# bigpon/QPNet

Hardware: AMD Instinct MI355X
Metric: train steps/sec (batch-1 chunk-steps of RF+20000 samples, aggregate over GPUs) (higher is better)
Workload: dtype f32; 1 GPU; config[1]: paper-size SI-QPNet (C=64,S=256,4F+4A) training step, forward+CE+backward+Adam on one chunk of 20900 samples (RF 946 + batch_length 19954), batch 1 per GPU; global_batch=1, parallelism=dp1 (utterance-sharded chunks, one flat-gradient all-reduce per step), backend=none, world_size=1, aux_1x1=frame rate (hoisted: K = 128 + one 4-deep step)

## Files before the change

### qpnet_amd/csrc/train_bwd.hip

```cpp
#include "train_common.h"
#include "train_post.h"
#include "qpn_handle.h"
#include <string.h>
#include <stdlib.h>
#include <math.h>

template <int MT>
__global__ __launch_bounds__(512) void k_post_bwd(TrainParams p, TrainBwd bw) {
    constexpr int TM = 16 * MT;
    extern __shared__ float sm[];
    const int S = p.S, Q = p.Q, LC = p.LC;
    const int ldp = tr_lda(Q > S ? Q : S), ldr = tr_lda(S);
    float* P = sm; float* R = sm + TM * ldp;
    const int b = blockIdx.y, t0 = blockIdx.x * TM;
    const int tid = threadIdx.x, lane = tid & 63, wave = tid >> 6;
    const int NTS = S / 16;
    const int npairs = (NTS + 1) / 2;
    const int np0 = wave < npairs ? wave : 0;
    const int pnt[2] = {2 * np0, (2 * np0 + 1 < NTS) ? 2 * np0 + 1 : 2 * np0};
    float my[2][MT][4], ms[2][MT][4];
    auto mask_load = [&](const float* src, float (&m)[2][MT][4]) {
#pragma unroll
        for (int j = 0; j < 2; ++j)
#pragma unroll
// ... 1031 lines not shown
            float ev[TR_EB_SLOTS];
#pragma unroll
            for (int k = 0; k < TR_EB_SLOTS; ++k) ev[k] = p.EB[(size_t)(l * TR_EB_SLOTS + k) * 2 * C + n];
#pragma unroll
            for (int k = 0; k < TR_EB_SLOTS; ++k) e += ev[k];
        }
        float acc = 0.f;
        for (int b = 0; b < p.B; ++b) {
            const float* hb = p.h + ((size_t)b * A + a) * p.F + p.ffirst;
            const float* D = p.DPA + (size_t)(l * p.B + b) * (p.nfr + 1) * 2 * C + n;
            for (int f0 = 0; f0 < p.nfr; f0 += 1024) {
                const int nf = p.nfr - f0 < 1024 ? p.nfr - f0 : 1024;
                __syncthreads();
                for (int i = tid; i < nf; i += 128) hrow[i] = hb[f0 + i];
                __syncthreads();
                int f = 0;
                for (; f + 64 <= nf; f += 64) {
                    float d[64];
#pragma unroll
                    for (int k = 0; k < 64; ++k) d[k] = D[(size_t)(f0 + f + k) * 2 * C];
#pragma unroll
                    for (int k = 0; k < 64; ++k) acc += d[k] * hrow[f + k];
                }
                for (; f + 16 <= nf; f += 16) {
                    float d[16];
#pragma unroll
                    for (int k = 0; k < 16; ++k) d[k] = D[(size_t)(f0 + f + k) * 2 * C];
#pragma unroll
                    for (int k = 0; k < 16; ++k) acc += d[k] * hrow[f + k];
                }
                for (; f < nf; ++f) acc += D[(size_t)(f0 + f) * 2 * C] * hrow[f];
            }
        }
        p.gflat[wi] = (acc + p.flat[p.up_b] * e) * p.gscale;
        v = va * e;
    } else {
        const int j = bx - L * A;
        const int q0 = p.F * p.U - p.N1;
        const int items = L * p.B * p.nfr;
        for (int it = tid; it < items; it += 128) {
            const int fx = it % p.nfr, lb = it / p.nfr, l = lb / p.B;
            const int n = (p.ffirst + fx) * p.U + j - q0;
            if (n >= ag.s_out[l] && n < p.N1) v += p.GW[(size_t)lb * p.N1 + n];
        }
    }
    for (int sft = 32; sft >= 1; sft >>= 1) v += __shfl_xor(v, sft);
    if ((tid & 63) == 0) red[tid >> 6] = v;
    __syncthreads();
    if (tid == 0) {
        if (role_a) atomicAdd(p.gflat + p.up_b, (red[0] + red[1]) * p.gscale);
        else p.gflat[p.up_w + (bx - L * A)] = (red[0] + red[1]) * p.gscale;
    }
}

struct AdamReports { int* h_status; double* h_loss; const double* d_loss; };
__device__ __forceinline__ void adam_update(float* __restrict__ w, float* __restrict__ m, float* __restrict__ v, int64_t i, float gi,
                                            float lr, float b1, float b2, float eps, float wd, float bc1, float bc2_sqrt) {
    if (wd != 0.f) gi += wd * w[i];
    const float mi = m[i] + (gi - m[i]) * (1.0f - b1);
    const float vi = v[i] * b2 + (1.0f - b2) * gi * gi;
    m[i] = mi; v[i] = vi;
    const float denom = sqrtf(vi) / bc2_sqrt + eps;
    w[i] = w[i] - (lr / bc1) * (mi / denom);
}
__global__ void k_adam(float* __restrict__ w, const float* __restrict__ g, float* __restrict__ m, float* __restrict__ v, int64_t n,
                       float lr, float b1, float b2, float eps, float wd, float bc1, float bc2_sqrt, const float* __restrict__ den, int* __restrict__ status, AdamReports rep) {
    int64_t i = (int64_t)blockIdx.x * blockDim.x + threadIdx.x;
    const bool peer = den && den[1] > 0.f;
    const bool skip = peer || (status && *status);
    if (blockIdx.x == 0) {
        if (rep.h_loss && threadIdx.x < 64) rep.h_loss[threadIdx.x] = rep.d_loss[threadIdx.x];
        if (threadIdx.x == 0 && status) {
            int st = *status;
            if (peer && !st) { st = 8; atomicOr(status, 8); }
            if (rep.h_status) *rep.h_status = st;
            if (!skip) atomicAdd((unsigned long long*)(status + 2), 1ull);
        }
    }
    if (i >= n || skip) return;
    float gi = g[i];
    if (den) gi = gi / den[0];
    adam_update(w, m, v, i, gi, lr, b1, b2, eps, wd, bc1, bc2_sqrt);
}

__device__ __forceinline__ double block_sum_f64(double x, double* red) {
    for (int sft = 32; sft >= 1; sft >>= 1) x += __shfl_xor(x, sft);
    if ((threadIdx.x & 63) == 0) red[threadIdx.x >> 6] = x;
    __syncthreads();
    return (red[0] + red[1]) + (red[2] + red[3]);
}
__global__ __launch_bounds__(256) void k_grad_sumsq(const float* __restrict__ g, int64_t n, double* __restrict__ part) {
    __shared__ double red[4];
    const int64_t nq = n >> 2, nthr = (int64_t)gridDim.x * 256, t = (int64_t)blockIdx.x * 256 + threadIdx.x;
    double acc = 0.0;
    if ((reinterpret_cast<uintptr_t>(g) & 15) == 0) {
        const float4* g4 = reinterpret_cast<const float4*>(g);
#pragma unroll 4
        for (int64_t q = t; q < nq; q += nthr) {
            const float4 x = g4[q];
            acc += (double)x.x * (double)x.x; acc += (double)x.y * (double)x.y; acc += (double)x.z * (double)x.z; acc += (double)x.w * (double)x.w;
        }
    } else {
#pragma unroll 4
        for (int64_t q = t; q < nq; q += nthr) {
            const float x0 = g[4 * q], x1 = g[4 * q + 1], x2 = g[4 * q + 2], x3 = g[4 * q + 3];
            acc += (double)x0 * (double)x0; acc += (double)x1 * (double)x1; acc += (double)x2 * (double)x2; acc += (double)x3 * (double)x3;
        }
    }
    if (t == nq % nthr) for (int64_t i = nq * 4; i < n; ++i) acc += (double)g[i] * (double)g[i];
    const double s = block_sum_f64(acc, red);
    if (threadIdx.x == 0) part[blockIdx.x] = s;
}

__global__ __launch_bounds__(256) void k_adam_clip(float* __restrict__ w, const float* __restrict__ g, float* __restrict__ m, float* __restrict__ v, int64_t n,
                                                   float lr, float b1, float b2, float eps, float wd, float bc1, float bc2_sqrt, const float* __restrict__ den, int* __restrict__ status, AdamReports rep,
                                                   const double* __restrict__ part, int npart, float max_norm, double* __restrict__ d_norm, double* h_norm) {
    __shared__ double red[4];
    int64_t i = (int64_t)blockIdx.x * blockDim.x + threadIdx.x;
    double total = sqrt(block_sum_f64((int)threadIdx.x < npart ? part[threadIdx.x] : 0.0, red));
    if (den) total = total / (double)den[0];
    const bool bad = !isfinite(total);
    const bool peer = den && den[1] > 0.f;
    const bool skip = bad || peer || (status && *status);
    if (blockIdx.x == 0) {
        if (rep.h_loss && threadIdx.x < 64) rep.h_loss[threadIdx.x] = rep.d_loss[threadIdx.x];
        if (threadIdx.x == 0) {
            *d_norm = total;
            if (h_norm) *h_norm = total;
            if (status) {
                int st = *status;
                if (peer && !st) { st = 8; atomicOr(status, 8); }
                if (bad) { st |= 1 << 16; atomicOr(status, 1 << 16); }
                if (rep.h_status) *rep.h_status = st;
                if (!skip) atomicAdd((unsigned long long*)(status + 2), 1ull);
            }
        }
    }
    if (i >= n || skip) return;
    const double c = (double)max_norm / (total + 1e-6);
    const float coef = c < 1.0 ? (float)c : 1.0f;
    float gi = g[i];
    if (den) gi = gi / den[0];
    gi = __fmul_rn(gi, coef);
    adam_update(w, m, v, i, gi, lr, b1, b2, eps, wd, bc1, bc2_sqrt);
}

__device__ __forceinline__ void zero_dx_slice(const TrainParams& p, const TrainBwd& bw, int j, int b, size_t part, size_t nparts, int t, int nthr) {
    const int C = p.C;
    const TrLayer ly = p.layers[j];
    const size_t nDX = (size_t)p.B * p.N1 * C;
    float* A = bw.DXA[0] + (size_t)j * nDX + (size_t)b * p.N1 * C;
    float* Bq = bw.DXB[0] + (size_t)j * nDX + (size_t)b * p.N1 * C;
    const int a0 = j == 0 ? 0 : ly.s_in, a1 = ly.s_out;
    const int b0 = ly.adaptive ? 0 : p.N1 - ly.dilation, b1 = p.N1;
    const size_t na = (size_t)(a1 - a0) * C / 4, nb = (size_t)(b1 > b0 ? b1 - b0 : 0) * C / 4;
    const float4 z = make_float4(0.f, 0.f, 0.f, 0.f);
    const size_t nh = p.hoist ? (size_t)(p.nfr + 1) * 2 * C / 4 : (j == 0 ? (size_t)p.N1 * p.Ap / 4 : 0);
    const size_t ne = (p.hoist && b == 0) ? (size_t)TR_EB_SLOTS * 2 * C / 4 : 0;
    float* H = p.hoist ? bw.DPA + (size_t)(j * p.B + b) * (p.nfr + 1) * 2 * C : bw.DHUP + (size_t)b * p.N1 * p.Ap;
    for (size_t i = part * nthr + t; i < na + nb + nh + ne; i += nparts * nthr) {
        if (i < na) ((float4*)(A + (size_t)a0 * C))[i] = z;
        else if (i < na + nb) ((float4*)(Bq + (size_t)(b0 > 0 ? b0 : 0) * C))[i - na] = z;
        else if (i < na + nb + nh) ((float4*)H)[i - na - nb] = z;
        else ((float4*)(bw.EB + (size_t)j * TR_EB_SLOTS * 2 * C))[i - na - nb - nh] = z;
    }
}
__global__ void k_zero_dx(TrainParams p, TrainBwd bw) {
    zero_dx_slice(p, bw, blockIdx.y, blockIdx.z, blockIdx.x, gridDim.x, threadIdx.x, blockDim.x);
}

void qpn_launch_zero_dx(const TrainParams& p, const TrainBwd& bw, hipStream_t stream) {
    hipLaunchKernelGGL(k_zero_dx, dim3(64, p.L, p.B), dim3(256), 0, stream, p, bw);
}

static void launch_reduce_early(const TrainBwd& bw, hipStream_t st, int tail, int nch_side) {
    const TrainSlabs& sl = *bw.sl;
    const int64_t n = (int64_t)(sl.g_early1 - sl.g_early0) + (tail ? bw.n_gzero + 4 : 0);
    hipLaunchKernelGGL(k_reduce_grad_s, dim3((unsigned)((n + 255) / 256)), dim3(256), 0, st, bw.slab, bw.gdst, bw.gdst_list, bw.gzero, bw.n_gzero,
                       nch_side, bw.gstage, bw.n_params, bw.gflat, bw.gscale, bw.append_scale, sl.g_early0, sl.g_early1, 0, 0, tail, bw.status, 0);
}
static void launch_up_bwd(const TrainParams& p, const TrainBwd& bw, hipStream_t st) {
    const UpArgs u = up_args(p, bw);
    hipLaunchKernelGGL(k_up_bwd, dim3(u.nfr, p.B), dim3(128), 0, st, u);
}

static void launch_aux_tail(const TrainParams& p, const TrainBwd& bw, const AuxGeom& ag, hipStream_t st) {
    hipLaunchKernelGGL(k_aux_tail, dim3(p.L * p.A + p.U), dim3(128), 0, st, tr_aux_args(p, &bw, ag));
}

int qpn_launch_grad_tail(const TrainParams& p, const TrainBwd& bw, const AuxGeom* ag, hipStream_t stream, bool early_done, bool up_done) {
    const int C = p.C, Q = p.Q, B = p.B, N1 = p.N1;
    const TrainSlabs& sl = *bw.sl;
    hipLaunchKernelGGL(k_reduce_grad_s, dim3((unsigned)(((int64_t)bw.gstage + (up_done ? 0 : bw.n_gzero + 4) + 255) / 256)), dim3(256), 0, stream, bw.slab, bw.gdst, bw.gdst_list, bw.gzero, bw.n_gzero,
                       bw.nch, bw.gstage, bw.n_params, bw.gflat, bw.gscale, bw.append_scale, 0, bw.gstage, early_done ? sl.g_early0 : 0, early_done ? sl.g_early1 : 0, up_done ? 0 : 1, bw.status, bw.append_scale == 1 ? 1 : 0);
    {
        const int64_t total = (int64_t)B * N1;
        const int nwg = 128, rpw = (int)((total + nwg - 1) / nwg);
        if (sl.g_cw < 0) {
            int CB = C < 64 ? C : 64;
            while (CB > 1 && (size_t)2 * Q * CB * sizeof(float) > 128 * 1024) CB /= 2;
            const size_t lds_c = (size_t)2 * Q * CB * sizeof(float);
            if (lds_c > 160 * 1024) { qpn_set_error("causal-table gradient: n_quantize too large for the LDS histogram"); return QPN_EINVAL; }
            if (lds_c > 48 * 1024) QPN_HIP(hipFuncSetAttribute((const void*)k_causal_bwd, hipFuncAttributeMaxDynamicSharedMemorySize, (int)lds_c));
            hipLaunchKernelGGL(k_causal_bwd, dim3(nwg), dim3(256), lds_c, stream, p, bw, rpw, CB);
        }
        if (p.U > 0 && !up_done && !p.hoist) launch_up_bwd(p, bw, stream);
        if (p.hoist && ag && !up_done) launch_aux_tail(p, bw, *ag, stream);
    }
    qpn_prof_mark(PG_GRAD_TAIL, stream);
    QPN_HIP(hipGetLastError());
    return QPN_OK;
}

bool qpn_stack_bwd_fits(const TrainParams& p);
int qpn_launch_stack_bwd(const TrainParams& p, const TrainBwd& bw, const StackQ& q, const TrainKnobs& k, hipStream_t stream);

void qpn_launch_post_fb(const TrainParams& p, const TrainBwd& bw, hipStream_t stream) {
    constexpr int MTW = 5;
    const size_t ldsw = (size_t)16 * MTW * (tr_lda(256) + 2 * tr_lda(64)) * sizeof(float);
    (void)hipFuncSetAttribute((const void*)k_post_fb_w<MTW>, hipFuncAttributeMaxDynamicSharedMemorySize, (int)ldsw);
    hipLaunchKernelGGL((k_post_fb_w<MTW>), dim3((p.BL + 16 * MTW - 1) / (16 * MTW), p.B), dim3(512), ldsw, stream, p, bw, 1);
}

int qpn_launch_bwd(const TrainParams& p, const TrainBwd& bw, const TrainKnobs& k, const AuxGeom& ag, const StackQ* sq, hipStream_t stream, bool post_done) {
    const int C = p.C, S = p.S, Q = p.Q, L = p.L, B = p.B, N1 = p.N1, BL = p.BL;
    const TrainSlabs& sl = *bw.sl;
    const bool off32 = N1 < (1 << 24) && (int64_t)N1 * (p.LC > 2 * C ? p.LC : 2 * C) < (1ll << 32);
    const bool persist = C == 64 && (p.Ktp == 176 || p.hoist) && p.Ap <= 64 && off32 && k.persist_bwd;
    const bool stack_q = persist && k.stack_q_bwd && sq && sq->flags && p.qctl && qpn_stack_bwd_fits(p);
    const bool wr_summed = stack_q;
    const size_t nDX = (size_t)B * N1 * C;
    const size_t lds_post = (size_t)16 * (tr_lda(Q > S ? Q : S) + tr_lda(S)) * sizeof(float);
    const size_t lds_layer = (size_t)16 * (4 * tr_lda(C) + tr_lda(2 * C)) * sizeof(float);
    if (lds_post > 160 * 1024 || lds_layer > 160 * 1024) { qpn_set_error("backward tiles do not fit LDS"); return QPN_EINVAL; }
    hipStream_t side = bw.side; hipEvent_t ev_fork = bw.ev_fork, ev_join = bw.ev_join;
    const bool overlap = side && !qpn_prof_serial() && !k.serial;
    const bool post_wide = S == 256 && Q == 256 && C == 64 && (p.LC == 256 || p.LC == 512) && k.post_wide;
    const bool zero_in_post = post_wide && k.zero_in_post;
    if (post_done) { }
    else if (!zero_in_post) qpn_launch_zero_dx(p, bw, stream);
    if (post_done) { }
    else if (post_wide) {
        constexpr int MTW = 5;
        const size_t ldsw = (size_t)16 * MTW * tr_lda(256) * sizeof(float);
        QPN_HIP(hipFuncSetAttribute((const void*)k_post_bwd_w<MTW>, hipFuncAttributeMaxDynamicSharedMemorySize, (int)ldsw));
        hipLaunchKernelGGL((k_post_bwd_w<MTW>), dim3((BL + 16 * MTW - 1) / (16 * MTW), B), dim3(512), ldsw, stream, p, bw, zero_in_post ? 1 : 0);
    } else {
        if (lds_post > 48 * 1024) (void)hipFuncSetAttribute((const void*)k_post_bwd<1>, hipFuncAttributeMaxDynamicSharedMemorySize, (int)lds_post);
        hipLaunchKernelGGL((k_post_bwd<1>), dim3((BL + 15) / 16, B), dim3(512), lds_post, stream, p, bw);
    }
    qpn_prof_mark(PG_POST_BWD, stream);
    const int nch = bw.nch;
    int nch_side_ = nch;
    const bool gen = k.wgrad_generic;
    Wg2 wbase; memset(&wbase, 0, sizeof(wbase));
    wbase.slab = bw.slab; wbase.gstage = bw.gstage; wbase.nb = B; wbase.C = C; wbase.Ap = p.Ap; wbase.hup = p.HUP; wbase.tap = p.TAP; wbase.ncol_groups = 1;
    bool ok = true;
    auto launch_skip_post = [&](hipStream_t st) {
        Wg2 w = wbase;
        {
            w.nlayers = L;
            w.A = bw.DS0; w.A2 = nullptr; w.A_lstride = 0; w.lda = S; w.M = S; w.rowsA = BL;
            w.bmode = 0; w.B1 = p.TH; w.B2 = nullptr; w.B_lstride = nDX; w.ldb = C; w.N = C; w.Nvalid = C; w.rowsB = N1; w.ldc = C;
            w.ncol_groups = wgrad_col_groups(w.M, w.N);
            for (int l = 0; l < L; ++l) { w.row0A[l] = 0; w.row0B[l] = N1 - BL; w.R[l] = BL; w.goff[l] = sl.g_ws[l]; w.gbias[l] = l == 0 ? sl.g_bs : -1; w.tap_off[l] = -1; }
            ok = ok && wgrad2_any(w, nch_side_, gen, st);
            qpn_prof_mark(PG_WGRAD_SKIP, st);
        }
        {
            w.nlayers = 1; w.A_lstride = w.B_lstride = 0; w.B2 = nullptr; w.bmode = 1; w.rowsA = w.rowsB = BL;
            w.row0A[0] = w.row0B[0] = 0; w.R[0] = BL; w.tap_off[0] = -1;
            w.ncol_groups = S % 64 == 0 ? S / 64 : 1;
            w.A = bw.dlogits; w.lda = Q; w.M = Q; w.B1 = p.Y0; w.ldb = S; w.N = S; w.Nvalid = S; w.ldc = S; w.goff[0] = sl.g_p2; w.gbias[0] = sl.g_bp2;
            if (Q == S && k.post_pair) {
                w.nlayers = 2;
                w.A_lstride = (size_t)(bw.DY0 - bw.dlogits); w.B_lstride = (size_t)(p.S0 - p.Y0);
                w.row0A[1] = w.row0B[1] = 0; w.R[1] = BL; w.tap_off[1] = -1; w.goff[1] = sl.g_p1; w.gbias[1] = sl.g_bp1;
                ok = ok && wgrad2_any(w, nch_side_, gen, st);
            } else {
                ok = ok && wgrad2_any(w, nch_side_, gen, st);
                w.A = bw.DY0; w.lda = S; w.M = S; w.B1 = p.S0; w.goff[0] = sl.g_p1; w.gbias[0] = sl.g_bp1;
                ok = ok && wgrad2_any(w, nch_side_, gen, st);
            }
            qpn_prof_mark(PG_WGRAD_POST, st);
        }
    };
    auto build_w1 = [&]() {
        Wg2 w = wbase;
        w.A = bw.DZ; w.A2 = nullptr; w.A_lstride = (size_t)B * N1 * 2 * C; w.lda = 2 * C; w.M = 2 * C; w.rowsA = N1;
        w.bmode = 3; w.B1 = p.X; w.B2 = nullptr; w.B_lstride = nDX; w.ldb = C; w.N = p.Ktp; w.Nvalid = p.hoist ? 2 * C : 2 * C + p.Ap; w.rowsB = N1;
        w.nlayers = L; w.ldc = p.Ktp; w.ncol_groups = wgrad_col_groups(w.M, w.N);
        for (int l = 0; l < L; ++l) {
            const TrLayer& ly = p.layers[l];
            w.row0A[l] = w.row0B[l] = ly.s_out; w.R[l] = N1 - ly.s_out; w.goff[l] = sl.g_w1[l]; w.gbias[l] = sl.g_b1[l];
            w.tap_off[l] = ly.tap_off; w.dil[l] = ly.dilation;
        }
        return w;
    };
    auto build_wr = [&]() {
        Wg2 w = wbase;
        w.A = bw.DXA[0] + nDX; w.A2 = wr_summed ? nullptr : bw.DXB[0] + nDX; w.A_lstride = nDX; w.lda = C; w.M = C; w.rowsA = N1;
        w.bmode = 0; w.B1 = p.TH; w.B2 = nullptr; w.B_lstride = nDX; w.ldb = C; w.N = C; w.Nvalid = C; w.rowsB = N1; w.ldc = C;
        w.nlayers = L; w.ncol_groups = wgrad_col_groups(w.M, w.N);
        for (int l = 0; l < L; ++l) {
            w.row0A[l] = w.row0B[l] = p.layers[l].s_out;
            w.R[l] = l == L - 1 ? 0 : N1 - p.layers[l].s_out; w.goff[l] = sl.g_wr[l]; w.gbias[l] = sl.g_br[l]; w.tap_off[l] = -1; w.dil[l] = 0;
        }
        return w;
    };
    const bool early_reduce = overlap && bw.gdst && sl.g_early1 > sl.g_early0 && k.reduce_early;
    const bool up_side = early_reduce && p.U > 0 && k.up_side;
    if (early_reduce) {
        nch_side_ = k.wgrad_chunks_side > 0 && k.wgrad_chunks_side <= nch ? k.wgrad_chunks_side : (nch <= 48 ? nch : 48);
    }
    if (overlap) {
        QPN_HIP(hipEventRecord(ev_fork, stream));
        QPN_HIP(hipStreamWaitEvent(side, ev_fork, 0));
        qpn_prof_mark(-1, side);
        launch_skip_post(side);
        if (early_reduce) { launch_reduce_early(bw, side, up_side ? 1 : 0, nch_side_); qpn_prof_mark(PG_GRAD_TAIL, side); }
        if (early_reduce && up_side && bw.ev_early && bw.early_recorded) { QPN_HIP(hipEventRecord(bw.ev_early, side)); *bw.early_recorded = 1; }
    }
    const int swz = k.xcd_swizzle ? 1 : 0;
    if (p.hoist && !persist) { qpn_set_error("internal: the frame-rate aux term needs the register-resident layer kernels"); return QPN_EINVAL; }
    if (stack_q) {
        const int rcq = qpn_launch_stack_bwd(p, bw, *sq, k, stream);
        if (rcq) return rcq;
    }
    for (int l = L - 1; l >= 0 && !stack_q; --l) {
        const TrLayer& ly = p.layers[l];
        const int rows = N1 - ly.s_out;
        const int tiles = (rows + 15) / 16;
        if (persist) {
            int G = qpn_num_cus() * 2; if (G > tiles) G = tiles;
            if (G > 1024) G = 1024;
            const size_t ldsp = (size_t)(8 * 16 * tr_lda(C) + 16 * tr_lda(2 * C) + 16 * tr_lda(p.Ktp) + 64) * sizeof(float);
            const bool last = l == L - 1;
            const void* kf = p.hoist ? (last ? (const void*)k_layer_bwd_p<8, true> : (const void*)k_layer_bwd_p<8, false>)
                                     : (last ? (const void*)k_layer_bwd_p<11, true> : (const void*)k_layer_bwd_p<11, false>);
            (void)hipFuncSetAttribute(kf, hipFuncAttributeMaxDynamicSharedMemorySize, (int)ldsp);
            if (p.hoist) {
                if (last) hipLaunchKernelGGL((k_layer_bwd_p<8, true>), dim3(G, B), dim3(256), ldsp, stream, p, bw, l, swz ? 2 : 0, tiles, p.scratch_rows);
                else hipLaunchKernelGGL((k_layer_bwd_p<8, false>), dim3(G, B), dim3(256), ldsp, stream, p, bw, l, swz ? 2 : 0, tiles, p.scratch_rows);
            } else {
                if (last) hipLaunchKernelGGL((k_layer_bwd_p<11, true>), dim3(G, B), dim3(256), ldsp, stream, p, bw, l, swz ? 2 : 0, tiles, p.scratch_rows);
                else hipLaunchKernelGGL((k_layer_bwd_p<11, false>), dim3(G, B), dim3(256), ldsp, stream, p, bw, l, swz ? 2 : 0, tiles, p.scratch_rows);
            }
        } else {
            if (lds_layer > 48 * 1024) (void)hipFuncSetAttribute((const void*)k_layer_bwd<1>, hipFuncAttributeMaxDynamicSharedMemorySize, (int)lds_layer);
            hipLaunchKernelGGL((k_layer_bwd<1>), dim3(tiles, B), dim3(256), lds_layer, stream, p, bw, l, l == L - 1 ? 1 : 0, swz);
        }
    }
    auto build_causal = [&]() {
        Wg2 w = wbase;
        w.nlayers = 2; w.ncol_groups = Q / (Q % 64 == 0 ? 64 : 128);      w.bmode = 4; w.xc = p.XC; w.B1 = w.B2 = nullptr; w.B_lstride = 0;
        w.A = bw.DXA[0]; w.A2 = bw.DXB[0]; w.A_lstride = 0; w.lda = C; w.M = C; w.rowsA = N1;
        w.N = Q; w.Nvalid = Q; w.rowsB = N1 + 1; w.ldb = 0; w.ldc = Q;
        for (int tp = 0; tp < 2; ++tp) { w.row0A[tp] = 0; w.row0B[tp] = tp; w.R[tp] = N1; w.goff[tp] = sl.g_cw + tp * C * Q; w.gbias[tp] = tp == 0 ? sl.g_cb : -1; w.tap_off[tp] = -1; w.dil[tp] = 0; }
        return w;
    };
    const bool wr_side = overlap && k.wr_side;
    if (wr_side || up_side) {
        QPN_HIP(hipEventRecord(bw.ev_mid, stream));
        QPN_HIP(hipStreamWaitEvent(side, bw.ev_mid, 0));
        qpn_prof_mark(-1, side);
        if (up_side) { if (p.hoist) launch_aux_tail(p, bw, ag, side); else launch_up_bwd(p, bw, side); qpn_prof_mark(PG_GRAD_TAIL, side); }
        if (wr_side) { ok = ok && wgrad2_any(build_wr(), nch, gen, side); qpn_prof_mark(PG_WGRAD_WR, side); }
    }
    if (overlap) QPN_HIP(hipEventRecord(ev_join, side));
    qpn_prof_mark(PG_LAYER_BWD, stream);
    ok = ok && wgrad2_any(build_w1(), nch, gen, stream);
    qpn_prof_mark(PG_WGRAD, stream);
    if (!wr_side) { ok = ok && wgrad2_any(build_wr(), nch, gen, stream); qpn_prof_mark(PG_WGRAD_WR, stream); }
    if (!overlap) launch_skip_post(stream);
    if (sl.g_cw >= 0) ok = ok && wgrad2_any(build_causal(), nch, gen, stream);
    qpn_prof_mark(PG_WGRAD_CAUSAL, stream);
    if (overlap) { QPN_HIP(hipStreamWaitEvent(stream, ev_join, 0)); qpn_prof_mark(-1, stream); }
    if (!ok) { qpn_set_error("weight-gradient tiles: unsupported geometry (n_resch <= 128 on this path; wider stacks take the GEMM path)"); return QPN_EINVAL; }
    return qpn_launch_grad_tail(p, bw, &ag, stream, early_reduce, up_side);
}

int qpn_launch_adam(float* w, const float* g, float* m, float* v, int64_t n, int step, float lr, float b1, float b2, float eps, float wd, const float* den, int* status,
                    int* h_status, double* h_loss, const double* d_loss, hipStream_t stream) {
// ... 22 lines not shown
```

### qpnet_amd/csrc/train_common.h

```cpp
#pragma once
#include "qpn_common.h"

typedef float f32x4 __attribute__((ext_vector_type(4)));

#define TR_MAXL QPN_MAX_LAYERS

__host__ __device__ static inline int tr_lda(int K) { return ((K + 29) / 32) * 32 + 2; }
__host__ __device__ static inline int tr_ldt(int N) { return ((N + 15) / 32) * 32 + 16; }

struct TrLayer {
    int adaptive, dilation;
    int s_in, s_out;
    int tap_off;
    int w1_f4, wr_f4;
    int w1t_f4, wrt_f4;
    int bias1, biasr;
};

struct TrainParams {
    int C, S, Q, A, Ap, L, U;
    int B, T, F, Td, BL, N1, N0, maxd;
    int Kt, Ktp;
    int LC;
    const float* flat;
    const float4* wp;
    const float* ct;
    float* bp;
    const int64_t* x; const float* h; const float* d;
    float* X;
    float* SG; float* TH;
    float* HUP;
    int hoist;
    int nfr, ffirst;
    float* PA;
    float2* WJ;
    int* TAP;
    int* XC;
    float* S0; float* Y0;
    float* logits;
    const int64_t* ce_tgt; int64_t ce_stride; float* ce_dlogits; double* ce_loss;
    int* status;
    float* scratch_rows;
    unsigned* qctl;
    int4* qtab;
    int4* qtab_b;
    int qtotal;
    int qP[TR_MAXL + 1];
    int qT[TR_MAXL];
    int ws_f4, p1_f4, p2_f4;
    int wst_f4, p1t_f4, p2t_f4;
    int bias_s, bias_p1, bias_p2;
    int64_t causal_w, causal_b, up_w, up_b;
    TrLayer layers[TR_MAXL];
};

struct TrainSlabs {
    int g_w1[TR_MAXL], g_b1[TR_MAXL], g_wr[TR_MAXL], g_br[TR_MAXL], g_ws[TR_MAXL], g_bs;
    int g_p1, g_bp1, g_p2, g_bp2;
    int g_early0, g_early1;
    int g_cw, g_cb;
};

struct TrainBwd {
    const float* dlogits; float* gflat;
    float* DXA[2]; float* DXB[2];
    float* DZ;
    float* DS0; float* DY0;
    float* DGS;
    float* DHUP;
    float* DPA;
    float* GW;
    float* EB;
    float* slab;
    const int* gdst; const int* gdst_list;
    const int* gzero; int n_gzero;
    int nch, gstage;
    int64_t n_params;
    const struct TrainSlabs* sl;
    float gscale;
    int append_scale;
    const int* status;
    hipStream_t side; hipEvent_t ev_fork, ev_join, ev_mid;
    hipEvent_t ev_early; int* early_recorded;
};


struct AuxGeom { int auxS[TR_MAXL], auxT[TR_MAXL], bias1[TR_MAXL], s_out[TR_MAXL]; };
struct AuxArgs {
    const float* flat; const float* h; float* PA; float* bp; const float* DPA; const float* EB; const float* GW; float* gflat;
    float gscale; int C, A, L, B, F, U, N1, nfr, ffirst; int64_t up_w, up_b;
    AuxGeom g;
};
static inline AuxArgs tr_aux_args(const TrainParams& p, const TrainBwd* bw, const AuxGeom& ag) {
    AuxArgs a; a.flat = p.flat; a.h = p.h; a.PA = p.PA; a.bp = p.bp; a.DPA = bw ? bw->DPA : nullptr; a.EB = bw ? bw->EB : nullptr; a.GW = bw ? bw->GW : nullptr;
    a.gflat = bw ? bw->gflat : nullptr; a.gscale = bw ? bw->gscale : 1.f;
    a.C = p.C; a.A = p.A; a.L = p.L; a.B = p.B; a.F = p.F; a.U = p.U; a.N1 = p.N1; a.nfr = p.nfr; a.ffirst = p.ffirst; a.up_w = p.up_w; a.up_b = p.up_b; a.g = ag;
    return a;
}
struct TrainKnobs {
    bool serial;
    bool stack_q_fwd, stack_q_bwd;
    int stack_wgs, stack_wgs_bwd;
    bool persist_fwd, persist_bwd;
    bool wgrad_generic;
    int wgrad_chunks, wgrad_chunks_side;
    bool post_fuse;
    bool up_side, reduce_early, wr_side;
    bool post_pair, zero_in_post, post_wide;
    bool xcd_swizzle;
    bool ce_separate;
    bool event_fence;
    bool aux_hoist;
    bool test_stack_gives_up;
};
void qpn_train_knobs_parse(TrainKnobs& k);

#define TR_QHEAD_STRIDE 1056
#define TR_QHDR_WORDS 17920
struct StackQ {
    unsigned* flags;
    unsigned* head;
    unsigned* stats;
    unsigned* abort;
    const int4* tab;
    unsigned epoch;
    unsigned epoch_pub;
    unsigned spin_limit;
    int total, nq;
};

__host__ __device__ __forceinline__ int tr_pa_off(const TrainParams& p, int l, int b, int n0) {
    const int q = p.F * p.U - p.N1 + n0;
    return ((l * p.B + b) * (p.nfr + 1) + (q / p.U - p.ffirst)) * 2 * p.C;
}

__device__ __forceinline__ void tr_queue_entry_fwd(const TrainParams& p, int pos, int4& a, int4& b) {
    const bool valid = pos < p.qtotal;
    const int ps = valid ? pos : 0;
    int l = 0;
    for (int k = 1; k < p.L; ++k) l += ps >= p.qP[k] ? 1 : 0;
    const int r = ps - p.qP[l], T = p.qT[l];
    const int bi = r / T, t = r - bi * T;
    const TrLayer ly = p.layers[l];
    const int n0 = ly.s_out + 16 * t;
    int first = 0, n = 0;
    if (valid && l > 0) {
        const int reach = ly.s_out - ly.s_in, s_prev = p.layers[l - 1].s_out;
        int lo = n0 - reach; if (lo < s_prev) lo = s_prev;
        int hi = n0 + 15; if (hi > p.N1 - 1) hi = p.N1 - 1;
        const int t_lo = (lo - s_prev) >> 4, t_hi = (hi - s_prev) >> 4;
        first = p.qP[l - 1] + bi * p.qT[l - 1] + t_lo; n = t_hi - t_lo + 1;
    }
    a = make_int4(n0, l | (bi << 8) | (l == p.L - 1 ? 1 << 24 : 0) | (valid ? 1 << 25 : 0), first, n);
    b = make_int4((l * p.B + bi) * p.N1, ly.tap_off + bi * p.N1, p.hoist ? tr_pa_off(p, l, bi, n0) : bi * p.N1, 0);
}

__device__ __forceinline__ void tr_queue_entry_bwd(const TrainParams& p, int pos, int4& a, int4& b) {
    const bool valid = pos < p.qtotal;
    const int ps = valid ? pos : 0;
    int k = 0, base = 0;
    for (int j = 0; j + 1 < p.L; ++j) { const int n = p.B * p.qT[p.L - 1 - j]; if (ps >= base + n) { base += n; k = j + 1; } else break; }
    const int l = p.L - 1 - k;
    const int r = ps - base, T = p.qT[l];
    const int bi = r / T, t = r - bi * T;
    const TrLayer ly = p.layers[l];
    const int n0 = ly.s_out + 16 * t;
    int first = 0, n = 0;
    if (valid && l < p.L - 1) {
        const TrLayer up = p.layers[l + 1];
        const int reach = up.s_out - up.s_in;
        int lo = n0 - up.s_out; if (lo < 0) lo = 0;
        int hi = n0 + 15 + reach; if (hi > p.N1 - 1) hi = p.N1 - 1;
        hi -= up.s_out;
        const int t_lo = lo >> 4, t_hi = hi >> 4;
        const int pbase = base - p.B * p.qT[l + 1];
        first = pbase + bi * p.qT[l + 1] + t_lo; n = t_hi - t_lo + 1;
    }
    a = make_int4(n0, l | (bi << 8) | (l == p.L - 1 ? 1 << 24 : 0) | (valid ? 1 << 25 : 0) | (ly.adaptive ? 1 << 26 : 0), first, n);
    b = make_int4((l * p.B + bi) * p.N1, ly.tap_off + bi * p.N1, p.hoist ? tr_pa_off(p, l, bi, n0) : bi * p.N1, bi * p.BL * p.LC + l * p.C);
}

struct TrainGemm {
    const float* wp;
    float* G;
    int K1;
    int N1g, Cg, Sg, Qg, LCg, Ktg;
    long w1[TR_MAXL], w1t[TR_MAXL], wr[TR_MAXL], wrt[TR_MAXL];
    long ws, wst, p1, p1t, p2, p2t;
};

#define TR_LDS_BARRIER() asm volatile("s_waitcnt lgkmcnt(0)\n\ts_barrier" ::: "memory")

int qpn_num_cus();

#define TR_GN_BLOCKS 256

enum { PG_PREP = 0, PG_LAYER_FWD, PG_POST_FWD, PG_CE, PG_POST_BWD, PG_WGRAD, PG_LAYER_BWD, PG_GRAD_TAIL, PG_ADAM, PG_ALLREDUCE,
       PG_WGRAD_WR, PG_WGRAD_SKIP, PG_WGRAD_POST, PG_WGRAD_CAUSAL, PG_COUNT };
void qpn_prof_mark(int group, hipStream_t stream);
bool qpn_prof_serial();
bool qpn_prof_active();

__device__ __forceinline__ int tr_xcd_tile(int orig, int nwg, int swz) {
    if (!swz || nwg <= 8) return orig;
    const int q = nwg / 8, r = nwg % 8, xcd = orig % 8;
    return (xcd < r ? xcd * (q + 1) : r * (q + 1) + (xcd - r) * q) + orig / 8;
}

__device__ __forceinline__ void tr_tile_range(int orig, int G, int tiles, int swz, int& t_first, int& t_count) {
    const int base = tiles / G, rem = tiles - base * G;
    if (!swz || G <= 8) { t_first = orig * base + (orig < rem ? orig : rem); t_count = base + (orig < rem ? 1 : 0); return; }
    const int q = G / 8, r = G % 8, xcd = orig % 8, j = orig / 8;
    const int g = (xcd < r ? xcd * (q + 1) : r * (q + 1) + (xcd - r) * q) + j;
    int before = 0;
    for (int x = 0; x < xcd; ++x) before += rem > x ? (rem - x + 7) / 8 : 0;
    const int mine = rem > xcd ? (rem - xcd + 7) / 8 : 0;
    before += j < mine ? j : mine;
    t_first = g * base + before; t_count = base + (orig < rem ? 1 : 0);
}

__device__ __forceinline__ int tr_aux_slot(float2 wj, int row) { return __float_as_int(wj.y) < row ? 1 : 0; }
__device__ __forceinline__ float tr_aux_a(float2 wj, int lane) { return tr_aux_slot(wj, lane & 15) == (lane >> 4) ? wj.x : 0.f; }
__device__ __forceinline__ float tr_dpp_row_sum(float a) {
    a += __int_as_float(__builtin_amdgcn_update_dpp(0, __float_as_int(a), 0x128, 0xf, 0xf, true));
    a += __int_as_float(__builtin_amdgcn_update_dpp(0, __float_as_int(a), 0x124, 0xf, 0xf, true));
    a += __int_as_float(__builtin_amdgcn_update_dpp(0, __float_as_int(a), 0x4E, 0xf, 0xf, true));
    a += __int_as_float(__builtin_amdgcn_update_dpp(0, __float_as_int(a), 0xB1, 0xf, 0xf, true));
    return a;
}
__device__ __forceinline__ float tr_wave_max(float a) {
    a = fmaxf(a, __int_as_float(__builtin_amdgcn_update_dpp(0, __float_as_int(a), 0x128, 0xf, 0xf, true)));
    a = fmaxf(a, __int_as_float(__builtin_amdgcn_update_dpp(0, __float_as_int(a), 0x124, 0xf, 0xf, true)));
    a = fmaxf(a, __int_as_float(__builtin_amdgcn_update_dpp(0, __float_as_int(a), 0x4E, 0xf, 0xf, true)));
    a = fmaxf(a, __int_as_float(__builtin_amdgcn_update_dpp(0, __float_as_int(a), 0xB1, 0xf, 0xf, true)));
    const int i = __float_as_int(a);
    return fmaxf(fmaxf(__int_as_float(__builtin_amdgcn_readlane(i, 0)), __int_as_float(__builtin_amdgcn_readlane(i, 16))),
                 fmaxf(__int_as_float(__builtin_amdgcn_readlane(i, 32)), __int_as_float(__builtin_amdgcn_readlane(i, 48))));
}
__device__ __forceinline__ float tr_wave_sum(float a) {
    const int i = __float_as_int(tr_dpp_row_sum(a));
    return (__int_as_float(__builtin_amdgcn_readlane(i, 0)) + __int_as_float(__builtin_amdgcn_readlane(i, 16))) +
           (__int_as_float(__builtin_amdgcn_readlane(i, 32)) + __int_as_float(__builtin_amdgcn_readlane(i, 48)));
}
struct TrAuxBwd { float d[4]; float gp[4]; float e[2]; };
#define TR_EB_SLOTS 32
__device__ __forceinline__ TrAuxBwd tr_aux_bwd(const float2 (&wj)[4], const float (&pa)[4], const float (&dzs)[4], const float (&dzt)[4], int lane) {
    TrAuxBwd o;
    f32x4 as = (f32x4){0, 0, 0, 0}, at = (f32x4){0, 0, 0, 0};
    const int m = lane & 15, g4 = 4 * (lane >> 4);
#pragma unroll
    for (int i = 0; i < 4; ++i) {
        const int k = tr_aux_slot(wj[i], g4 + i);
        const float a = m == 2 ? 1.f : (k == m ? wj[i].x : 0.f);
        as = __builtin_amdgcn_mfma_f32_16x16x4f32(a, dzs[i], as, 0, 0, 0);
        at = __builtin_amdgcn_mfma_f32_16x16x4f32(a, dzt[i], at, 0, 0, 0);
        o.gp[i] = tr_dpp_row_sum(dzs[i] * (k ? pa[2] : pa[0]) + dzt[i] * (k ? pa[3] : pa[1]));
    }
    o.d[0] = as[0]; o.d[1] = at[0]; o.d[2] = as[1]; o.d[3] = at[1];
    o.e[0] = as[2]; o.e[1] = at[2];
    return o;
}

template <int MT, int NJ>
__device__ __forceinline__ void wave_gemm_step(f32x4 (&acc)[MT][NJ], const float* __restrict__ A_lds, int lda, int ks4, int arow, int ak, const float4 (&b)[NJ]) {
#pragma unroll
    for (int mt = 0; mt < MT; ++mt) {
        const float* ap = A_lds + (size_t)(16 * mt + arow) * lda + 16 * ks4 + ak;
        const float a0 = ap[0], a1 = ap[4], a2 = ap[8], a3 = ap[12];
#pragma unroll
        for (int j = 0; j < NJ; ++j) {
            acc[mt][j] = __builtin_amdgcn_mfma_f32_16x16x4f32(a0, b[j].x, acc[mt][j], 0, 0, 0);
            acc[mt][j] = __builtin_amdgcn_mfma_f32_16x16x4f32(a1, b[j].y, acc[mt][j], 0, 0, 0);
            acc[mt][j] = __builtin_amdgcn_mfma_f32_16x16x4f32(a2, b[j].z, acc[mt][j], 0, 0, 0);
            acc[mt][j] = __builtin_amdgcn_mfma_f32_16x16x4f32(a3, b[j].w, acc[mt][j], 0, 0, 0);
        }
    }
}
template <int MT, int NJ>
__device__ __forceinline__ void wave_gemm(f32x4 (&acc)[MT][NJ], const float* __restrict__ A_lds, int lda,
                                          const float4* __restrict__ Bp, int NT, const int (&nts)[NJ], int K, int lane) {
    const int arow = lane & 15, ak = lane >> 4;
    const int nk = K / 16;
    float4 b0[NJ], b1[NJ];
#pragma unroll
    for (int j = 0; j < NJ; ++j) b0[j] = Bp[(size_t)nts[j] * 64 + lane];
    int ks4 = 0;
    for (; ks4 + 1 < nk; ks4 += 2) {
#pragma unroll
        for (int j = 0; j < NJ; ++j) b1[j] = Bp[((size_t)(ks4 + 1) * NT + nts[j]) * 64 + lane];
        __builtin_amdgcn_sched_barrier(0);
        wave_gemm_step<MT, NJ>(acc, A_lds, lda, ks4, arow, ak, b0);
        __builtin_amdgcn_sched_barrier(0);
        const int kn = ks4 + 2 < nk ? ks4 + 2 : nk - 1;
#pragma unroll
        for (int j = 0; j < NJ; ++j) b0[j] = Bp[((size_t)kn * NT + nts[j]) * 64 + lane];
        __builtin_amdgcn_sched_barrier(0);
        wave_gemm_step<MT, NJ>(acc, A_lds, lda, ks4 + 1, arow, ak, b1);
        __builtin_amdgcn_sched_barrier(0);
    }
    if (ks4 < nk) wave_gemm_step<MT, NJ>(acc, A_lds, lda, ks4, arow, ak, b0);
}

template <int NJ, int PD>
__device__ __forceinline__ void wave_b_preload(float4 (&bq)[PD][NJ], const float4* __restrict__ Bp, int NT, const int (&nts)[NJ], int K, int lane) {
    const int nk = K / 16;
#pragma unroll
    for (int d = 0; d < PD; ++d) {
        const int kd = d < nk ? d : nk - 1;
#pragma unroll
        for (int j = 0; j < NJ; ++j) bq[d][j] = Bp[((size_t)kd * NT + nts[j]) * 64 + lane];
    }
}
template <int MT, int NJ, int PD>
__device__ __forceinline__ void wave_gemm_run(f32x4 (&acc)[MT][NJ], const float* __restrict__ A_lds, int lda, float4 (&bq)[PD][NJ],
                                              const float4* __restrict__ Bp, int NT, const int (&nts)[NJ], int K, int lane) {
    const int arow = lane & 15, ak = lane >> 4;
    const int nk = K / 16;
    for (int ks0 = 0; ks0 < nk; ks0 += PD) {
        const bool more = ks0 + PD < nk;
#pragma unroll
        for (int d = 0; d < PD; ++d) {
            const int ks4 = ks0 + d;
            if (ks4 < nk) {
#pragma unroll
                for (int mt = 0; mt < MT; ++mt) {
                    const float* ap = A_lds + (size_t)(16 * mt + arow) * lda + 16 * ks4 + ak;
                    const float a0 = ap[0], a1 = ap[4], a2 = ap[8], a3 = ap[12];
#pragma unroll
                    for (int j = 0; j < NJ; ++j) {
                        acc[mt][j] = __builtin_amdgcn_mfma_f32_16x16x4f32(a0, bq[d][j].x, acc[mt][j], 0, 0, 0);
                        acc[mt][j] = __builtin_amdgcn_mfma_f32_16x16x4f32(a1, bq[d][j].y, acc[mt][j], 0, 0, 0);
// ... 66 lines not shown
```

### qpnet_amd/csrc/train_fwd.hip

```cpp
#include "train_common.h"
#include "train_post.h"

__device__ __forceinline__ float sigmoidf_(float z) { return __builtin_amdgcn_rcpf(1.0f + __expf(-z)); }
__device__ __forceinline__ float tanhf_(float z) { return 2.0f * __builtin_amdgcn_rcpf(1.0f + __expf(-2.0f * z)) - 1.0f; }

#define AUXP_FPB 8
__device__ __forceinline__ void aux_proj_block(const TrainParams& p, const AuxGeom& ag, int fxb, int l, int b, float* sm) {
    const int fx0 = fxb * AUXP_FPB, tid = threadIdx.x, n = tid & 127, fh = tid >> 7, C = p.C, A = p.A, CA = C * A;
    float* Va = sm; float* hs = sm + 2 * CA;
    {
        const float* s0 = p.flat + ag.auxS[l]; const float* s1 = p.flat + ag.auxT[l];
        for (int base = 0; base < 2 * CA; base += 256 * 16) {
            float v[16];
#pragma unroll
            for (int k = 0; k < 16; ++k) { const int i = base + 256 * k + tid, ic = i < 2 * CA ? i : 0; v[k] = ic < CA ? s0[ic] : s1[ic - CA]; }
#pragma unroll
            for (int k = 0; k < 16; ++k) { const int i = base + 256 * k + tid; if (i < 2 * CA) Va[i] = v[k]; }
        }
    }
    for (int i = tid; i < A * AUXP_FPB; i += 256) {
        const int a = i / AUXP_FPB, f = i - a * AUXP_FPB, fx = fx0 + f;
        hs[i] = fx < p.nfr ? p.h[((size_t)b * A + a) * p.F + p.ffirst + fx] : 0.f;
    }
    __syncthreads();
    float acc[4] = {0.f, 0.f, 0.f, 0.f}, vs = 0.f;
    for (int a = 0; a < A; ++a) {
        const float v = Va[n * A + a];
        const float4 h4 = *(const float4*)(hs + a * AUXP_FPB + 4 * fh);
        acc[0] += v * h4.x; acc[1] += v * h4.y; acc[2] += v * h4.z; acc[3] += v * h4.w;
        vs += v;
    }
    float* out = p.PA + ((size_t)(l * p.B + b) * (p.nfr + 1) + fx0 + 4 * fh) * 2 * C + n;
#pragma unroll
    for (int f = 0; f < 4; ++f) if (fx0 + 4 * fh + f <= p.nfr) out[(size_t)f * 2 * C] = acc[f];
    if (fxb == 0 && b == 0 && fh == 0) p.bp[ag.bias1[l] + n] += p.flat[p.up_b] * vs;
}

__global__ __launch_bounds__(256) void k_train_prep(TrainParams p, AuxGeom ag, int nprep) {
    const int b = blockIdx.y;
    if ((int)blockIdx.x >= nprep) {
        extern __shared__ float sm[];
        const int idx = blockIdx.x - nprep, nfxb = (p.nfr + 1 + AUXP_FPB - 1) / AUXP_FPB;
        aux_proj_block(p, ag, idx % nfxb, idx / nfxb, b, sm);
        return;
    }
    const int C = p.C, Q = p.Q, N1 = p.N1, Ap = p.Ap;
    const int C4 = C / 4, A4 = Ap / 4;
    const int nX = N1 * C4, nH = p.hoist ? 0 : N1 * A4;
    const int total = nX + nH + N1 * p.L;
    if (p.hoist && b == 0)
        for (int n = blockIdx.x * 256 + threadIdx.x; n < N1 + 16; n += nprep * 256) {
            const int q = p.F * p.U - N1 + n, j = q - (q / p.U) * p.U;
            p.WJ[n] = make_float2(p.flat[p.up_w + j], __int_as_float(j));
        }
    if (p.qctl && blockIdx.x == 0 && b == 0 && threadIdx.x < 32) p.qctl[threadIdx.x < 16 ? threadIdx.x : 1024 + (threadIdx.x - 16) * TR_QHEAD_STRIDE] = 0u;
    if (p.qtab && b == 0)
        for (int pos = blockIdx.x * 256 + threadIdx.x; pos <= p.qtotal; pos += nprep * 256) {
            int4 ea, eb; tr_queue_entry_fwd(p, pos, ea, eb);
            p.qtab[2 * pos] = ea; p.qtab[2 * pos + 1] = eb;
            if (p.qtab_b) { tr_queue_entry_bwd(p, pos, ea, eb); p.qtab_b[2 * pos] = ea; p.qtab_b[2 * pos + 1] = eb; }
        }
    for (int it = blockIdx.x * 256 + threadIdx.x; it < total; it += nprep * 256) {
        if (it < nX) {
            const int n = it / C4, c = (it - n * C4) * 4;
            const int64_t xo = (int64_t)p.T - p.N0 + n;
            int64_t s0 = p.x[(size_t)b * p.T + xo] % Q, s1 = p.x[(size_t)b * p.T + xo + 1] % Q;
            if (s0 < 0) s0 += Q;
            if (s1 < 0) s1 += Q;
            const float4 r0 = *(const float4*)(p.ct + (size_t)s0 * C + c);
            const float4 r1 = *(const float4*)(p.ct + ((size_t)Q + s1) * C + c);
            const float4 bb = *(const float4*)(p.flat + p.causal_b + c);
            float4 v;
            v.x = (r0.x + r1.x) + bb.x; v.y = (r0.y + r1.y) + bb.y; v.z = (r0.z + r1.z) + bb.z; v.w = (r0.w + r1.w) + bb.w;
            *(float4*)(p.X + ((size_t)b * N1 + n) * C + c) = v;
            if (c == 0) { p.XC[(size_t)b * (N1 + 1) + n] = (int)s0; if (n == N1 - 1) p.XC[(size_t)b * (N1 + 1) + N1] = (int)s1; }
        } else if (it < nX + nH) {
            const int i2 = it - nX, n = i2 / A4, a0 = (i2 - n * A4) * 4;
            float v[4];
            int64_t f = 0; int j = 0;
            if (p.U > 0) { const int64_t q = (int64_t)p.F * p.U - N1 + n; f = q / p.U; j = (int)(q - f * p.U); }
            else f = (int64_t)p.F - N1 + n;
            const float wj = p.U > 0 ? p.flat[p.up_w + j] : 1.0f, ub = p.U > 0 ? p.flat[p.up_b] : 0.0f;
#pragma unroll
            for (int e = 0; e < 4; ++e) {
                const int a = a0 + e;
                float t = 0.0f;
                if (a < p.A) { t = p.h[((size_t)b * p.A + a) * p.F + f]; if (p.U > 0) t = t * wj + ub; }
                v[e] = t;
            }
            *(float4*)(p.HUP + ((size_t)b * N1 + n) * Ap + a0) = make_float4(v[0], v[1], v[2], v[3]);
        } else {
            const int i3 = it - nX - nH, l = i3 / N1, n = i3 - l * N1;
            const TrLayer ly = p.layers[l];
            int tap;
            if (ly.adaptive) {
                const float dv = p.d[(size_t)b * p.Td + (p.Td - N1 + n)];
                const float dil = -dv * (float)ly.dilation;
                const float s = __fadd_rn(dil, (float)(n - N1));
                tap = N1 + (int)rintf(s);
                if (n >= ly.s_out && (tap < ly.s_in || tap > n)) { atomicOr(p.status, 1); }
            } else tap = n - ly.dilation;
            tap = tap < 0 ? 0 : (tap >= N1 ? N1 - 1 : tap);
            p.TAP[ly.tap_off + (size_t)b * N1 + n] = tap;
        }
    }
}

template <int MT>
__device__ __forceinline__ void layer_fwd_tile(const TrainParams& p, const int l, const int last, const int b, const int n0, float* sm) {
    constexpr int TM = 16 * MT;
    const TrLayer ly = p.layers[l];
    const int C = p.C, Ktp = p.Ktp, Ap = p.Ap;
    const int lda = tr_lda(Ktp), ldg = tr_lda(C);
    float* As = sm; float* Gs = sm + TM * lda;
    const int tid = threadIdx.x, lane = tid & 63, wave = tid >> 6;
    const float* Xin = p.X + ((size_t)(l * p.B + b) * p.N1) * C;
    const float* hup = p.HUP + (size_t)b * p.N1 * Ap;
    const int* taps = p.TAP + ly.tap_off + (size_t)b * p.N1;
    const float* bias1 = p.bp + ly.bias1;
    const float* br = p.bp + ly.biasr;
    const int cpre = 16 * (wave < C / 16 ? wave : 0) + (lane & 15);
    const float bs_pre = bias1[cpre], bt_pre = bias1[C + cpre], bb_pre = br[cpre];
    float4 wrq[4][1];
    if (!last) { const int ntp[1] = {wave < C / 16 ? wave : 0}; wave_b_preload<1, 4>(wrq, p.wp + ly.wr_f4, C / 16, ntp, C, lane); }
    {
        const int K4 = Ktp / 4;
        const int tpr = K4 < 64 ? K4 : 64;
        const int rpp = 256 / tpr;
        const int tr = tid / tpr, tc = tid - tr * tpr;
        constexpr int NR = TM / 4;
        if (tr < rpp) {
            int tp[NR];
#pragma unroll
            for (int k = 0; k < NR; ++k) {
                const int n = n0 + tr + k * rpp;
                tp[k] = taps[n < p.N1 ? n : p.N1 - 1];
            }
            for (int c4 = tc; c4 < K4; c4 += tpr) {
                const int k0 = c4 * 4;
                const int kind = k0 < C ? 0 : k0 < 2 * C ? 1 : k0 < 2 * C + Ap ? 2 : 3;
                const bool from_x = kind <= 1;
                const int col = kind == 0 ? k0 : kind == 1 ? k0 - C : kind == 2 ? k0 - 2 * C : 0;
                const unsigned long long ax = (unsigned long long)Xin, ah = (unsigned long long)hup;
                const float* base = (const float*)(from_x ? ax : ah) + col;
                const int stride = from_x ? C : Ap;
                float4 v[NR];
#pragma unroll
                for (int k = 0; k < NR; ++k) {
                    const int r = tr + k * rpp, n = n0 + r;
                    const bool ok = r < TM && n < p.N1 && kind != 3;
                    const int row = ok ? (kind == 1 ? tp[k] : n) : 0;
                    v[k] = *(const float4*)(base + (size_t)row * stride);
                }
                __builtin_amdgcn_sched_barrier(0);
#pragma unroll
                for (int k = 0; k < NR; ++k) {
                    const int r = tr + k * rpp;
                    if (r < TM) {
                        const bool ok = n0 + r < p.N1 && kind != 3;
                        const float4 w = ok ? v[k] : make_float4(0.f, 0.f, 0.f, 0.f);
                        float* dst = As + (size_t)r * lda + k0;
                        *(float2*)dst = make_float2(w.x, w.y); *(float2*)(dst + 2) = make_float2(w.z, w.w);
                    }
                }
            }
        }
    }
    __syncthreads();
    const float4* W1 = p.wp + ly.w1_f4;
    asm volatile("" :: "v"(bs_pre), "v"(bt_pre), "v"(bb_pre));
    float* SG = p.SG + ((size_t)(l * p.B + b) * p.N1) * C;
    float* TH = p.TH + ((size_t)(l * p.B + b) * p.N1) * C;
    const int NCG = C / 16;
    for (int cg = wave; cg < NCG; cg += 4) {
        f32x4 acc[MT][2];
#pragma unroll
        for (int mt = 0; mt < MT; ++mt) { acc[mt][0] = (f32x4){0, 0, 0, 0}; acc[mt][1] = (f32x4){0, 0, 0, 0}; }
        const int nts[2] = {cg, NCG + cg};
        wave_gemm<MT, 2>(acc, As, lda, W1, 2 * NCG, nts, Ktp, lane);
        const int c = 16 * cg + (lane & 15);
        const float bs = cg == wave ? bs_pre : bias1[c], bt = cg == wave ? bt_pre : bias1[C + c];
#pragma unroll
        for (int mt = 0; mt < MT; ++mt)
#pragma unroll
            for (int i = 0; i < 4; ++i) {
                const int r = 16 * mt + 4 * (lane >> 4) + i;
                const float sg = sigmoidf_(acc[mt][0][i] + bs);
                const float th = tanhf_(acc[mt][1][i] + bt);
                const float gg = sg * th;
                Gs[(size_t)r * ldg + c] = gg;
                if (n0 + r < p.N1) { SG[(size_t)(n0 + r) * C + c] = sg; TH[(size_t)(n0 + r) * C + c] = gg; }
            }
    }
    if (last) return;
    __syncthreads();
    const float4* Wr = p.wp + ly.wr_f4;
    float* Xout = p.X + ((size_t)((l + 1) * p.B + b) * p.N1) * C;
    for (int nt = wave; nt < NCG; nt += 4) {
        f32x4 acc[MT][1];
#pragma unroll
        for (int mt = 0; mt < MT; ++mt) acc[mt][0] = (f32x4){0, 0, 0, 0};
        const int nts[1] = {nt};
        if (nt == wave) wave_gemm_run<MT, 1, 4>(acc, Gs, ldg, wrq, Wr, NCG, nts, C, lane);
        else wave_gemm_deep<MT, 1, 4>(acc, Gs, ldg, Wr, NCG, nts, C, lane);
        const int c = 16 * nt + (lane & 15);
        const float bb = nt == wave ? bb_pre : br[c];
#pragma unroll
        for (int mt = 0; mt < MT; ++mt)
#pragma unroll
            for (int i = 0; i < 4; ++i) {
                const int r = 16 * mt + 4 * (lane >> 4) + i;
                if (n0 + r < p.N1) Xout[(size_t)(n0 + r) * C + c] = (acc[mt][0][i] + bb) + As[(size_t)r * lda + c];
            }
    }
}

template <int MT>
__global__ __launch_bounds__(256) void k_layer_fwd(TrainParams p, int l, int last) {
    extern __shared__ float sm[];
    layer_fwd_tile<MT>(p, l, last & 1, blockIdx.y, p.layers[l].s_out + tr_xcd_tile(blockIdx.x, gridDim.x, last & 2) * 16 * MT, sm);
}

template <int KS, bool LAST>
__global__ __launch_bounds__(256, 2) void k_layer_fwd_p(TrainParams p, int l, int flags, int tiles, float* dummy) {
    constexpr int C = 64, Ktp = 16 * KS;
    constexpr bool HOIST = KS == 8;
    constexpr int lda = ((Ktp + 29) / 32) * 32 + 2, ldg = ((C + 29) / 32) * 32 + 2;
    extern __shared__ float sm[];
    float* Gs = sm + 32 * lda;
    float* SGs = Gs + 16 * ldg; float* THs = SGs + 16 * ldg; float* Xs = THs + 16 * ldg;
    const TrLayer ly = p.layers[l];
    const int Ap = p.Ap, N1 = p.N1;
    const int tid = threadIdx.x, lane = tid & 63, wave = __builtin_amdgcn_readfirstlane(tid >> 6);
    const int b = blockIdx.y;
    int t_first, t_count;
    tr_tile_range(blockIdx.x, gridDim.x, tiles, flags & 2, t_first, t_count);
    if (t_count <= 0) return;
    const int t_last = t_first + t_count - 1;
    const float* Xin = p.X + ((size_t)(l * p.B + b) * N1) * C;
    const float* hup = p.HUP + (size_t)b * N1 * Ap;
    const int* taps = p.TAP + ly.tap_off + (size_t)b * N1;
    float* SG = p.SG + ((size_t)(l * p.B + b) * N1) * C;
    float* TH = p.TH + ((size_t)(l * p.B + b) * N1) * C;
    float* Xout = p.X + ((size_t)((l + 1) * p.B + b) * N1) * C;
    const float4* W1 = p.wp + ly.w1_f4; const float4* Wr = p.wp + ly.wr_f4;
    float4 w1[KS][2], wr[4];
#pragma unroll
    for (int ks = 0; ks < KS; ++ks) { w1[ks][0] = W1[((size_t)ks * 8 + wave) * 64 + lane]; w1[ks][1] = W1[((size_t)ks * 8 + 4 + wave) * 64 + lane]; }
#pragma unroll
    for (int ks = 0; ks < 4; ++ks) wr[ks] = LAST ? make_float4(0.f, 0.f, 0.f, 0.f) : Wr[((size_t)ks * 4 + wave) * 64 + lane];
    const int c = 16 * wave + (lane & 15);
    const float bs = p.bp[ly.bias1 + c], bt = p.bp[ly.bias1 + C + c], bb = p.bp[ly.biasr + c];
    const int srow = tid >> 4, sc4 = tid & 15;
    const bool aux_thread = sc4 < (Ktp - 2 * C) / 4, aux_real = 4 * sc4 < Ap;
    const int orow = tid >> 5, oc2 = (tid & 31) * 2;
    float* const dmy = dummy + (size_t)(blockIdx.y * gridDim.x + blockIdx.x) * 2 * C + oc2;
// ... 464 lines not shown
```

### qpnet_amd/csrc/train_host.hip

```cpp
#include "train_common.h"
#include "qpn_handle.h"
#include <algorithm>
#include <string.h>

int qpn_launch_fwd(const TrainParams& p, const TrainKnobs& k, const AuxGeom& ag, const StackQ* sq, hipStream_t stream, const TrainBwd* fuse_post_bwd);
void qpn_stack_fill(TrainParams& p);
int qpn_launch_ce(const float* logits, const int64_t* tgt, int64_t tgt_stride, int B, int BL, int Q, float* dlogits, double* loss, int* status, bool loss_cleared, hipStream_t stream);
int qpn_launch_bwd(const TrainParams& p, const TrainBwd& bw, const TrainKnobs& k, const AuxGeom& ag, const StackQ* sq, hipStream_t stream, bool post_done);
int qpn_launch_fwd_gemm(const TrainParams& p, const TrainGemm& w, hipStream_t stream);
int qpn_launch_bwd_gemm(const TrainParams& p, const TrainBwd& bw, const TrainGemm& w, hipStream_t stream);
int qpn_launch_adam(float* w, const float* g, float* m, float* v, int64_t n, int step, float lr, float b1, float b2, float eps, float wd, const float* den, int* status,
                    int* h_status, double* h_loss, const double* d_loss, hipStream_t stream);
int qpn_launch_adam_clip(float* w, const float* g, float* m, float* v, int64_t n, int step, float lr, float b1, float b2, float eps, float wd, const float* den, int* status,
                         int* h_status, double* h_loss, const double* d_loss, float max_norm, double* part, double* d_norm, double* h_norm, hipStream_t stream);

#define LOSS_SLOT 72

struct TrainState {
    std::vector<int> h_wmap;
    std::vector<int> h_bstart, h_blist;
    std::vector<int> h_gsrc;
    int* d_wmap; float* d_wp; int* d_bstart; int* d_blist; float* d_bp; int n_bias;
    int* d_gdst; int* d_gdst_list; int* d_gzero; int n_gzero;
    bool hoist;
    TrainParams tp;
    TrainBwd bw;
    TrainSlabs slabs;
    TrainKnobs knobs;
    AuxGeom ag;
    float* d_ws; size_t ws_cap;
    int* d_tap; size_t tap_cap;
    int* d_status; double* d_loss;
    hipStream_t last_stream;
    int* h_status_pinned; hipEvent_t ev_status[2]; bool status_pending[2]; int status_newest;
    double* h_loss_pinned; hipEvent_t ev_loss[2]; bool loss_pending[2]; int loss_newest;
    double* d_gnorm; bool gnorm_last;
    bool gnorm_slot[2];
    double gnorm_collected; bool gnorm_collected_valid;
    bool fwd_valid;
    bool loss_clear;
    bool use_gemm;
    int* d_ctmap; float* d_ct;
    std::vector<int> h_gmap; int* d_gmap; float* d_gwp;
    TrainGemm gm;
    int64_t generation;
    hipStream_t side; hipEvent_t ev_fork, ev_join, ev_mid;
    hipEvent_t ev_early; int early_recorded; int64_t early_first;
    int64_t bwd_generation;
    const float* post_bwd_dlogits;
    bool post_bwd_done;
    bool stack_disabled;
    unsigned* d_sq; size_t sq_pos_cap, sq_per_dir;
    StackQ sqf, sqb;
};

static int env_int(const char* name, int dflt) { const char* e = getenv(name); return (e && *e) ? atoi(e) : dflt; }
void qpn_train_knobs_parse(TrainKnobs& k) {
    k.serial = env_int("QPN_TRAIN_SERIAL", 0) != 0;
    k.stack_q_fwd = env_int("QPN_STACK_QUEUE", 1) != 0;
    k.stack_q_bwd = k.stack_q_fwd && env_int("QPN_STACK_QUEUE_BWD", 1) != 0;
    k.stack_wgs = env_int("QPN_STACK_WGS", 0); if (k.stack_wgs < 0 || k.stack_wgs > 4096) k.stack_wgs = 0;
    k.stack_wgs_bwd = env_int("QPN_STACK_WGS_BWD", 0); if (k.stack_wgs_bwd < 0 || k.stack_wgs_bwd > 4096) k.stack_wgs_bwd = 0;
    k.persist_fwd = env_int("QPN_LAYER_PERSIST", 1) != 0;
    k.persist_bwd = env_int("QPN_LAYER_BWD_PERSIST", 1) != 0;
    k.wgrad_generic = getenv("QPN_WGRAD_GENERIC") != nullptr;
    k.wgrad_chunks = env_int("QPN_WGRAD_CHUNKS", 0); if (k.wgrad_chunks < 1 || k.wgrad_chunks > 512) k.wgrad_chunks = 0;
    k.wgrad_chunks_side = env_int("QPN_WGRAD_CHUNKS_SIDE", 0); if (k.wgrad_chunks_side < 1 || k.wgrad_chunks_side > 512) k.wgrad_chunks_side = 0;
    k.up_side = env_int("QPN_UP_SIDE", 1) != 0;
    k.reduce_early = env_int("QPN_REDUCE_EARLY", 1) != 0;
    k.wr_side = env_int("QPN_WR_SIDE", 1) != 0;
    k.post_fuse = env_int("QPN_POST_FUSE", 1) != 0;
    k.post_pair = env_int("QPN_POST_WGRAD_PAIR", 1) != 0;
    k.zero_in_post = env_int("QPN_ZERO_IN_POST", 1) != 0;
    k.post_wide = env_int("QPN_POST_WIDE", 1) != 0;
    k.xcd_swizzle = getenv("QPN_NO_XCD_SWIZZLE") == nullptr;
    k.ce_separate = getenv("QPN_CE_SEPARATE") != nullptr;
    k.event_fence = env_int("QPN_EVENT_FENCE", 0) == 1;
    k.aux_hoist = env_int("QPN_AUX_HOIST", 1) != 0;
    k.test_stack_gives_up = false;
#ifdef QPN_TESTING
    k.test_stack_gives_up = env_int("QPN_TEST_STACK_GIVES_UP", 0) == 1;
#endif
}

int qpn_num_cus() {
    static int cached[64] = {0};
    int dev = 0;
    if (hipGetDevice(&dev) != hipSuccess || dev < 0 || dev >= 64) return 256;
    if (!cached[dev]) { int n = 0; if (hipDeviceGetAttribute(&n, hipDeviceAttributeMultiprocessorCount, dev) != hipSuccess || n < 1) n = 256; cached[dev] = n; }
    return cached[dev];
}

struct Prof { bool on = false; bool overlapped = false; std::vector<hipEvent_t> ev; std::vector<int> grp; std::vector<hipStream_t> st; size_t used = 0; };
static thread_local Prof g_prof;
bool qpn_prof_active() { return g_prof.on; }
bool qpn_prof_serial() { return g_prof.on && !g_prof.overlapped; }
void qpn_prof_mark(int group, hipStream_t stream) {
    Prof& P = g_prof;
    if (!P.on) return;
    if (P.used == P.ev.size()) { hipEvent_t e; if (hipEventCreate(&e) != hipSuccess) return; P.ev.push_back(e); P.grp.push_back(0); P.st.push_back(nullptr); }
    P.grp[P.used] = group; P.st[P.used] = stream;
    (void)hipEventRecord(P.ev[P.used++], stream);
}
extern "C" int qpn_train_profile_begin(qpn_handle* h, void* stream) {
    (void)h; g_prof.on = true; g_prof.overlapped = false; g_prof.used = 0;
    qpn_prof_mark(-1, (hipStream_t)stream);
    return QPN_OK;
}
extern "C" int qpn_train_profile_begin_overlapped(qpn_handle* h, void* stream) {
    (void)h; g_prof.on = true; g_prof.overlapped = true; g_prof.used = 0;
    qpn_prof_mark(-1, (hipStream_t)stream);
    return QPN_OK;
}
extern "C" int qpn_train_profile_mark(qpn_handle* h, int group, void* stream) {
    (void)h; qpn_prof_mark(group, (hipStream_t)stream); return QPN_OK;
}
extern "C" int qpn_train_profile_end(qpn_handle* h, float* h_ms, int n, void* stream) {
    Prof& P = g_prof;
    QPN_HIP(hipStreamSynchronize((hipStream_t)stream));
    if (h && h->train && h->train->side) QPN_HIP(hipStreamSynchronize(h->train->side));
    for (int i = 0; i < n; ++i) h_ms[i] = 0.f;
    for (size_t i = 1; i < P.used; ++i) {
        if (P.grp[i] < 0 || P.grp[i] >= n) continue;
        size_t j = i;
        while (j > 0 && P.st[j - 1] != P.st[i]) --j;
        if (j == 0) continue;
        float ms = 0.f;
        QPN_HIP(hipEventElapsedTime(&ms, P.ev[j - 1], P.ev[i]));
        h_ms[P.grp[i]] += ms;
    }
    P.on = false;
    return QPN_OK;
}

__global__ void k_gather_f(const float* __restrict__ flat, const int* __restrict__ map, float* __restrict__ out, int64_t n) {
    int64_t i = (int64_t)blockIdx.x * blockDim.x + threadIdx.x;
    if (i < n) { int m = map[i]; out[i] = m >= 0 ? flat[m] : 0.0f; }
}
__global__ void k_refresh(const float* __restrict__ flat, const int* __restrict__ wmap, float* __restrict__ wout, int64_t nw,
                          const int* __restrict__ ctmap, float* __restrict__ ct, int64_t nct,
                          const int* __restrict__ bstart, const int* __restrict__ blist, float* __restrict__ bp, int nb,
                          int* __restrict__ status, double* __restrict__ loss) {
    int64_t i = (int64_t)blockIdx.x * blockDim.x + threadIdx.x;
    if (i < nw) { const int m = wmap[i]; wout[i] = m >= 0 ? flat[m] : 0.0f; return; }
    i -= nw;
    if (i < nct) { ct[i] = flat[ctmap[i]]; return; }
    i -= nct;
    if (i < nb) { float a = 0.f; for (int j = bstart[i]; j < bstart[i + 1]; ++j) a += flat[blist[j]]; bp[i] = a; return; }
    i -= nb;
    (void)status;
    if (i >= 16 && i < 16 + 64) loss[i - 16] = 0.0;
}
template <class F>
static long kmajor_pack(std::vector<int>& map, int K, int Kp, int N, int Np, F src) {
    const long off = (long)map.size();
    map.resize(map.size() + (size_t)Kp * Np, -1);
    int* m = map.data() + off;
    for (int k = 0; k < K; ++k)
        for (int n = 0; n < N; ++n) m[(size_t)k * Np + n] = (int)src(k, n);
    return off;
}
static inline int pad_to(int v, int q) { return (v + q - 1) / q * q; }

template <class F>
static int frag_pack(std::vector<int>& map, int K, int N, F src) {
    const int NT = N / 16, off4 = (int)(map.size() / 4);
    map.resize(map.size() + (size_t)K * N);
    int* m = map.data() + (size_t)off4 * 4;
    for (int ks4 = 0; ks4 < K / 16; ++ks4)
        for (int nt = 0; nt < NT; ++nt)
            for (int lane = 0; lane < 64; ++lane)
                for (int e = 0; e < 4; ++e) {
                    int k = 16 * ks4 + 4 * e + (lane >> 4), n = 16 * nt + (lane & 15);
                    m[(((size_t)ks4 * NT + nt) * 64 + lane) * 4 + e] = (int)src(k, n);
                }
    return off4;
}

static int train_init(qpn_handle* h) {
    if (h->train) return QPN_OK;
    const Geom& g = h->g;
    const int C = g.C, S = g.S, Q = g.Q, A = g.A, L = g.L;
    if (L > TR_MAXL) { qpn_set_error("training kernels support up to %d residual layers", TR_MAXL); return QPN_EINVAL; }
    if (C % 16 || S % 16 || Q % 16) { qpn_set_error("training kernels need n_resch, n_skipch, n_quantize multiples of 16"); return QPN_EINVAL; }
    TrainState* t = new TrainState();
    memset(&t->tp, 0, sizeof(t->tp)); memset(&t->bw, 0, sizeof(t->bw));
    t->d_wmap = nullptr; t->d_wp = nullptr; t->d_bstart = t->d_blist = nullptr; t->d_bp = nullptr;
    t->d_gdst = t->d_gdst_list = t->d_gzero = nullptr; t->n_gzero = 0;
    t->d_ws = nullptr; t->ws_cap = 0; t->d_tap = nullptr; t->tap_cap = 0; t->d_status = nullptr; t->d_loss = nullptr; t->fwd_valid = false; t->loss_clear = false;
    t->generation = 0; t->side = nullptr; t->ev_fork = t->ev_join = t->ev_mid = nullptr; t->ev_early = nullptr; t->early_recorded = 0; t->early_first = -1;
    t->d_sq = nullptr; t->sq_pos_cap = 0; t->sq_per_dir = 0; t->bwd_generation = -1; t->stack_disabled = false; memset(&t->sqf, 0, sizeof(t->sqf)); memset(&t->sqb, 0, sizeof(t->sqb));
    qpn_train_knobs_parse(t->knobs);
    memset(&t->slabs, 0, sizeof(t->slabs));
    t->use_gemm = (C > 128 || getenv("QPN_TRAIN_GEMM")) && !getenv("QPN_TRAIN_TILES");
    t->d_gmap = nullptr; t->d_gwp = nullptr; t->d_ctmap = nullptr; t->d_ct = nullptr; memset(&t->gm, 0, sizeof(t->gm));
    if (t->use_gemm && (C % 32 || S % 32 || Q % 32)) { qpn_set_error("the GEMM training path needs n_resch, n_skipch, n_quantize multiples of 32"); delete t; return QPN_EINVAL; }
    TrainParams& p = t->tp;
    const int Ap = (A + 3) / 4 * 4;
    t->hoist = !t->use_gemm && C == 64 && g.U >= 16 && A <= 64 && t->knobs.aux_hoist && t->knobs.persist_fwd && t->knobs.persist_bwd;
    p.hoist = t->hoist ? 1 : 0;
    p.C = C; p.S = S; p.Q = Q; p.A = A; p.Ap = Ap; p.L = L; p.U = g.U;
    p.Kt = t->hoist ? 2 * C : 2 * C + Ap; p.Ktp = (p.Kt + 15) / 16 * 16; p.LC = L * C;
    p.causal_w = g.causal_w; p.causal_b = g.causal_b; p.up_w = g.up_w; p.up_b = g.up_b;
    std::vector<int>& map = t->h_wmap;
    std::vector<std::vector<int>> biases;
    auto add_bias = [&](int n, auto f) { int off = (int)biases.size(); for (int i = 0; i < n; ++i) biases.push_back(f(i)); return off; };
    const int Ktp = p.Ktp;
    int n_adapt = 0;
    for (int l = 0; l < L; ++l) {
        const LayerGeom y = g.layers[l];
        TrLayer& ly = p.layers[l];
        ly.adaptive = y.adaptive; ly.dilation = y.dilation;
        ly.tap_off = y.adaptive ? n_adapt++ : -1;
        auto w1src = [&](int k, int n) -> int64_t {
            const int half = n / C, r = n % C;
            if (k < C) return y.adaptive ? (half ? y.wT : y.wS) + (int64_t)r * C + k : (half ? y.wT : y.wS) + ((int64_t)r * C + k) * 2 + 1;
            if (k < 2 * C) { const int kk = k - C; return y.adaptive ? (half ? y.wTP : y.wSP) + (int64_t)r * C + kk : (half ? y.wT : y.wS) + ((int64_t)r * C + kk) * 2; }
            if (k < 2 * C + A) return (half ? y.auxT : y.auxS) + (int64_t)r * A + (k - 2 * C);
            return -1;
        };
        ly.w1_f4 = frag_pack(map, Ktp, 2 * C, w1src);
        ly.w1t_f4 = frag_pack(map, 2 * C, Ktp, [&](int k, int n) { return w1src(n, k); });
        ly.wr_f4 = frag_pack(map, C, C, [&](int k, int n) { return y.res + (int64_t)n * C + k; });
        ly.wrt_f4 = frag_pack(map, C, C, [&](int k, int n) { return y.res + (int64_t)k * C + n; });
        ly.bias1 = add_bias(2 * C, [&](int n) {
            const int half = n / C, r = n % C;
            std::vector<int> v{(int)((half ? y.bT : y.bS) + r), (int)((half ? y.auxTb : y.auxSb) + r)};
            if (y.adaptive) v.push_back((int)((half ? y.bTP : y.bSP) + r));
            return v; });
        ly.biasr = add_bias(C, [&](int n) { return std::vector<int>{(int)(y.resb + n)}; });
    }
    p.ws_f4 = frag_pack(map, L * C, S, [&](int k, int n) { return g.layers[k / C].skip + (int64_t)n * C + (k % C); });
    p.wst_f4 = frag_pack(map, S, L * C, [&](int k, int n) { return g.layers[n / C].skip + (int64_t)k * C + (n % C); });
    p.p1_f4 = frag_pack(map, S, S, [&](int k, int n) { return g.post1_w + (int64_t)n * S + k; });
    p.p1t_f4 = frag_pack(map, S, S, [&](int k, int n) { return g.post1_w + (int64_t)k * S + n; });
    p.p2_f4 = frag_pack(map, S, Q, [&](int k, int n) { return g.post2_w + (int64_t)n * S + k; });
    p.p2t_f4 = frag_pack(map, Q, S, [&](int k, int n) { return g.post2_w + (int64_t)k * S + n; });
    p.bias_s = add_bias(S, [&](int n) { std::vector<int> v; for (int l = 0; l < L; ++l) v.push_back((int)(g.layers[l].skipb + n)); return v; });
    p.bias_p1 = add_bias(S, [&](int n) { return std::vector<int>{(int)(g.post1_b + n)}; });
    p.bias_p2 = add_bias(Q, [&](int n) { return std::vector<int>{(int)(g.post2_b + n)}; });
    if (t->use_gemm) {
        TrainGemm& gm = t->gm;
        std::vector<int>& gmap = t->h_gmap;
        const int Apad = pad_to(Ap, 32);
        gm.K1 = 2 * C + Apad; gm.N1g = pad_to(C, 64) * 2; gm.Cg = pad_to(C, 128); gm.Sg = pad_to(S, 128); gm.Qg = pad_to(Q, 128);
        gm.LCg = pad_to(L * C, 128); gm.Ktg = pad_to(2 * C + Ap, 128);
        for (int l = 0; l < L; ++l) {
            const LayerGeom y = g.layers[l];
            auto w1src = [&](int k, int n) -> int64_t {
                const int half = n / C, r = n % C;
                if (k < C) return y.adaptive ? (half ? y.wT : y.wS) + (int64_t)r * C + k : (half ? y.wT : y.wS) + ((int64_t)r * C + k) * 2 + 1;
                if (k < 2 * C) { const int kk = k - C; return y.adaptive ? (half ? y.wTP : y.wSP) + (int64_t)r * C + kk : (half ? y.wT : y.wS) + ((int64_t)r * C + kk) * 2; }
                if (k < 2 * C + A) return (half ? y.auxT : y.auxS) + (int64_t)r * A + (k - 2 * C);
                return -1;
            };
            gm.w1[l] = kmajor_pack(gmap, 2 * C + A, gm.K1, gm.N1g, gm.N1g, [&](int k, int q) -> int64_t {
                const int tile = q / 128, w = q % 128, half = w / 64, c = 64 * tile + w % 64;
                return c < C ? w1src(k, half * C + c) : -1; });
            gm.w1t[l] = kmajor_pack(gmap, 2 * C, 2 * C, 2 * C + A, gm.Ktg, [&](int k, int n) { return w1src(n, k); });
            gm.wr[l] = kmajor_pack(gmap, C, C, C, gm.Cg, [&](int k, int n) { return y.res + (int64_t)n * C + k; });
            gm.wrt[l] = kmajor_pack(gmap, C, C, C, gm.Cg, [&](int k, int n) { return y.res + (int64_t)k * C + n; });
        }
        gm.ws = kmajor_pack(gmap, L * C, L * C, S, gm.Sg, [&](int k, int n) { return g.layers[k / C].skip + (int64_t)n * C + (k % C); });
        gm.wst = kmajor_pack(gmap, S, S, L * C, gm.LCg, [&](int k, int n) { return g.layers[n / C].skip + (int64_t)k * C + (n % C); });
        gm.p1 = kmajor_pack(gmap, S, S, S, gm.Sg, [&](int k, int n) { return g.post1_w + (int64_t)n * S + k; });
        gm.p1t = kmajor_pack(gmap, S, S, S, gm.Sg, [&](int k, int n) { return g.post1_w + (int64_t)k * S + n; });
        gm.p2 = kmajor_pack(gmap, S, S, Q, gm.Qg, [&](int k, int n) { return g.post2_w + (int64_t)n * S + k; });
        gm.p2t = kmajor_pack(gmap, Q, Q, S, gm.Sg, [&](int k, int n) { return g.post2_w + (int64_t)k * S + n; });
    }
    memset(&t->ag, 0, sizeof(t->ag));
    for (int l = 0; l < L; ++l) { t->ag.auxS[l] = (int)g.layers[l].auxS; t->ag.auxT[l] = (int)g.layers[l].auxT; t->ag.bias1[l] = p.layers[l].bias1; }
    t->n_bias = (int)biases.size();
    t->h_bstart.assign(1, 0);
    for (auto& v : biases) { for (int x : v) t->h_blist.push_back(x); t->h_bstart.push_back((int)t->h_blist.size()); }

    TrainBwd& bw = t->bw;
    TrainSlabs& sl = t->slabs;
    bw.sl = &t->slabs;
    int go = 0;
    auto gtake = [&](int n) { int r = go; go += (n + 63) & ~63; return r; };
    std::vector<int>& gs = t->h_gsrc;
    gs.assign(g.n_params, -1);
    for (int l = 0; l < L; ++l) {
        sl.g_w1[l] = gtake(2 * C * Ktp);
        sl.g_b1[l] = gtake(2 * C);
        sl.g_wr[l] = gtake(C * C);
        sl.g_br[l] = gtake(C);
    }
    sl.g_early0 = go;
    for (int l = 0; l < L; ++l) sl.g_ws[l] = gtake(S * C);
    for (int l = 0; l < L; ++l) {
        const LayerGeom y = g.layers[l];
        for (int n = 0; n < 2 * C; ++n) {
            const int half = n / C, r = n % C;
            if (t->hoist) for (int a = 0; a < A; ++a) gs[(half ? y.auxT : y.auxS) + (int64_t)r * A + a] = -2;
            for (int k = 0; k < (t->hoist ? 2 * C : 2 * C + A); ++k) {
                int64_t dst;
                if (k < C) dst = y.adaptive ? (half ? y.wT : y.wS) + (int64_t)r * C + k : (half ? y.wT : y.wS) + ((int64_t)r * C + k) * 2 + 1;
                else if (k < 2 * C) { const int kk = k - C; dst = y.adaptive ? (half ? y.wTP : y.wSP) + (int64_t)r * C + kk : (half ? y.wT : y.wS) + ((int64_t)r * C + kk) * 2; }
                else dst = (half ? y.auxT : y.auxS) + (int64_t)r * A + (k - 2 * C);
                gs[dst] = sl.g_w1[l] + n * Ktp + k;
            }
            gs[(half ? y.bT : y.bS) + r] = sl.g_b1[l] + n;
            gs[(half ? y.auxTb : y.auxSb) + r] = sl.g_b1[l] + n;
            if (y.adaptive) gs[(half ? y.bTP : y.bSP) + r] = sl.g_b1[l] + n;
        }
        for (int o = 0; o < C; ++o) { for (int c = 0; c < C; ++c) gs[y.res + (int64_t)o * C + c] = sl.g_wr[l] + o * C + c; gs[y.resb + o] = sl.g_br[l] + o; }
        for (int s = 0; s < S; ++s) for (int c = 0; c < C; ++c) gs[y.skip + (int64_t)s * C + c] = sl.g_ws[l] + s * C + c;
    }
    sl.g_bs = gtake(S);
    for (int l = 0; l < L; ++l) for (int s = 0; s < S; ++s) gs[g.layers[l].skipb + s] = sl.g_bs + s;
    sl.g_p1 = gtake(S * S); sl.g_bp1 = gtake(S); sl.g_p2 = gtake(Q * S); sl.g_bp2 = gtake(Q);
    sl.g_early1 = go;
    t->early_first = (g.post1_b == g.post1_w + (int64_t)S * S && g.post2_w == g.post1_b + S && g.post2_b == g.post2_w + (int64_t)Q * S && g.post2_b + Q == g.n_params) ? g.post1_w : -1;
    for (int o = 0; o < S; ++o) { for (int s = 0; s < S; ++s) gs[g.post1_w + (int64_t)o * S + s] = sl.g_p1 + o * S + s; gs[g.post1_b + o] = sl.g_bp1 + o; }
    for (int q = 0; q < Q; ++q) { for (int s = 0; s < S; ++s) gs[g.post2_w + (int64_t)q * S + s] = sl.g_p2 + q * S + s; gs[g.post2_b + q] = sl.g_bp2 + q; }
    sl.g_cw = sl.g_cb = -1;
    if (C == 64 && Q % 128 == 0 && !t->use_gemm) {
        sl.g_cw = gtake(2 * C * Q); sl.g_cb = gtake(C);
        for (int c = 0; c < C; ++c) {
            for (int q = 0; q < Q; ++q) for (int tp = 0; tp < 2; ++tp) gs[g.causal_w + ((int64_t)c * Q + q) * 2 + tp] = sl.g_cw + tp * C * Q + c * Q + q;
            gs[g.causal_b + c] = sl.g_cb + c;
        }
    }
    bw.gstage = go; bw.nch = t->use_gemm ? 4 : 64; bw.n_params = g.n_params;
    if (t->knobs.wgrad_chunks > 0) bw.nch = t->knobs.wgrad_chunks;
    if (t->hoist) for (int j = 0; j < g.U; ++j) gs[g.up_w + j] = -2;

    const size_t nmap = t->use_gemm ? 4 : map.size();
    QPN_HIP(hipMalloc(&t->d_wmap, nmap * sizeof(int)));
    QPN_HIP(hipMalloc(&t->d_wp, nmap * sizeof(float)));
    QPN_HIP(hipMalloc(&t->d_bstart, t->h_bstart.size() * sizeof(int)));
    QPN_HIP(hipMalloc(&t->d_blist, t->h_blist.size() * sizeof(int)));
    QPN_HIP(hipMalloc(&t->d_bp, (size_t)t->n_bias * sizeof(float)));
    QPN_HIP(hipMalloc(&t->d_status, 64));
    QPN_HIP(hipMemset(t->d_status, 0, 64));
    t->last_stream = nullptr;
    t->h_status_pinned = nullptr; t->ev_status[0] = t->ev_status[1] = nullptr; t->status_pending[0] = t->status_pending[1] = false; t->status_newest = 0;
    QPN_HIP(hipHostMalloc((void**)&t->h_status_pinned, 64, hipHostMallocDefault));
    t->h_loss_pinned = nullptr; t->ev_loss[0] = t->ev_loss[1] = nullptr; t->loss_pending[0] = t->loss_pending[1] = false; t->loss_newest = 0;
    QPN_HIP(hipHostMalloc((void**)&t->h_loss_pinned, 2 * LOSS_SLOT * sizeof(double), hipHostMallocDefault));
    t->d_gnorm = nullptr; t->gnorm_last = false; t->gnorm_slot[0] = t->gnorm_slot[1] = false; t->gnorm_collected = 0.0; t->gnorm_collected_valid = false;
    QPN_HIP(hipMalloc(&t->d_gnorm, TR_GN_BLOCKS * sizeof(double)));
    QPN_HIP(hipMemset(t->d_gnorm, 0, TR_GN_BLOCKS * sizeof(double)));
    QPN_HIP(hipEventCreateWithFlags(&t->ev_loss[0], hipEventDisableTiming));
    QPN_HIP(hipEventCreateWithFlags(&t->ev_loss[1], hipEventDisableTiming));
    QPN_HIP(hipEventCreateWithFlags(&t->ev_status[0], hipEventDisableTiming));
    QPN_HIP(hipEventCreateWithFlags(&t->ev_status[1], hipEventDisableTiming));
    QPN_HIP(hipMalloc(&t->d_loss, LOSS_SLOT * sizeof(double)));
    QPN_HIP(hipMemset(t->d_loss, 0, LOSS_SLOT * sizeof(double)));
    if (!t->use_gemm) QPN_HIP(hipMemcpy(t->d_wmap, map.data(), nmap * sizeof(int), hipMemcpyHostToDevice));
    QPN_HIP(hipMemcpy(t->d_bstart, t->h_bstart.data(), t->h_bstart.size() * sizeof(int), hipMemcpyHostToDevice));
    QPN_HIP(hipMemcpy(t->d_blist, t->h_blist.data(), t->h_blist.size() * sizeof(int), hipMemcpyHostToDevice));
    {
        std::vector<int> start((size_t)go + 1, 0), list, gz;
        for (int64_t i = 0; i < g.n_params; ++i) { if (gs[i] >= 0) ++start[(size_t)gs[i] + 1]; else if (gs[i] == -1) gz.push_back((int)i); }
        for (int k = 0; k < go; ++k) start[(size_t)k + 1] += start[k];
        list.resize((size_t)start[go] + 1);
        std::vector<int> fill(start.begin(), start.end() - 1);
        for (int64_t i = 0; i < g.n_params; ++i) if (gs[i] >= 0) list[(size_t)fill[gs[i]]++] = (int)i;
        QPN_HIP(hipMalloc(&t->d_gdst, start.size() * sizeof(int)));
        QPN_HIP(hipMemcpy(t->d_gdst, start.data(), start.size() * sizeof(int), hipMemcpyHostToDevice));
        QPN_HIP(hipMalloc(&t->d_gdst_list, list.size() * sizeof(int)));
        QPN_HIP(hipMemcpy(t->d_gdst_list, list.data(), list.size() * sizeof(int), hipMemcpyHostToDevice));
        t->n_gzero = (int)gz.size();
        QPN_HIP(hipMalloc(&t->d_gzero, (gz.size() + 1) * sizeof(int)));
        if (!gz.empty()) QPN_HIP(hipMemcpy(t->d_gzero, gz.data(), gz.size() * sizeof(int), hipMemcpyHostToDevice));
    }
    if (t->use_gemm) {
        QPN_HIP(hipMalloc(&t->d_gmap, t->h_gmap.size() * sizeof(int)));
        QPN_HIP(hipMalloc(&t->d_gwp, t->h_gmap.size() * sizeof(float)));
        QPN_HIP(hipMemcpy(t->d_gmap, t->h_gmap.data(), t->h_gmap.size() * sizeof(int), hipMemcpyHostToDevice));
        t->gm.wp = t->d_gwp;
        std::vector<int>().swap(t->h_wmap);
    }
    {
        std::vector<int> ctm((size_t)2 * Q * C);
        for (int tp = 0; tp < 2; ++tp) for (int q = 0; q < Q; ++q) for (int c = 0; c < C; ++c)
            ctm[((size_t)tp * Q + q) * C + c] = (int)(g.causal_w + ((int64_t)c * Q + q) * 2 + tp);
        QPN_HIP(hipMalloc(&t->d_ctmap, ctm.size() * sizeof(int)));
        QPN_HIP(hipMalloc(&t->d_ct, ctm.size() * sizeof(float)));
        QPN_HIP(hipMemcpy(t->d_ctmap, ctm.data(), ctm.size() * sizeof(int), hipMemcpyHostToDevice));
    }
    QPN_HIP(hipStreamCreateWithFlags(&t->side, hipStreamNonBlocking));
    const unsigned evf = hipEventDisableTiming | (t->knobs.event_fence ? 0u : (unsigned)hipEventDisableSystemFence);
    QPN_HIP(hipEventCreateWithFlags(&t->ev_fork, evf));
    QPN_HIP(hipEventCreateWithFlags(&t->ev_join, evf));
    QPN_HIP(hipEventCreateWithFlags(&t->ev_mid, evf));
    QPN_HIP(hipEventCreateWithFlags(&t->ev_early, evf));
    h->train = t;
    return QPN_OK;
}

void qpn_train_destroy(TrainState* t) {
    if (!t) return;
    void* bufs[] = {t->d_wmap, t->d_wp, t->d_bstart, t->d_blist, t->d_bp, t->d_gdst, t->d_gdst_list, t->d_gzero, t->d_ws, t->d_tap, t->d_status, t->d_loss, t->d_gmap, t->d_gwp, t->d_ctmap, t->d_ct, t->d_sq, t->d_gnorm};
    for (void* b : bufs) if (b) (void)hipFree(b);
    if (t->h_status_pinned) (void)hipHostFree(t->h_status_pinned);
    if (t->h_loss_pinned) (void)hipHostFree(t->h_loss_pinned);
    for (int i = 0; i < 2; ++i) if (t->ev_loss[i]) (void)hipEventDestroy(t->ev_loss[i]);
    for (int i = 0; i < 2; ++i) if (t->ev_status[i]) (void)hipEventDestroy(t->ev_status[i]);
    if (t->side) (void)hipStreamDestroy(t->side);
    if (t->ev_fork) (void)hipEventDestroy(t->ev_fork);
    if (t->ev_join) (void)hipEventDestroy(t->ev_join);
    if (t->ev_mid) (void)hipEventDestroy(t->ev_mid);
    if (t->ev_early) (void)hipEventDestroy(t->ev_early);
    delete t;
}

static int need_dev(qpn_handle* h) {
    if (!h) { qpn_set_error("null handle"); return QPN_EINVAL; }
    if (h->device < 0) { qpn_set_error("no HIP device: libqpnet_hip has no CPU fallback"); return QPN_ENODEV; }
    return QPN_OK;
}

static int train_forward_impl(qpn_handle* h, const float* d_flat, int B, int64_t T, int64_t F, int64_t Td, int BL, int maxd,
                              const int64_t* d_x, const float* d_h, const float* d_dfac, float* d_logits,
                              const int64_t* d_targets, int64_t tgt_stride, float* d_dlogits, int want_logits, void* stream_, bool fuse_bwd = false) {
    int rc = need_dev(h); if (rc) return rc;
    rc = train_init(h); if (rc) return rc;
    TrainState* t = h->train;
    hipStream_t stream = (hipStream_t)stream_;
    const Geom& g = h->g;
    if (!d_flat || !d_x || !d_h || !d_dfac || !d_logits || B < 1 || BL < 1 || maxd < 1) { qpn_set_error("bad train_forward arguments"); return QPN_EINVAL; }
    if (d_targets && tgt_stride < BL) { qpn_set_error("bad train_forward_loss arguments: target rows shorter than batch_length"); return QPN_EINVAL; }
    const int64_t N0 = (int64_t)g.recA * maxd + g.recF + 1 + BL;
    if (N0 > T || N0 - 1 > Td || N0 - 1 > (g.U > 0 ? F * g.U : F)) {
        qpn_set_error("chunk too short: need receptive field (%lld) + batch_length (%d) = %lld samples, have x:%lld d:%lld h_up:%lld",
                      (long long)(N0 - BL), BL, (long long)N0, (long long)T, (long long)Td, (long long)(g.U > 0 ? F * g.U : F));
        return QPN_EINVAL;
    }
    if (T >= ((int64_t)1 << 31) || Td >= ((int64_t)1 << 31) || F * (g.U > 0 ? g.U : 1) >= ((int64_t)1 << 31) || (int64_t)B * N0 >= ((int64_t)1 << 31)) {
        qpn_set_error("chunk too long: the training kernels index rows with 32 bits"); return QPN_EINVAL;
    }
    TrainParams& p = t->tp;
    p.B = B; p.T = (int)T; p.F = (int)F; p.Td = (int)Td; p.BL = BL; p.N0 = (int)N0; p.N1 = (int)N0 - 1; p.maxd = maxd;
    const int C = g.C, S = g.S, L = g.L, N1 = p.N1;
    int s = 0, nA = 0;
    for (int l = 0; l < L; ++l) {
        TrLayer& ly = p.layers[l];
        ly.s_in = s; s += ly.adaptive ? ly.dilation * maxd : ly.dilation; ly.s_out = s;
        ly.tap_off = (nA++) * B * N1;
        t->ag.s_out[l] = ly.s_out;
    }
    if (t->hoist) {
        if (N1 >= (1 << 24)) { qpn_set_error("chunk too long for the register-resident layer kernels (%d rows; QPN_AUX_HOIST=0 QPN_LAYER_PERSIST=0 QPN_LAYER_BWD_PERSIST=0 selects the tile-per-workgroup kernels)", N1); return QPN_EINVAL; }
        p.ffirst = (int)(((int64_t)F * g.U - N1) / g.U); p.nfr = (int)F - p.ffirst;
    } else { p.ffirst = 0; p.nfr = 0; }
    const size_t nPA = t->hoist ? (size_t)L * B * (p.nfr + 1) * 2 * C : 0, nWJ = t->hoist ? (size_t)2 * (N1 + 16) : 0, nGW = t->hoist ? (size_t)L * B * N1 : 0;
    const size_t nX = (size_t)(L + 1) * B * N1 * C, nG = (size_t)L * B * N1 * C, nH = t->hoist ? 64 : (size_t)B * N1 * p.Ap, nS = (size_t)B * BL * S;
    TrainBwd& bw = t->bw;
    const size_t nDX = (size_t)B * N1 * C, nDZ = (size_t)B * N1 * 2 * C, nDGS = (size_t)B * BL * L * C, nSlab = (size_t)bw.nch * bw.gstage;
    const size_t nXC = (size_t)B * (N1 + 1);
    const size_t nScr = (size_t)B * 1024 * 2 * 128;
    size_t need = nScr + nX + 2 * nG + nH + 2 * (nS + 96 * (size_t)S + 64) + 2 * (size_t)(L + 1) * nDX + (size_t)L * nDZ + 2 * nS + nDGS + nH + nSlab + nXC + (t->use_gemm ? nG : 0) + 2 * nPA + nWJ + nGW + (size_t)L * TR_EB_SLOTS * 2 * C + 8192;
    if (need > t->ws_cap) {
        if (t->d_ws) (void)hipFree(t->d_ws);
        t->d_ws = nullptr; t->ws_cap = 0;
        hipError_t e = hipMalloc(&t->d_ws, need * sizeof(float));
        if (e != hipSuccess) { qpn_set_error("hipMalloc(%zu MiB) for the training workspace failed", need * 4 >> 20); return QPN_ENOMEM; }
        t->ws_cap = need;
    }
    const size_t ntap = (size_t)std::max(nA, 1) * B * N1;
    if (ntap > t->tap_cap) {
        if (t->d_tap) (void)hipFree(t->d_tap);
        t->d_tap = nullptr; t->tap_cap = 0;
        QPN_HIP(hipMalloc(&t->d_tap, ntap * sizeof(int)));
        t->tap_cap = ntap;
    }
    float* w = t->d_ws;
    auto carve = [&](size_t n) { float* r = w; w += (n + 63) & ~(size_t)63; return r; };
    p.X = carve(nX); p.SG = carve(nG); p.TH = carve(nG); p.HUP = carve(nH); p.S0 = carve(nS + 96 * (size_t)S); p.Y0 = carve(nS + 96 * (size_t)S);
    bw.DXA[0] = carve((size_t)(L + 1) * nDX); bw.DXB[0] = carve((size_t)(L + 1) * nDX); bw.DXA[1] = bw.DXB[1] = nullptr;
    bw.DZ = carve((size_t)L * nDZ); bw.DS0 = carve(nS); bw.DY0 = carve(nS); bw.DGS = carve(nDGS); bw.DHUP = carve(nH); bw.slab = carve(nSlab);
    p.XC = (int*)carve(nXC);
    p.scratch_rows = carve(nScr);
    if (t->use_gemm) t->gm.G = carve(nG);
    p.PA = nullptr; p.WJ = nullptr; bw.DPA = nullptr; bw.GW = nullptr;
    bw.EB = nullptr;
    if (t->hoist) { p.PA = carve(nPA); bw.DPA = carve(nPA + (size_t)L * TR_EB_SLOTS * 2 * C); bw.EB = bw.DPA + nPA; p.WJ = (float2*)carve(nWJ); bw.GW = carve(nGW); }
    p.TAP = t->d_tap; p.status = t->d_status;
    t->last_stream = stream;
    {
        qpn_stack_fill(p);
        if ((size_t)p.qtotal > t->sq_pos_cap) {
            if (t->d_sq) (void)hipFree(t->d_sq);
            t->d_sq = nullptr; t->sq_pos_cap = 0;
            const size_t cap = (size_t)p.qtotal + (size_t)p.qtotal / 2 + 64;
            const size_t per_dir = (cap / 32 + 2) * 1056;
            const size_t nsq = TR_QHDR_WORDS + 2 * per_dir + 2 * (cap + 1) * 8;
            QPN_HIP(hipMalloc(&t->d_sq, nsq * sizeof(unsigned)));
            QPN_HIP(hipMemsetAsync(t->d_sq, 0, nsq * sizeof(unsigned), stream));
            t->sq_pos_cap = cap; t->sq_per_dir = per_dir;
        }
        hipStreamCaptureStatus cap_st = hipStreamCaptureStatusNone;
        (void)hipStreamIsCapturing(stream, &cap_st);
        const bool no_queue = t->stack_disabled || cap_st != hipStreamCaptureStatusNone;
        p.qctl = no_queue ? nullptr : t->d_sq;
        p.qtab = no_queue ? nullptr : (int4*)(t->d_sq + TR_QHDR_WORDS + 2 * t->sq_per_dir);
        p.qtab_b = no_queue ? nullptr : p.qtab + 2 * (t->sq_pos_cap + 1);
        const unsigned epoch = (unsigned)((t->generation + 1) % 0xFFFFFFFFll) + 1u;
        StackQ& f = t->sqf; StackQ& bq = t->sqb;
        f.flags = t->d_sq + TR_QHDR_WORDS; f.head = t->d_sq + 1024; f.abort = t->d_sq + 1; f.stats = t->d_sq + 4; f.epoch = epoch; f.total = p.qtotal; f.tab = p.qtab;
        bq.flags = f.flags + t->sq_per_dir; bq.head = f.head + 8 * TR_QHEAD_STRIDE; bq.abort = f.abort; bq.stats = t->d_sq + 8; bq.epoch = epoch; bq.total = p.qtotal; bq.tab = p.qtab_b;
    }
    p.flat = d_flat; p.wp = (const float4*)t->d_wp; p.bp = t->d_bp; p.x = d_x; p.h = d_h; p.d = d_dfac; p.logits = d_logits;
    {
        const int* wmap = t->use_gemm ? t->d_gmap : t->d_wmap;
        float* wout = t->use_gemm ? t->d_gwp : t->d_wp;
        const int64_t nw = (int64_t)(t->use_gemm ? t->h_gmap.size() : t->h_wmap.size()), nct = (int64_t)2 * g.Q * g.C;
        const int64_t tot = nw + nct + t->n_bias + 16 + 64;
        hipLaunchKernelGGL(k_refresh, dim3((unsigned)((tot + 255) / 256)), dim3(256), 0, stream, d_flat, wmap, wout, nw, t->d_ctmap, t->d_ct, nct,
                           t->d_bstart, t->d_blist, t->d_bp, t->n_bias, t->d_status, t->d_loss);
        p.ct = t->d_ct;
    }
    qpn_prof_mark(PG_PREP, stream);
    t->fwd_valid = false; t->loss_clear = true;
    ++t->generation;
    const bool fuse_ce = d_targets && !t->use_gemm && g.Q <= g.S && g.Q % 256 == 0 && !t->knobs.ce_separate;
    p.ce_tgt = fuse_ce ? d_targets : nullptr; p.ce_stride = tgt_stride; p.ce_dlogits = d_dlogits; p.ce_loss = t->d_loss;
    if (fuse_ce && !want_logits) p.logits = nullptr;
    const bool fuse_post = fuse_bwd && fuse_ce && d_dlogits && t->knobs.post_fuse && t->knobs.post_wide && t->knobs.zero_in_post && g.S == 256 && g.Q == 256 && g.C == 64 && (p.LC == 256 || p.LC == 512);
    t->post_bwd_done = false;
    rc = t->use_gemm ? qpn_launch_fwd_gemm(p, t->gm, stream) : qpn_launch_fwd(p, t->knobs, t->ag, &t->sqf, stream, fuse_post ? &t->bw : nullptr);
    if (!rc) { t->post_bwd_done = fuse_post; t->post_bwd_dlogits = d_dlogits; }
    p.ce_tgt = nullptr; p.logits = d_logits;
    if (rc) return rc;
    t->fwd_valid = true;
    if (fuse_ce) { t->loss_clear = false; qpn_prof_mark(PG_CE, stream); }
    else if (d_targets) {
        rc = qpn_launch_ce(d_logits, d_targets, tgt_stride, B, BL, g.Q, d_dlogits, t->d_loss, t->d_status, t->loss_clear, stream); if (rc) return rc;
        t->loss_clear = false;
    }
    return QPN_OK;
}

extern "C" int qpn_train_forward(qpn_handle* h, const float* d_flat, int B, int64_t T, int64_t F, int64_t Td, int BL, int maxd,
                                 const int64_t* d_x, const float* d_h, const float* d_dfac, float* d_logits, void* stream_) {
    return train_forward_impl(h, d_flat, B, T, F, Td, BL, maxd, d_x, d_h, d_dfac, d_logits, nullptr, 0, nullptr, 1, stream_);
}

extern "C" int qpn_train_forward_loss(qpn_handle* h, const float* d_flat, int B, int64_t T, int64_t F, int64_t Td, int BL, int maxd,
                                      const int64_t* d_x, const float* d_h, const float* d_dfac, const int64_t* d_targets, int64_t tgt_stride,
                                      float* d_logits, int want_logits, float* d_dlogits, void* stream_) {
    if (!d_targets) { qpn_set_error("bad train_forward_loss arguments: no targets"); return QPN_EINVAL; }
    return train_forward_impl(h, d_flat, B, T, F, Td, BL, maxd, d_x, d_h, d_dfac, d_logits, d_targets, tgt_stride, d_dlogits, want_logits & 1, stream_, (want_logits & QPN_FWD_BACKWARD_FOLLOWS) != 0);
}

extern "C" int qpn_train_loss(qpn_handle* h, double* h_loss, void* stream_) {
    int rc = need_dev(h); if (rc) return rc;
    if (!h->train || !h_loss) { qpn_set_error("qpn_train_loss needs a preceding qpn_train_forward_loss / qpn_ce_loss"); return QPN_ESTATE; }
    hipStream_t stream = (hipStream_t)stream_;
    double parts[64];
    QPN_HIP(hipMemcpyAsync(parts, h->train->d_loss, sizeof(parts), hipMemcpyDeviceToHost, stream));
    QPN_HIP(hipStreamSynchronize(stream));
    double sum = 0.0;
    for (int i = 0; i < 64; ++i) sum += parts[i];
    *h_loss = sum;
    return QPN_OK;
}

extern "C" int qpn_train_loss_enqueue(qpn_handle* h, void* stream_) {
    int rc = need_dev(h); if (rc) return rc;
    if (!h->train) { qpn_set_error("qpn_train_loss_enqueue needs a preceding qpn_train_forward_loss / qpn_ce_loss"); return QPN_ESTATE; }
    TrainState* t = h->train;
    const int slot = t->loss_newest ^ 1;
    if (t->loss_pending[slot]) QPN_HIP(hipEventSynchronize(t->ev_loss[slot]));
    QPN_HIP(hipMemcpyAsync(t->h_loss_pinned + LOSS_SLOT * slot, t->d_loss, (t->gnorm_last ? 65 : 64) * sizeof(double), hipMemcpyDeviceToHost, (hipStream_t)stream_));
    t->gnorm_slot[slot] = t->gnorm_last;
    QPN_HIP(hipEventRecord(t->ev_loss[slot], (hipStream_t)stream_));
    t->loss_pending[slot] = true; t->loss_newest = slot;
    return QPN_OK;
}
extern "C" int qpn_train_loss_collect(qpn_handle* h, int newest, double* h_loss, int* h_valid) {
    int rc = need_dev(h); if (rc) return rc;
    if (!h_loss || !h_valid) { qpn_set_error("bad loss_collect arguments"); return QPN_EINVAL; }
    *h_valid = 0; *h_loss = 0.0;
    if (!h->train) return QPN_OK;
    TrainState* t = h->train;
    const int slot = newest ? t->loss_newest : t->loss_newest ^ 1;
    t->gnorm_collected_valid = false;
    if (!t->loss_pending[slot]) return QPN_OK;
    QPN_HIP(hipEventSynchronize(t->ev_loss[slot]));
    t->loss_pending[slot] = false;
    double sum = 0.0;
    for (int i = 0; i < 64; ++i) sum += t->h_loss_pinned[LOSS_SLOT * slot + i];
    *h_loss = sum; *h_valid = 1;
    if (t->gnorm_slot[slot]) { t->gnorm_collected = t->h_loss_pinned[LOSS_SLOT * slot + 64]; t->gnorm_collected_valid = true; }
    return QPN_OK;
}

static int status_to_rc(int st);
extern "C" int qpn_train_status(qpn_handle* h, void* stream_) {
    int rc = need_dev(h); if (rc) return rc;
    if (!h->train) { qpn_set_error("no training call yet"); return QPN_ESTATE; }
    QPN_HIP(hipStreamSynchronize((hipStream_t)stream_));
    int st = 0;
    QPN_HIP(hipMemcpy(&st, h->train->d_status, sizeof(int), hipMemcpyDeviceToHost));
    if (st) QPN_HIP(hipMemsetAsync(h->train->d_status, 0, sizeof(int), (hipStream_t)stream_));
    h->train->last_stream = (hipStream_t)stream_;
    if (st & 4) h->train->stack_disabled = true;
    h->train->status_pending[0] = h->train->status_pending[1] = false;
    return status_to_rc(st);
}

static int status_to_rc(int st) {
    if (st & 1) { qpn_set_error("pitch-dependent tap outside the layer input (dilated factor > maxd or < 0; reference assert qpnet.py:294)"); return QPN_ERANGE; }
    if (st & 4) { qpn_set_error("the one-launch residual stack gave up waiting for a peer workgroup: the flagged step's results are invalid (its Adam update, and that of the steps enqueued behind it until this report, were skipped on the device: parameters and moments are those of the last clean step); the handle runs a launch per layer from here on (QPN_STACK_QUEUE=0 selects that from the start)"); return QPN_ENODEV; }
    if (st & 2) { qpn_set_error("target class outside [0, n_quantize) (reference assert qpnet_train.py:525)"); return QPN_ERANGE; }
    if (st & (1 << 16)) { qpn_set_error("non-finite gradient norm (an inf or NaN in the gradient): the step's Adam update, and that of the steps enqueued behind it until this report, were skipped on the device: parameters and moments are those of the last clean step"); return QPN_ERANGE; }
    if (st & 8) { qpn_set_error("a peer rank flagged its chunk of this data-parallel step (a tap or target out of range, or an abandoned stack launch there): every rank skipped the update, the replicas are unchanged"); return QPN_ERANGE; }
    return QPN_OK;
}

static int status_collect_slot(TrainState* t, int slot) {
    if (!t->status_pending[slot]) return QPN_OK;
    QPN_HIP(hipEventSynchronize(t->ev_status[slot]));
    t->status_pending[slot] = false;
    const int st = t->h_status_pinned[slot];
    if (st & 4) t->stack_disabled = true;
    if (st) {
        QPN_HIP(hipMemsetAsync(t->d_status, 0, sizeof(int), t->last_stream));
        const int other = slot ^ 1;
        if (t->status_pending[other]) {
            QPN_HIP(hipEventSynchronize(t->ev_status[other]));
            t->h_status_pinned[other] &= ~st;
            if (!t->h_status_pinned[other]) t->status_pending[other] = false;
        }
    }
    return status_to_rc(st);
}
extern "C" int qpn_train_status_enqueue(qpn_handle* h, void* stream_) {
    int rc = need_dev(h); if (rc) return rc;
    if (!h->train) { qpn_set_error("no training call yet"); return QPN_ESTATE; }
    TrainState* t = h->train;
    const int slot = t->status_newest ^ 1;
    t->last_stream = (hipStream_t)stream_;
    rc = status_collect_slot(t, slot); if (rc) return rc;
    QPN_HIP(hipMemcpyAsync(t->h_status_pinned + slot, t->d_status, sizeof(int), hipMemcpyDeviceToHost, (hipStream_t)stream_));
    QPN_HIP(hipEventRecord(t->ev_status[slot], (hipStream_t)stream_));
    t->status_pending[slot] = true; t->status_newest = slot;
    return QPN_OK;
}
extern "C" int qpn_train_status_collect(qpn_handle* h) {
    int rc = need_dev(h); if (rc) return rc;
    if (!h->train) return QPN_OK;
    TrainState* t = h->train;
    rc = status_collect_slot(t, t->status_newest ^ 1); if (rc) return rc;
    return status_collect_slot(t, t->status_newest);
}
extern "C" int qpn_train_status_poll(qpn_handle* h, int* pending) {
    int rc = need_dev(h); if (rc) return rc;
    if (pending) *pending = 0;
    if (!h->train) return QPN_OK;
    TrainState* t = h->train;
    for (int k = 0; k < 2; ++k) {
        const int slot = k == 0 ? t->status_newest ^ 1 : t->status_newest;
        if (!t->status_pending[slot]) continue;
// ... 197 lines not shown
```

### qpnet_amd/csrc/train_stack.hip

```cpp
#include "train_common.h"

typedef unsigned u32x4 __attribute__((ext_vector_type(4)));
#ifndef SQ_EXP
#define SQ_EXP 0
#endif
#if SQ_EXP & 2
#define SQ_SC1 0
#else
#define SQ_SC1 16
#endif
#define SQ_OOB 0x80000000u
#define SQ_SPIN_LIMIT (1u << 22)
#define SQ_FLINE 1056u
#define SQ_NQ 8

__device__ __forceinline__ unsigned sq_ld(const unsigned* p) { return __hip_atomic_load(p, __ATOMIC_RELAXED, __HIP_MEMORY_SCOPE_AGENT); }
__device__ __forceinline__ void sq_st(unsigned* p, unsigned v) { __hip_atomic_store(p, v, __ATOMIC_RELAXED, __HIP_MEMORY_SCOPE_AGENT); }
__device__ __forceinline__ int sq_rfl(int v) { return __builtin_amdgcn_readfirstlane(v); }
__device__ __forceinline__ float sq_sigmoid(float z) { return __builtin_amdgcn_rcpf(1.0f + __expf(-z)); }
__device__ __forceinline__ float sq_tanh(float z) { return 2.0f * __builtin_amdgcn_rcpf(1.0f + __expf(-2.0f * z)) - 1.0f; }

#ifdef QPN_STACK_STAMPS
#define SQ_STAMP(i) do { __builtin_amdgcn_sched_barrier(0); unsigned long long t_; asm volatile("s_memtime %0\n\ts_waitcnt lgkmcnt(0)" : "=s"(t_) :: "memory"); \
    __builtin_amdgcn_sched_barrier(0); if (blockIdx.x == 5 && tid == 0 && it < 25) q.stats[596 + 8 * it + (i)] = (unsigned)t_; __builtin_amdgcn_sched_barrier(0); } while (0)
#else
#define SQ_STAMP(i) do { } while (0)
#endif
#ifdef QPN_STACK_STAMPS_BWD
#define SQ_STAMPB(i) do { __builtin_amdgcn_sched_barrier(0); unsigned long long t_; asm volatile("s_memtime %0\n\ts_waitcnt lgkmcnt(0)" : "=s"(t_) :: "memory"); \
    __builtin_amdgcn_sched_barrier(0); if (blockIdx.x == 5 && tid == 0 && it < 25) q.stats[592 + 8 * it + (i)] = (unsigned)t_; __builtin_amdgcn_sched_barrier(0); } while (0)
#else
#define SQ_STAMPB(i) do { } while (0)
#endif

__host__ __device__ __forceinline__ static unsigned sq_fidx(unsigned pos) { return (pos >> 5) * SQ_FLINE + (pos & 31u); }

#ifdef SQ_NOPRIO
#define SQ_PRIO(x) do { } while (0)
#else
#define SQ_PRIO(x) __builtin_amdgcn_s_setprio(x)
#endif

struct SqTile { int n0, meta, dfirst, dn, xrow, tapb, hrow, dgs, pos; };
__device__ __forceinline__ bool sq_valid(const SqTile& d) { return (d.meta >> 25) & 1; }
__device__ __forceinline__ bool sq_last(const SqTile& d) { return (d.meta >> 24) & 1; }
__device__ __forceinline__ int sq_layer(const SqTile& d) { return d.meta & 255; }

struct SqRaw { int4 a, b; int pos; };
__device__ __forceinline__ SqRaw sq_fetch(const StackQ& q, int pos) {
    const int i = (pos >= 0 && pos < q.total) ? pos : q.total;
    SqRaw r; r.a = q.tab[2 * i]; r.b = q.tab[2 * i + 1]; r.pos = i;
    return r;
}
__device__ __forceinline__ SqTile sq_take(const SqRaw& r) {
    SqTile d;
    d.n0 = sq_rfl(r.a.x); d.meta = sq_rfl(r.a.y); d.dfirst = sq_rfl(r.a.z); d.dn = sq_rfl(r.a.w);
    d.xrow = sq_rfl(r.b.x); d.tapb = sq_rfl(r.b.y); d.hrow = sq_rfl(r.b.z); d.dgs = sq_rfl(r.b.w); d.pos = r.pos;
    return d;
}

__device__ __forceinline__ int sq_wait(const StackQ& q, int first, int n, int lane, int* status, unsigned bound) {
    unsigned total_spins = 0;
    int rc = 1;
    for (int base = 0; base < n && rc == 1; base += 64) {
        const int i = base + lane < n ? base + lane : n - 1;
        const unsigned* fp = q.flags + sq_fidx((unsigned)(first + i));
        unsigned spins = 0;
        for (;;) {
            const unsigned v = sq_ld(fp);
            if (__all(v == q.epoch)) break;
            ++total_spins;
            if ((spins & 63u) == 63u && sq_ld(q.abort)) { rc = 0; break; }
            ++spins;
            if (bound && spins >= bound) { rc = 2; break; }
            if (spins > q.spin_limit) {
#ifdef QPN_STACK_DEBUG
                if (sq_ld(q.abort) == 0u) { const unsigned long long miss = __ballot(v != q.epoch); if (lane == 0) { q.stats[24] = (unsigned)first; q.stats[25] = (unsigned)n; q.stats[26] = (unsigned)base; q.stats[27] = (unsigned)miss; q.stats[28] = (unsigned)(miss >> 32); q.stats[29] = blockIdx.x; q.stats[30] = q.epoch; } if (lane == (int)__ffsll(miss) - 1) q.stats[31] = v; }
#endif
                if (lane == 0) { sq_st(q.abort, 1u); atomicOr(status, 4); } rc = 0; break; }
            if (spins > 2) __builtin_amdgcn_s_sleep(8);
        }
    }
    if (total_spins && lane == 0) atomicAdd(q.stats + 1, total_spins);
    return rc;
}

template <int KS>
__global__ __launch_bounds__(256, 2) void k_stack_fwd(TrainParams p, StackQ q) {
    constexpr int C = 64, Ktp = 16 * KS;
    constexpr bool HOIST = KS == 8;
    constexpr int lda = ((Ktp + 29) / 32) * 32 + 2, ldg = ((C + 29) / 32) * 32 + 2;
    extern __shared__ float sm[];
    float* Gs = sm + 32 * lda;
    float* SGs = Gs + 16 * ldg; float* THs = SGs + 16 * ldg; float* Xs = THs + 16 * ldg;
    int* ctl = (int*)(Xs + 16 * ldg);
    const int Ap = p.Ap, N1 = p.N1;
    const int tid = threadIdx.x, lane = tid & 63, wave = sq_rfl(tid >> 6);
    const int srow = tid >> 4, sc4 = tid & 15;
    const bool aux_thread = sc4 < (Ktp - 2 * C) / 4, aux_real = 4 * sc4 < Ap;
    const int orow = tid >> 5, oc2 = (tid & 31) * 2;
    const int c = 16 * wave + (lane & 15);
    const int arow = lane & 15, ak = lane >> 4;
    float* const dmy = p.scratch_rows + (size_t)blockIdx.x * 2 * C + oc2;
    const unsigned xbytes = (unsigned)N1 * C * 4u;
    const size_t xlayer = (size_t)p.B * N1 * C;

    float4 w1[KS][2], wr[4];
    float bs = 0.f, bt = 0.f, bb = 0.f;
    auto load_weights = [&](int l) {
        const TrLayer ly = p.layers[l];
        const float4* W1 = p.wp + ly.w1_f4; const float4* Wr = p.wp + ly.wr_f4;
#pragma unroll
        for (int ks = 0; ks < KS; ++ks) { w1[ks][0] = W1[((size_t)ks * 8 + wave) * 64 + lane]; w1[ks][1] = W1[((size_t)ks * 8 + 4 + wave) * 64 + lane]; }
#pragma unroll
        for (int ks = 0; ks < 4; ++ks) wr[ks] = Wr[((size_t)ks * 4 + wave) * 64 + lane];
        bs = p.bp[ly.bias1 + c]; bt = p.bp[ly.bias1 + C + c]; bb = p.bp[ly.biasr + c];
        __builtin_amdgcn_s_waitcnt(0x0F70);
    };
    auto xrsrc = [&](const float* base) { return __builtin_amdgcn_make_buffer_rsrc((void*)base, 0, xbytes, 0x00020000); };
    int tp = 0; float4 rc, rp, rx = make_float4(0.f, 0.f, 0.f, 0.f);
    float2 rwj = make_float2(0.f, 0.f); float rpb0 = 0.f, rpb1 = 0.f, xaux_a = 0.f, xaux_b0 = 0.f, xaux_b1 = 0.f;
    auto load_tap = [&](const SqTile& d, int& out) {
        const int n = d.n0 + srow;
        out = (p.TAP + d.tapb)[n < N1 ? n : N1 - 1];
    };
    auto load_rows = [&](const SqTile& d, bool go) {
        const int n = d.n0 + srow, nn = n < N1 ? n : N1 - 1;
        const auto rs = xrsrc(p.X + (size_t)d.xrow * C);
        const unsigned oc = go ? (__umul24((unsigned)nn, (unsigned)C) + 4u * sc4) * 4u : SQ_OOB;
        const unsigned op = go ? (__umul24((unsigned)tp, (unsigned)C) + 4u * sc4) * 4u : SQ_OOB;
        const u32x4 a = __builtin_amdgcn_raw_buffer_load_b128(rs, (int)oc, 0, SQ_SC1);
        const u32x4 b4 = __builtin_amdgcn_raw_buffer_load_b128(rs, (int)op, 0, SQ_SC1);
        rc = make_float4(__uint_as_float(a.x), __uint_as_float(a.y), __uint_as_float(a.z), __uint_as_float(a.w));
        rp = make_float4(__uint_as_float(b4.x), __uint_as_float(b4.y), __uint_as_float(b4.z), __uint_as_float(b4.w));
        if constexpr (HOIST) {
            const float* pa = p.PA + d.hrow + ((lane >> 4) & 1) * 2 * C + 16 * wave + (lane & 15);
            rwj = p.WJ[d.n0 + (lane & 15)];
            rpb0 = pa[0]; rpb1 = pa[C];
        } else rx = *(const float4*)(p.HUP + (size_t)d.hrow * Ap + (__umul24((unsigned)nn, (unsigned)Ap) + (aux_real ? 4u * sc4 : 0u)));
        __builtin_amdgcn_sched_barrier(0);
    };
    auto store_rows = [&](const SqTile& d, float* As) {
        if constexpr (HOIST) asm volatile("" : "+v"(rpb1)); else asm volatile("" : "+v"(rx.w));
        const bool in = d.n0 + srow < N1;
        const float4 z = make_float4(0.f, 0.f, 0.f, 0.f);
        const float4 vc = in ? rc : z, vp = in ? rp : z, vx = (in && aux_real) ? rx : z;
        float* dd = As + (size_t)srow * lda + 4 * sc4;
        *(float2*)dd = make_float2(vc.x, vc.y); *(float2*)(dd + 2) = make_float2(vc.z, vc.w);
        *(float2*)(dd + C) = make_float2(vp.x, vp.y); *(float2*)(dd + C + 2) = make_float2(vp.z, vp.w);
        if constexpr (HOIST) { xaux_a = tr_aux_a(rwj, lane); xaux_b0 = lane < 32 ? rpb0 : 0.f; xaux_b1 = lane < 32 ? rpb1 : 0.f; }
        else if (aux_thread) { *(float2*)(dd + 2 * C) = make_float2(vx.x, vx.y); *(float2*)(dd + 2 * C + 2) = make_float2(vx.z, vx.w); }
    };
    auto store_out = [&](const float* T, float* dst, int n0) {
        const float2 v0 = *(const float2*)(T + (size_t)orow * ldg + oc2), v1 = *(const float2*)(T + (size_t)(orow + 8) * ldg + oc2);
        float* d0 = dst + (__umul24((unsigned)(n0 + orow), (unsigned)C) + oc2);
        float* d1 = d0 + 8 * C;
        d0 = n0 + orow < N1 ? d0 : dmy;
        d1 = n0 + orow + 8 < N1 ? d1 : dmy + C;
        *(float2*)d0 = v0; *(float2*)d1 = v1;
    };
    u32x4 xkeep = {0u, 0u, 0u, 0u};
    auto store_x = [&](const SqTile& d, bool go) {
        const float2 v0 = *(const float2*)(Xs + (size_t)srow * ldg + 4 * sc4), v1 = *(const float2*)(Xs + (size_t)srow * ldg + 4 * sc4 + 2);
        const int n = d.n0 + srow;
        const unsigned o = (go && n < N1) ? (__umul24((unsigned)n, (unsigned)C) + 4u * sc4) * 4u : SQ_OOB;
        const u32x4 v = {__float_as_uint(v0.x), __float_as_uint(v0.y), __float_as_uint(v1.x), __float_as_uint(v1.y)};
        __builtin_amdgcn_raw_buffer_store_b128(v, xrsrc(p.X + (size_t)d.xrow * C + xlayer), (int)o, 0, SQ_SC1);
        xkeep = v;
    };
    auto publishes = [&](const SqTile& d) { return sq_valid(d) && !sq_last(d); };

    int zero_v; asm volatile("v_mov_b32 %0, 0" : "=v"(zero_v));
    const int NQ = q.nq, sub = (blockIdx.x / 8) % NQ;
    unsigned* const head = q.head + sub * TR_QHEAD_STRIDE + zero_v;
    if (tid == 0) {
        ctl[8] = 0;
        const unsigned k0 = atomicAdd(head, 1u); ctl[0] = (int)(k0 * NQ + sub);
        asm volatile("" ::: "memory");
        const unsigned k1 = atomicAdd(head, 1u); ctl[1] = (int)(k1 * NQ + sub);
        asm volatile("" ::: "memory");
        const unsigned k2 = atomicAdd(head, 1u); ctl[2] = (int)(k2 * NQ + sub);
    }
    __syncthreads();
    SqTile cur = sq_take(sq_fetch(q, sq_rfl(ctl[0]))), next = sq_take(sq_fetch(q, sq_rfl(ctl[1]))), nn = sq_take(sq_fetch(q, sq_rfl(ctl[2])));
    if (!sq_valid(cur)) return;
    SqTile prev = cur; prev.meta = 0;
    int lw = sq_layer(cur);
    load_weights(lw);
    load_tap(cur, tp);
    sq_wait(q, cur.dfirst, cur.dn, lane, p.status, 0u);
    load_rows(cur, true);
    store_rows(cur, sm);
    load_tap(next, tp);
    bool cur_published = false;
    for (int it = 0;; ++it) {
        float* As = sm + (it & 1) * 16 * lda;
        const bool last = sq_last(cur);
        SQ_STAMP(0);
        unsigned rtk = 0;
// ... 18 lines not shown
#pragma unroll
        for (int ks = 0; ks < KS; ++ks) {
            a0 = __builtin_amdgcn_mfma_f32_16x16x4f32(xa[ks][0], w1[ks][0].x, a0, 0, 0, 0); a1 = __builtin_amdgcn_mfma_f32_16x16x4f32(xa[ks][0], w1[ks][1].x, a1, 0, 0, 0);
            a0 = __builtin_amdgcn_mfma_f32_16x16x4f32(xa[ks][1], w1[ks][0].y, a0, 0, 0, 0); a1 = __builtin_amdgcn_mfma_f32_16x16x4f32(xa[ks][1], w1[ks][1].y, a1, 0, 0, 0);
            a0 = __builtin_amdgcn_mfma_f32_16x16x4f32(xa[ks][2], w1[ks][0].z, a0, 0, 0, 0); a1 = __builtin_amdgcn_mfma_f32_16x16x4f32(xa[ks][2], w1[ks][1].z, a1, 0, 0, 0);
            a0 = __builtin_amdgcn_mfma_f32_16x16x4f32(xa[ks][3], w1[ks][0].w, a0, 0, 0, 0); a1 = __builtin_amdgcn_mfma_f32_16x16x4f32(xa[ks][3], w1[ks][1].w, a1, 0, 0, 0);
        }
        SQ_PRIO(2);
        __builtin_amdgcn_sched_barrier(0);
        SQ_STAMP(2);
        __builtin_amdgcn_s_waitcnt(0x0F71);
        asm volatile("" :: "v"(xkeep));
        if (lane == 0) {
            const int old = __hip_atomic_fetch_add(ctl + 8, 1, __ATOMIC_RELAXED, __HIP_MEMORY_SCOPE_WORKGROUP);
            if ((old & 3) == 3 && pub_prev) sq_st(q.flags + sq_fidx((unsigned)prev.pos), q.epoch_pub);
        }
        __builtin_amdgcn_sched_barrier(0);
        SQ_STAMP(3);
#pragma unroll
        for (int i = 0; i < 4; ++i) {
            const int o = (4 * (lane >> 4) + i) * ldg + c;
            const float sg = sq_sigmoid(a0[i] + bs), th = sq_tanh(a1[i] + bt);
            Gs[o] = sg * th; SGs[o] = sg;
        }
        SQ_STAMP(4);
        if (tid == 0) ctl[(it + 3) & 3] = (int)(rtk * NQ + sub);
        TR_LDS_BARRIER();
        SQ_STAMP(5);
        const SqRaw raw3 = sq_fetch(q, sq_rfl(ctl[(it + 3) & 3]));
        const int fn = next.dn, fnm1 = fn > 0 ? fn - 1 : 0, fbase = fn > 0 ? next.dfirst : cur.pos;
        unsigned fv0 = sq_ld(q.flags + sq_fidx((unsigned)(fbase + (lane < fnm1 ? lane : fnm1)))), fv1 = sq_ld(q.flags + sq_fidx((unsigned)(fbase + (lane + 64 < fnm1 ? lane + 64 : fnm1))));
        asm volatile("" ::: "memory");
        float* SG = p.SG + (size_t)cur.xrow * C;
        float* TH = p.TH + (size_t)cur.xrow * C;
        if (!last) {
            float ga[4][4];
#pragma unroll
            for (int ks = 0; ks < 4; ++ks) {
                const float* gp = Gs + (size_t)arow * ldg + 16 * ks + ak;
                ga[ks][0] = gp[0]; ga[ks][1] = gp[4]; ga[ks][2] = gp[8]; ga[ks][3] = gp[12];
            }
            __builtin_amdgcn_sched_barrier(0);
            SQ_PRIO(0);
            f32x4 ar0 = (f32x4){0, 0, 0, 0}, ar1 = (f32x4){0, 0, 0, 0};
#pragma unroll
            for (int ks = 0; ks < 4; ks += 2) {
                ar0 = __builtin_amdgcn_mfma_f32_16x16x4f32(ga[ks][0], wr[ks].x, ar0, 0, 0, 0); ar1 = __builtin_amdgcn_mfma_f32_16x16x4f32(ga[ks + 1][0], wr[ks + 1].x, ar1, 0, 0, 0);
                ar0 = __builtin_amdgcn_mfma_f32_16x16x4f32(ga[ks][1], wr[ks].y, ar0, 0, 0, 0); ar1 = __builtin_amdgcn_mfma_f32_16x16x4f32(ga[ks + 1][1], wr[ks + 1].y, ar1, 0, 0, 0);
                ar0 = __builtin_amdgcn_mfma_f32_16x16x4f32(ga[ks][2], wr[ks].z, ar0, 0, 0, 0); ar1 = __builtin_amdgcn_mfma_f32_16x16x4f32(ga[ks + 1][2], wr[ks + 1].z, ar1, 0, 0, 0);
                ar0 = __builtin_amdgcn_mfma_f32_16x16x4f32(ga[ks][3], wr[ks].w, ar0, 0, 0, 0); ar1 = __builtin_amdgcn_mfma_f32_16x16x4f32(ga[ks + 1][3], wr[ks + 1].w, ar1, 0, 0, 0);
            }
            SQ_PRIO(2);
#pragma unroll
            for (int i = 0; i < 4; ++i) {
                const int r = 4 * (lane >> 4) + i;
                Xs[r * ldg + c] = ((ar0[i] + ar1[i]) + bb) + As[(size_t)r * lda + c];
            }
        }
        SQ_STAMP(6);
        asm volatile("" : "+v"(fv0), "+v"(fv1));
        bool ready = fn == 0 || (fn <= 128 && __all(fv0 == q.epoch && fv1 == q.epoch));
#if SQ_EXP & 512
        ready = true;
#endif
        asm volatile("" ::: "memory");
#if !(SQ_EXP & 64)
        store_out(SGs, SG, cur.n0);
        store_out(Gs, TH, cur.n0);
#endif
        if (lane == 0) ctl[4 + wave] = ready ? 0 : 1;
        TR_LDS_BARRIER();
        int any_slow = sq_rfl(ctl[4] | ctl[5] | ctl[6] | ctl[7]);
        cur_published = false;
        if (any_slow) {
            if (tid == 0) atomicAdd(q.stats + 2, 1u);
            if (!ready) {
                const unsigned g0 = sq_ld(q.flags + sq_fidx((unsigned)(fbase + (lane < fnm1 ? lane : fnm1)))), g1 = sq_ld(q.flags + sq_fidx((unsigned)(fbase + (lane + 64 < fnm1 ? lane + 64 : fnm1))));
                ready = fn <= 128 && __all(g0 == q.epoch && g1 == q.epoch);
            }
            if (lane == 0) ctl[12 + wave] = ready ? 0 : 1;
            TR_LDS_BARRIER();
            any_slow = sq_rfl(ctl[12] | ctl[13] | ctl[14] | ctl[15]);
        }
        if (any_slow) {
            if (tid == 0) atomicAdd(q.stats, 1u);
            store_x(cur, publishes(cur));
            asm volatile("s_waitcnt vmcnt(0)" ::: "memory");
            TR_LDS_BARRIER();
            if (tid == 0 && publishes(cur)) sq_st(q.flags + sq_fidx((unsigned)cur.pos), q.epoch_pub);
            cur_published = true;
            if (!ready) sq_wait(q, next.dfirst, next.dn, lane, p.status, 0u);
        }
#if SQ_EXP & 256
        rc = rp = rx = make_float4(0.25f, 0.5f, 0.125f, 0.75f); rwj = make_float2(0.5f, 0.f); rpb0 = rpb1 = 0.25f;
#else
        load_rows(next, true);
#endif
#if !(SQ_EXP & 128)
        store_x(cur, publishes(cur) && !any_slow);
#endif
        store_rows(next, sm + ((it + 1) & 1) * 16 * lda);
        SQ_STAMP(7);
        tp = tpn;
        prev = cur; cur = next; next = nn; nn = sq_take(raw3);
        if (!sq_valid(cur)) break;
    }
    asm volatile("s_waitcnt vmcnt(0)" ::: "memory");
    TR_LDS_BARRIER();
    if (tid == 0 && publishes(prev) && !cur_published) sq_st(q.flags + sq_fidx((unsigned)prev.pos), q.epoch_pub);
}

template <int NTK>
__global__ __launch_bounds__(256, 2) void k_stack_bwd(TrainParams p, TrainBwd bw, StackQ q) {
    constexpr int C = 64;
    constexpr int ldx = ((C + 29) / 32) * 32 + 2, ldz = ((2 * C + 29) / 32) * 32 + 2, ldo = ((16 * NTK + 29) / 32) * 32 + 2;
    constexpr int NJ = (NTK + 3) / 4;
    constexpr bool HOIST = NTK == 8;
    extern __shared__ float sm[];
    float* Dz = sm + 8 * 16 * ldx;
    float* Os = Dz + 16 * ldz;
    int* ctl = (int*)(Os + 16 * ldo);
    float* Gp = (float*)(ctl + 32);
    const int Ap = p.Ap, N1 = p.N1;
    const int tid = threadIdx.x, lane = tid & 63, wave = sq_rfl(tid >> 6);
    const int srow = tid >> 4, sc4 = tid & 15;
    const int zrow = tid >> 6, zc2 = (tid & 63) * 2;
    const int arow = lane & 15, ak = lane >> 4;
    const int c = 16 * wave + (lane & 15);
    const int win0 = N1 - p.BL;
    const unsigned xbytes = (unsigned)N1 * C * 4u;
    const size_t nDX = (size_t)p.B * N1 * C;
    float* const dmy = p.scratch_rows + (size_t)blockIdx.x * 2 * 128;

    float4 wr[4], w1[NJ][8];
    auto load_weights = [&](int l, bool last) {
        const TrLayer ly = p.layers[l];
        const float4* Wrt = p.wp + ly.wrt_f4; const float4* W1t = p.wp + ly.w1t_f4;
#pragma unroll
        for (int ks = 0; ks < 4; ++ks) { const float4 v = Wrt[((size_t)ks * 4 + wave) * 64 + lane]; wr[ks] = last ? make_float4(0.f, 0.f, 0.f, 0.f) : v; }
#pragma unroll
        for (int j = 0; j < NJ; ++j) {
            const int nt = wave + 4 * j < NTK ? wave + 4 * j : NTK - 1;
#pragma unroll
            for (int ks = 0; ks < 8; ++ks) w1[j][ks] = W1t[((size_t)ks * NTK + nt) * 64 + lane];
        }
        static_assert(NJ == 3 || NJ == 2, "the operand lists below name every float4 of wr / w1");
        asm volatile("" :: "v"(wr[0].w), "v"(wr[1].w), "v"(wr[2].w), "v"(wr[3].w),
                     "v"(w1[0][0].w), "v"(w1[0][1].w), "v"(w1[0][2].w), "v"(w1[0][3].w), "v"(w1[0][4].w), "v"(w1[0][5].w), "v"(w1[0][6].w), "v"(w1[0][7].w),
                     "v"(w1[1][0].w), "v"(w1[1][1].w), "v"(w1[1][2].w), "v"(w1[1][3].w), "v"(w1[1][4].w), "v"(w1[1][5].w), "v"(w1[1][6].w), "v"(w1[1][7].w));
        if constexpr (NJ == 3)
            asm volatile("" :: "v"(w1[NJ - 1][0].w), "v"(w1[NJ - 1][1].w), "v"(w1[NJ - 1][2].w), "v"(w1[NJ - 1][3].w), "v"(w1[NJ - 1][4].w), "v"(w1[NJ - 1][5].w), "v"(w1[NJ - 1][6].w), "v"(w1[NJ - 1][7].w));
    };
    auto rsrc = [&](const float* base) { return __builtin_amdgcn_make_buffer_rsrc((void*)base, 0, xbytes, 0x00020000); };
    float4 ra, rb2, rsg, rth, rdg;
    auto row_off = [&](const SqTile& d) { const int n = d.n0 + srow, nn_ = n < N1 ? n : N1 - 1; return __umul24((unsigned)nn_, (unsigned)C) + 4u * sc4; };
    auto load_own = [&](const SqTile& d) {
        const unsigned o = row_off(d);
        const int n = d.n0 + srow, nn_ = n < N1 ? n : N1 - 1;
        rsg = *(const float4*)(p.SG + (size_t)d.xrow * C + o); rth = *(const float4*)(p.TH + (size_t)d.xrow * C + o);
        const int nw = nn_ >= win0 ? nn_ - win0 : 0;
        rdg = *(const float4*)(bw.DGS + (size_t)d.dgs + (__umul24((unsigned)nw, (unsigned)p.LC) + 4u * sc4));
    };
    auto load_ab = [&](const SqTile& d, float4& a4, float4& b4_) {
        const unsigned ob = sq_last(d) ? SQ_OOB : row_off(d) * 4u;
        const u32x4 a = __builtin_amdgcn_raw_buffer_load_b128(rsrc(bw.DXA[0] + (size_t)d.xrow * C + nDX), (int)ob, 0, SQ_SC1);
        const u32x4 b4 = __builtin_amdgcn_raw_buffer_load_b128(rsrc(bw.DXB[0] + (size_t)d.xrow * C + nDX), (int)ob, 0, SQ_SC1);
        a4 = make_float4(__uint_as_float(a.x), __uint_as_float(a.y), __uint_as_float(a.z), __uint_as_float(a.w));
        b4_ = make_float4(__uint_as_float(b4.x), __uint_as_float(b4.y), __uint_as_float(b4.z), __uint_as_float(b4.w));
    };
    auto store_own = [&](const SqTile& d, float* B) {
        const int n = d.n0 + srow;
        const bool in = n < N1;
        const float4 z = make_float4(0.f, 0.f, 0.f, 0.f);
        const float4 sg = in ? rsg : z, th = in ? rth : z, dg = (in && n >= win0) ? rdg : z;
        float* d1 = B + (size_t)(16 + srow) * ldx + 4 * sc4; *(float2*)d1 = make_float2(sg.x, sg.y); *(float2*)(d1 + 2) = make_float2(sg.z, sg.w);
        float* d2 = d1 + 16 * ldx; *(float2*)d2 = make_float2(th.x, th.y); *(float2*)(d2 + 2) = make_float2(th.z, th.w);
        float* d3 = d2 + 16 * ldx; *(float2*)d3 = make_float2(dg.x, dg.y); *(float2*)(d3 + 2) = make_float2(dg.z, dg.w);
    };
    auto store_dx = [&](const SqTile& d, float* B, const float4& a4, const float4& b4_) {
        const int n = d.n0 + srow;
        const bool in = n < N1 && !sq_last(d);
        const float4 dx = in ? make_float4(a4.x + b4_.x, a4.y + b4_.y, a4.z + b4_.z, a4.w + b4_.w) : make_float4(0.f, 0.f, 0.f, 0.f);
        float* d0 = B + (size_t)srow * ldx + 4 * sc4;
        *(float2*)d0 = make_float2(dx.x, dx.y); *(float2*)(d0 + 2) = make_float2(dx.z, dx.w);
        if (in) *(float4*)(bw.DXA[0] + (size_t)d.xrow * C + nDX + row_off(d)) = dx;
    };
    float2 cwj[4], nwj[4]; float cpa[4], npa[4]; float dacc[4] = {0.f, 0.f, 0.f, 0.f};
    float eacc[2] = {0.f, 0.f};
    auto load_aux = [&](const SqTile& d, float2 (&wj)[4], float (&pa)[4]) {
        const float2* w = p.WJ + d.n0 + 4 * (lane >> 4);
        const float* q4 = p.PA + d.hrow + 16 * wave + (lane & 15);
#pragma unroll
        for (int i = 0; i < 4; ++i) wj[i] = w[i];
        pa[0] = q4[0]; pa[1] = q4[C]; pa[2] = q4[2 * C]; pa[3] = q4[3 * C];
    };
    int tprow[4];
    auto load_taps = [&](const SqTile& d, int (&tp)[4]) {
#pragma unroll
        for (int i = 0; i < 4; ++i) { const int n = d.n0 + 4 * wave + i; tp[i] = (p.TAP + d.tapb)[n < N1 ? n : N1 - 1]; }
    };
    auto outputs = [&](const SqTile& d, const float* Dx) {
        const bool adaptive = (d.meta >> 26) & 1;
        const int dil = p.layers[sq_layer(d)].dilation;
#if !(SQ_EXP & 16)
        {
            const int n = d.n0 + srow;
            const float2 o0 = *(const float2*)(Os + (size_t)srow * ldo + 4 * sc4), o1 = *(const float2*)(Os + (size_t)srow * ldo + 4 * sc4 + 2);
            const float2 x0 = *(const float2*)(Dx + (size_t)srow * ldx + 4 * sc4), x1 = *(const float2*)(Dx + (size_t)srow * ldx + 4 * sc4 + 2);
            const u32x4 v = {__float_as_uint(o0.x + x0.x), __float_as_uint(o0.y + x0.y), __float_as_uint(o1.x + x1.x), __float_as_uint(o1.y + x1.y)};
            const unsigned off = n < N1 ? (__umul24((unsigned)n, (unsigned)C) + 4u * sc4) * 4u : SQ_OOB;
            __builtin_amdgcn_raw_buffer_store_b128(v, rsrc(bw.DXA[0] + (size_t)d.xrow * C), (int)off, 0, SQ_SC1);
            if (!adaptive) {
                const float2 p0 = *(const float2*)(Os + (size_t)srow * ldo + C + 4 * sc4), p1 = *(const float2*)(Os + (size_t)srow * ldo + C + 4 * sc4 + 2);
                const u32x4 w = {__float_as_uint(p0.x), __float_as_uint(p0.y), __float_as_uint(p1.x), __float_as_uint(p1.y)};
                const int tr = n - dil;
                const unsigned offb = (n < N1 && tr >= 0) ? (__umul24((unsigned)tr, (unsigned)C) + 4u * sc4) * 4u : SQ_OOB;
                __builtin_amdgcn_raw_buffer_store_b128(w, rsrc(bw.DXB[0] + (size_t)d.xrow * C), (int)offb, 0, SQ_SC1);
            }
        }
#endif
        float* DBout = bw.DXB[0] + (size_t)d.xrow * C;
        float* DH = HOIST ? nullptr : bw.DHUP + (size_t)d.hrow * Ap;
#pragma unroll
        for (int i = 0; i < 4; ++i) {
            const int r = 4 * wave + i, n = d.n0 + r;
            const bool in = n < N1;
#if !(SQ_EXP & 1)
            if (adaptive) {
                float* db = DBout + (__umul24((unsigned)tprow[i], (unsigned)C) + lane);
                atomicAdd(in ? db : dmy + 128 + lane, Os[(size_t)r * ldo + C + lane]);
            }
            if constexpr (!HOIST) if (lane < Ap) {
                float* dh = DH + (__umul24((unsigned)n, (unsigned)Ap) + lane);
                atomicAdd(in ? dh : dmy + 192 + lane, Os[(size_t)r * ldo + 2 * C + lane]);
            }
#endif
        }
        if constexpr (HOIST) {
#if !(SQ_EXP & 1)
            if (lane < 16) {
                float* dp = bw.DPA + d.hrow + 16 * wave + lane;
                atomicAdd(dp, dacc[0]); atomicAdd(dp + C, dacc[1]); atomicAdd(dp + 2 * C, dacc[2]); atomicAdd(dp + 3 * C, dacc[3]);
                float* ep = bw.EB + (size_t)(sq_layer(d) * TR_EB_SLOTS + (blockIdx.x & (TR_EB_SLOTS - 1))) * 2 * C + 16 * wave + lane;
                atomicAdd(ep, eacc[0]); atomicAdd(ep + C, eacc[1]);
            }
#endif
            if (tid < 16 && d.n0 + tid < N1) bw.GW[(size_t)d.xrow + d.n0 + tid] = (Gp[tid] + Gp[16 + tid]) + (Gp[32 + tid] + Gp[48 + tid]);
        }
    };
    auto publishes = [&](const SqTile& d) { return sq_valid(d) && sq_layer(d) > 0; };

    int zero_v; asm volatile("v_mov_b32 %0, 0" : "=v"(zero_v));
    const int NQ = q.nq, sub = (blockIdx.x / 8) % NQ;
    unsigned* const head = q.head + sub * TR_QHEAD_STRIDE + zero_v;
    if (tid == 0) {
        ctl[8] = 0;
        const unsigned k0 = atomicAdd(head, 1u); ctl[0] = (int)(k0 * NQ + sub);
        asm volatile("" ::: "memory");
        const unsigned k1 = atomicAdd(head, 1u); ctl[1] = (int)(k1 * NQ + sub);
        asm volatile("" ::: "memory");
        const unsigned k2 = atomicAdd(head, 1u); ctl[16] = (int)(k2 * NQ + sub);
    }
    __syncthreads();
    SqTile cur = sq_take(sq_fetch(q, sq_rfl(ctl[0]))), next = sq_take(sq_fetch(q, sq_rfl(ctl[1])));
    if (!sq_valid(cur)) return;
    SqTile prev = cur; prev.meta = 0;
    int lw = sq_layer(cur);
    load_weights(lw, sq_last(cur));
    sq_wait(q, cur.dfirst, cur.dn, lane, p.status, 0u);
    load_own(cur); load_ab(cur, ra, rb2);
    if constexpr (HOIST) load_aux(cur, cwj, cpa);
    load_taps(cur, tprow);
    store_own(cur, sm); store_dx(cur, sm, ra, rb2);
    bool cur_published = false;
    const __amdgpu_buffer_rsrc_t frs = __builtin_amdgcn_make_buffer_rsrc((void*)q.flags, 0, (int)((sq_fidx((unsigned)q.total) + 64u) * 4u), 0x00020000);
    for (int it = 0;; ++it) {
        float* Dx = sm + (it & 1) * 4 * 16 * ldx; float* Sg = Dx + 16 * ldx; float* Th = Sg + 16 * ldx; float* Dg = Th + 16 * ldx;
        float* Bn = sm + ((it + 1) & 1) * 4 * 16 * ldx;
        const bool last = sq_last(cur);
        if (sq_layer(cur) != lw) { lw = sq_layer(cur); load_weights(lw, last); }
        const bool pub_prev = publishes(prev) && !cur_published;
        SQ_STAMPB(0);
        TR_LDS_BARRIER();
        float xa[4][4];
#pragma unroll
        for (int ks = 0; ks < 4; ++ks) { const float* ap = Dx + (size_t)arow * ldx + 16 * ks + ak; xa[ks][0] = ap[0]; xa[ks][1] = ap[4]; xa[ks][2] = ap[8]; xa[ks][3] = ap[12]; }
        __builtin_amdgcn_sched_barrier(0);
        SQ_PRIO(0);
        f32x4 a0 = (f32x4){0, 0, 0, 0}, a1 = (f32x4){0, 0, 0, 0};
        if (!last) {
#pragma unroll
            for (int ks = 0; ks < 4; ks += 2) {
                a0 = __builtin_amdgcn_mfma_f32_16x16x4f32(xa[ks][0], wr[ks].x, a0, 0, 0, 0); a1 = __builtin_amdgcn_mfma_f32_16x16x4f32(xa[ks + 1][0], wr[ks + 1].x, a1, 0, 0, 0);
                a0 = __builtin_amdgcn_mfma_f32_16x16x4f32(xa[ks][1], wr[ks].y, a0, 0, 0, 0); a1 = __builtin_amdgcn_mfma_f32_16x16x4f32(xa[ks + 1][1], wr[ks + 1].y, a1, 0, 0, 0);
                a0 = __builtin_amdgcn_mfma_f32_16x16x4f32(xa[ks][2], wr[ks].z, a0, 0, 0, 0); a1 = __builtin_amdgcn_mfma_f32_16x16x4f32(xa[ks + 1][2], wr[ks + 1].z, a1, 0, 0, 0);
                a0 = __builtin_amdgcn_mfma_f32_16x16x4f32(xa[ks][3], wr[ks].w, a0, 0, 0, 0); a1 = __builtin_amdgcn_mfma_f32_16x16x4f32(xa[ks + 1][3], wr[ks + 1].w, a1, 0, 0, 0);
            }
        }
        SQ_PRIO(2);
        float dzs[4], dzt[4];
#pragma unroll
        for (int i = 0; i < 4; ++i) {
            const int r = 4 * (lane >> 4) + i;
            const float dg = (a0[i] + a1[i]) + Dg[(size_t)r * ldx + c];
            const float sg = Sg[(size_t)r * ldx + c], th = Th[(size_t)r * ldx + c];
            tr_gate_bwd(dg, sg, th, dzs[i], dzt[i]);
            Dz[(size_t)r * ldz + c] = dzs[i];
            Dz[(size_t)r * ldz + C + c] = dzt[i];
        }
        if constexpr (HOIST) {
            const TrAuxBwd ab = tr_aux_bwd(cwj, cpa, dzs, dzt, lane);
#pragma unroll
            for (int k = 0; k < 4; ++k) dacc[k] = ab.d[k];
            eacc[0] = ab.e[0]; eacc[1] = ab.e[1];
            if ((lane & 15) == 0) { float* gq = Gp + 16 * wave + 4 * (lane >> 4); gq[0] = ab.gp[0]; gq[1] = ab.gp[1]; gq[2] = ab.gp[2]; gq[3] = ab.gp[3]; }
        }
        SQ_STAMPB(1);
        TR_LDS_BARRIER();
        const SqRaw raw2 = sq_fetch(q, sq_rfl(ctl[16 + (it & 1)]));
        const int fn = next.dn, fnm1 = fn > 0 ? fn - 1 : 0, fbase = fn > 0 ? next.dfirst : cur.pos;
        unsigned fv0 = sq_ld(q.flags + sq_fidx((unsigned)(fbase + (lane < fnm1 ? lane : fnm1)))), fv1 = sq_ld(q.flags + sq_fidx((unsigned)(fbase + (lane + 64 < fnm1 ? lane + 64 : fnm1))));
        load_own(next);
        if constexpr (HOIST) load_aux(next, nwj, npa);
        int tpn[4]; load_taps(next, tpn);
        unsigned rtk = 0;
        if (tid == 0) rtk = atomicAdd(head, 1u);
        asm volatile("" ::: "memory");
        float za[8][4];
#pragma unroll
        for (int ks = 0; ks < 8; ++ks) { const float* zp = Dz + (size_t)arow * ldz + 16 * ks + ak; za[ks][0] = zp[0]; za[ks][1] = zp[4]; za[ks][2] = zp[8]; za[ks][3] = zp[12]; }
        __builtin_amdgcn_sched_barrier(0);
        SQ_PRIO(0);
        f32x4 acc[NJ];
#pragma unroll
        for (int j = 0; j < NJ; ++j) acc[j] = (f32x4){0, 0, 0, 0};
#define SQB_MFMA(ks) do { \
            _Pragma("unroll") for (int j = 0; j < NJ; ++j) acc[j] = __builtin_amdgcn_mfma_f32_16x16x4f32(za[ks][0], w1[j][ks].x, acc[j], 0, 0, 0); \
            _Pragma("unroll") for (int j = 0; j < NJ; ++j) acc[j] = __builtin_amdgcn_mfma_f32_16x16x4f32(za[ks][1], w1[j][ks].y, acc[j], 0, 0, 0); \
            _Pragma("unroll") for (int j = 0; j < NJ; ++j) acc[j] = __builtin_amdgcn_mfma_f32_16x16x4f32(za[ks][2], w1[j][ks].z, acc[j], 0, 0, 0); \
            _Pragma("unroll") for (int j = 0; j < NJ; ++j) acc[j] = __builtin_amdgcn_mfma_f32_16x16x4f32(za[ks][3], w1[j][ks].w, acc[j], 0, 0, 0); } while (0)
        SQB_MFMA(0); SQB_MFMA(1); SQB_MFMA(2); SQB_MFMA(3);
        __builtin_amdgcn_sched_barrier(0);
        if constexpr (HOIST) { if (wave == 0) asm volatile("s_waitcnt vmcnt(16)" ::: "memory"); else asm volatile("s_waitcnt vmcnt(15)" ::: "memory"); }
        else { if (wave == 0) asm volatile("s_waitcnt vmcnt(10)" ::: "memory"); else asm volatile("s_waitcnt vmcnt(9)" ::: "memory"); }
        {
            int old = 0;
            if (lane == 0) old = __hip_atomic_fetch_add(ctl + 8, 1, __ATOMIC_RELAXED, __HIP_MEMORY_SCOPE_WORKGROUP);
            const bool pub = pub_prev && (sq_rfl(old) & 3) == 3;
            const unsigned foff = (pub && lane == 0) ? sq_fidx((unsigned)prev.pos) * 4u : SQ_OOB;
            __builtin_amdgcn_raw_buffer_store_b32(q.epoch_pub, frs, (int)foff, 0, SQ_SC1);
        }
        __builtin_amdgcn_sched_barrier(0);
        SQB_MFMA(4); SQB_MFMA(5); SQB_MFMA(6); SQB_MFMA(7);
#undef SQB_MFMA
        SQ_PRIO(2);
        __builtin_amdgcn_sched_barrier(0);
        SQ_STAMPB(2);
        asm volatile("s_waitcnt vmcnt(0)" ::: "memory");
        asm volatile("" : "+v"(fv0), "+v"(fv1), "+v"(rtk), "+v"(tpn[0]), "+v"(tpn[1]), "+v"(tpn[2]), "+v"(tpn[3]));
        if constexpr (HOIST) asm volatile("" : "+v"(nwj[0].x), "+v"(nwj[1].x), "+v"(nwj[2].x), "+v"(nwj[3].x), "+v"(npa[0]), "+v"(npa[1]), "+v"(npa[2]), "+v"(npa[3]));
        SQ_STAMPB(3);
        bool ready = fn == 0 || (fn <= 128 && __all(fv0 == q.epoch && fv1 == q.epoch));
#if SQ_EXP & 32
        ready = true;
#endif
        load_ab(next, ra, rb2);
        store_own(next, Bn);
        const SqTile n2 = sq_take(raw2);
        if (tid == 0) ctl[16 + ((it + 1) & 1)] = (int)(rtk * NQ + sub);
        __builtin_amdgcn_sched_barrier(0);
#pragma unroll
        for (int j = 0; j < NJ; ++j) {
            const int nt = wave + 4 * j;
            if (nt >= NTK) continue;
#pragma unroll
            for (int i = 0; i < 4; ++i) Os[(size_t)(4 * (lane >> 4) + i) * ldo + 16 * nt + (lane & 15)] = acc[j][i];
        }
        SQ_STAMPB(4);
#if !(SQ_EXP & 4)
        {
            float* DZg = bw.DZ + (size_t)cur.xrow * 2 * C;
#pragma unroll
            for (int k = 0; k < 4; ++k) {
                const int r = zrow + 4 * k;
                float* d = DZg + (__umul24((unsigned)(cur.n0 + r), 2u * C) + zc2);
                d = cur.n0 + r < N1 ? d : dmy + zc2;
                *(float2*)d = *(const float2*)(Dz + (size_t)r * ldz + zc2);
            }
        }
#endif
        if (lane == 0) ctl[4 + wave] = ready ? 0 : 1;
        SQ_STAMPB(5);
        TR_LDS_BARRIER();
        SQ_STAMPB(6);
        int any_slow = sq_rfl(ctl[4] | ctl[5] | ctl[6] | ctl[7]);
        const int any_late = any_slow;
        cur_published = false;
        if (any_slow) {
            if (tid == 0) atomicAdd(q.stats + 2, 1u);
            if (!ready) {
                const unsigned g0 = sq_ld(q.flags + sq_fidx((unsigned)(fbase + (lane < fnm1 ? lane : fnm1)))), g1 = sq_ld(q.flags + sq_fidx((unsigned)(fbase + (lane + 64 < fnm1 ? lane + 64 : fnm1))));
                ready = fn <= 128 && __all(g0 == q.epoch && g1 == q.epoch);
            }
            if (lane == 0) ctl[12 + wave] = ready ? 0 : 1;
            TR_LDS_BARRIER();
            any_slow = sq_rfl(ctl[12] | ctl[13] | ctl[14] | ctl[15]);
        }
        asm volatile("" : "+v"(ra.w), "+v"(rb2.w));
        if (any_slow) {
            if (tid == 0) atomicAdd(q.stats, 1u);
            outputs(cur, Dx);
            asm volatile("s_waitcnt vmcnt(0)" ::: "memory");
            TR_LDS_BARRIER();
            if (tid == 0 && publishes(cur)) sq_st(q.flags + sq_fidx((unsigned)cur.pos), q.epoch_pub);
            cur_published = true;
            if (!ready) sq_wait(q, next.dfirst, next.dn, lane, p.status, 0u);
            float4 la, lb; load_ab(next, la, lb);
            store_dx(next, Bn, la, lb);
        } else if (any_late) {
            float4 la, lb; load_ab(next, la, lb);
            store_dx(next, Bn, la, lb);
            outputs(cur, Dx);
        } else {
            store_dx(next, Bn, ra, rb2);
            outputs(cur, Dx);
        }
        SQ_STAMPB(7);
#pragma unroll
        for (int i = 0; i < 4; ++i) tprow[i] = tpn[i];
        if constexpr (HOIST) {
#pragma unroll
            for (int i = 0; i < 4; ++i) { cwj[i] = nwj[i]; cpa[i] = npa[i]; }
        }
        prev = cur; cur = next; next = n2;
        if (!sq_valid(cur)) break;
    }
    asm volatile("s_waitcnt vmcnt(0)" ::: "memory");
    TR_LDS_BARRIER();
    if (tid == 0 && publishes(prev) && !cur_published) sq_st(q.flags + sq_fidx((unsigned)prev.pos), q.epoch_pub);
}

static void sq_arm(StackQ& q, const TrainKnobs& k) {
    q.epoch_pub = q.epoch; q.spin_limit = SQ_SPIN_LIMIT;
#ifdef QPN_TESTING
    if (k.test_stack_gives_up) { q.epoch_pub = q.epoch ^ 0x55555555u; q.spin_limit = 2000u; }
#else
    (void)k;
#endif
}
bool qpn_stack_fwd_fits(const TrainParams& p) {
    return p.C == 64 && (p.hoist ? p.Ktp == 128 : p.Ktp == 176) && p.L >= 1 && p.L <= TR_MAXL && p.B < 65536 && (int64_t)p.N1 * p.C * 4 <= (1ll << 30) &&
           (int64_t)(p.L + 1) * p.B * p.N1 < (1ll << 31);
}

void qpn_stack_fill(TrainParams& p) {
    int pos = 0;
    for (int l = 0; l < p.L; ++l) {
        p.qT[l] = (p.N1 - p.layers[l].s_out + 15) / 16;
        p.qP[l] = pos; pos += p.B * p.qT[l];
    }
    for (int l = p.L; l <= TR_MAXL; ++l) p.qP[l] = pos;
    p.qtotal = pos;
}

template <int KS>
static int launch_stack_fwd_k(const TrainParams& p, const StackQ& q, const TrainKnobs& k, hipStream_t stream) {
    constexpr int lda = ((16 * KS + 29) / 32) * 32 + 2, ldg = ((64 + 29) / 32) * 32 + 2;
    const size_t lds = (size_t)(32 * lda + 4 * 16 * ldg) * sizeof(float) + 64;
    int G = k.stack_wgs > 0 ? k.stack_wgs : qpn_num_cus() * 2;
    if (G > q.total) G = q.total;
    if (G > 1024) G = 1024;
    QPN_HIP(hipFuncSetAttribute((const void*)k_stack_fwd<KS>, hipFuncAttributeMaxDynamicSharedMemorySize, (int)lds));
    StackQ qq = q; qq.nq = G / 8 < 1 ? 1 : (G / 8 < SQ_NQ ? G / 8 : SQ_NQ);
    sq_arm(qq, k);
    hipLaunchKernelGGL((k_stack_fwd<KS>), dim3(G), dim3(256), lds, stream, p, qq);
    return QPN_OK;
}
int qpn_launch_stack_fwd(const TrainParams& p, const StackQ& q, const TrainKnobs& k, hipStream_t stream) {
    return p.hoist ? launch_stack_fwd_k<8>(p, q, k, stream) : launch_stack_fwd_k<11>(p, q, k, stream);
}

bool qpn_stack_bwd_fits(const TrainParams& p) {
    return qpn_stack_fwd_fits(p) && p.Ap <= 64 && (int64_t)p.B * p.BL * p.LC < (1ll << 31) && (int64_t)p.N1 * (p.LC > 2 * p.C ? p.LC : 2 * p.C) < (1ll << 32);
}

template <int NTK>
static int launch_stack_bwd_k(const TrainParams& p, const TrainBwd& bw, const StackQ& q, const TrainKnobs& k, hipStream_t stream) {
    constexpr int ldx = ((64 + 29) / 32) * 32 + 2, ldz = ((128 + 29) / 32) * 32 + 2, ldo = ((16 * NTK + 29) / 32) * 32 + 2;
    const size_t lds = (size_t)(8 * 16 * ldx + 16 * ldz + 16 * ldo) * sizeof(float) + 128 + 256;
    int G = k.stack_wgs_bwd > 0 ? k.stack_wgs_bwd : (NTK == 8 ? qpn_num_cus() * 5 / 4 / 64 * 64 : qpn_num_cus() * 3 / 2);
    if (G < 8) G = qpn_num_cus();
    if (G > q.total) G = q.total;
    if (G > 1024) G = 1024;
    QPN_HIP(hipFuncSetAttribute((const void*)k_stack_bwd<NTK>, hipFuncAttributeMaxDynamicSharedMemorySize, (int)lds));
    StackQ qq = q; qq.nq = G / 8 < 1 ? 1 : (G / 8 < SQ_NQ ? G / 8 : SQ_NQ);
    sq_arm(qq, k);
    hipLaunchKernelGGL((k_stack_bwd<NTK>), dim3(G), dim3(256), lds, stream, p, bw, qq);
    return QPN_OK;
}
int qpn_launch_stack_bwd(const TrainParams& p, const TrainBwd& bw, const StackQ& q, const TrainKnobs& k, hipStream_t stream) {
    return p.hoist ? launch_stack_bwd_k<8>(p, bw, q, k, stream) : launch_stack_bwd_k<11>(p, bw, q, k, stream);
}
```

Measured before the change: 1475 steps/s.

## Gather adaptive-tap gradients via inverse tap map instead of scatter atomics

For adaptive layers after the first, the backward stack no longer scatters tap-branch gradients with per-lane atomicAdd into the previous layer's DXB rows. The forward pass builds an inverse tap map with atomicMin. Each tile now stores its tap gradient to a private DPT buffer, and the consumer tile gathers it back with an extra buffer load. Rows with several contributors ('late' rows) fall back to the atomic path and are zeroed in the zero-dx kernel. The change adds a workspace buffer, extra inverse-map arrays, an extra load per tile and more bookkeeping.

```diff
diff --git a/qpnet_amd/csrc/train_bwd.hip b/qpnet_amd/csrc/train_bwd.hip
--- a/qpnet_amd/csrc/train_bwd.hip
+++ b/qpnet_amd/csrc/train_bwd.hip
@@ -1207,17 +1207,32 @@
     float* A = bw.DXA[0] + (size_t)j * nDX + (size_t)b * p.N1 * C;
     float* Bq = bw.DXB[0] + (size_t)j * nDX + (size_t)b * p.N1 * C;
     const int a0 = j == 0 ? 0 : ly.s_in, a1 = ly.s_out;
-    const int b0 = ly.adaptive ? 0 : p.N1 - ly.dilation, b1 = p.N1;
+    const bool gather = bw.tap_gather && ly.adaptive && j > 0;
+    const int b0 = ly.adaptive ? (gather ? p.N1 : 0) : p.N1 - ly.dilation, b1 = p.N1;
+    const size_t ng = gather ? (size_t)(p.N1 - ly.s_out) : 0;
     const size_t na = (size_t)(a1 - a0) * C / 4, nb = (size_t)(b1 > b0 ? b1 - b0 : 0) * C / 4;
     const float4 z = make_float4(0.f, 0.f, 0.f, 0.f);
     const size_t nh = p.hoist ? (size_t)(p.nfr + 1) * 2 * C / 4 : (j == 0 ? (size_t)p.N1 * p.Ap / 4 : 0);
     const size_t ne = (p.hoist && b == 0) ? (size_t)TR_EB_SLOTS * 2 * C / 4 : 0;
     float* H = p.hoist ? bw.DPA + (size_t)(j * p.B + b) * (p.nfr + 1) * 2 * C : bw.DHUP + (size_t)b * p.N1 * p.Ap;
-    for (size_t i = part * nthr + t; i < na + nb + nh + ne; i += nparts * nthr) {
+    for (size_t i = part * nthr + t; i < na + nb + nh + ne + ng; i += nparts * nthr) {
         if (i < na) ((float4*)(A + (size_t)a0 * C))[i] = z;
         else if (i < na + nb) ((float4*)(Bq + (size_t)(b0 > 0 ? b0 : 0) * C))[i - na] = z;
         else if (i < na + nb + nh) ((float4*)H)[i - na - nb] = z;
-        else ((float4*)(bw.EB + (size_t)j * TR_EB_SLOTS * 2 * C))[i - na - nb - nh] = z;
+        else if (i < na + nb + nh + ne) ((float4*)(bw.EB + (size_t)j * TR_EB_SLOTS * 2 * C))[i - na - nb - nh] = z;
+        else {
+            const int n = ly.s_out + (int)(i - na - nb - nh - ne);
+            const size_t e = (size_t)ly.tap_off + (size_t)b * p.N1;
+            const int tp = p.TAP[e + n];
+            const bool late = (p.INV[e + tp] & 0x7FFFFFFFu) != (unsigned)n;
+            p.TAPB[e + n] = late ? (int)((unsigned)tp | 0x80000000u) : tp;
+            if (late) {
+                atomicAnd(p.INV + e + tp, 0x7FFFFFFFu);
+                float4* zr = (float4*)(Bq + (size_t)tp * C);
+                for (int k = 0; k < C / 4; ++k) zr[k] = z;
+                if (p.qctl) atomicAdd(p.qctl + TR_QLATE + j, 1u);
+            }
+        }
     }
 }
 __global__ void k_zero_dx(TrainParams p, TrainBwd bw) {
@@ -1270,6 +1285,14 @@
 bool qpn_stack_bwd_fits(const TrainParams& p);
 int qpn_launch_stack_bwd(const TrainParams& p, const TrainBwd& bw, const StackQ& q, const TrainKnobs& k, hipStream_t stream);
 
+static bool bwd_persist(const TrainParams& p, const TrainKnobs& k) {
+    const bool off32 = p.N1 < (1 << 24) && (int64_t)p.N1 * (p.LC > 2 * p.C ? p.LC : 2 * p.C) < (1ll << 32);
+    return p.C == 64 && (p.Ktp == 176 || p.hoist) && p.Ap <= 64 && off32 && k.persist_bwd;
+}
+bool qpn_tap_gather_applies(const TrainParams& p, const TrainKnobs& k) {
+    return k.tap_gather && bwd_persist(p, k) && k.stack_q_bwd && p.qctl && p.qtab_b && qpn_stack_bwd_fits(p);
+}
+
 void qpn_launch_post_fb(const TrainParams& p, const TrainBwd& bw, hipStream_t stream) {
     constexpr int MTW = 5;
     const size_t ldsw = (size_t)16 * MTW * (tr_lda(256) + 2 * tr_lda(64)) * sizeof(float);
@@ -1277,13 +1300,15 @@
     hipLaunchKernelGGL((k_post_fb_w<MTW>), dim3((p.BL + 16 * MTW - 1) / (16 * MTW), p.B), dim3(512), ldsw, stream, p, bw, 1);
 }
 
-int qpn_launch_bwd(const TrainParams& p, const TrainBwd& bw, const TrainKnobs& k, const AuxGeom& ag, const StackQ* sq, hipStream_t stream, bool post_done) {
-    const int C = p.C, S = p.S, Q = p.Q, L = p.L, B = p.B, N1 = p.N1, BL = p.BL;
-    const TrainSlabs& sl = *bw.sl;
-    const bool off32 = N1 < (1 << 24) && (int64_t)N1 * (p.LC > 2 * C ? p.LC : 2 * C) < (1ll << 32);
-    const bool persist = C == 64 && (p.Ktp == 176 || p.hoist) && p.Ap <= 64 && off32 && k.persist_bwd;
-    const bool stack_q = persist && k.stack_q_bwd && sq && sq->flags && p.qctl && qpn_stack_bwd_fits(p);
+int qpn_launch_bwd(const TrainParams& p_in, const TrainBwd& bw_in, const TrainKnobs& k, const AuxGeom& ag, const StackQ* sq, hipStream_t stream, bool post_done) {
+    const int C = p_in.C, S = p_in.S, Q = p_in.Q, L = p_in.L, B = p_in.B, N1 = p_in.N1, BL = p_in.BL;
+    const TrainSlabs& sl = *bw_in.sl;
+    const bool persist = bwd_persist(p_in, k);
+    const bool stack_q = persist && k.stack_q_bwd && sq && sq->flags && p_in.qctl && qpn_stack_bwd_fits(p_in);
     const bool wr_summed = stack_q;
+    const TrainParams& p = p_in; TrainBwd bw = bw_in;
+    bw.tap_gather = p.tap_gather && stack_q ? 1 : 0;
+    if (post_done && p.tap_gather && !stack_q) { qpn_set_error("internal: the forward zeroed for the gathering queue, the backward has none"); return QPN_EINVAL; }
     const size_t nDX = (size_t)B * N1 * C;
     const size_t lds_post = (size_t)16 * (tr_lda(Q > S ? Q : S) + tr_lda(S)) * sizeof(float);
     const size_t lds_layer = (size_t)16 * (4 * tr_lda(C) + tr_lda(2 * C)) * sizeof(float);
diff --git a/qpnet_amd/csrc/train_common.h b/qpnet_amd/csrc/train_common.h
--- a/qpnet_amd/csrc/train_common.h
+++ b/qpnet_amd/csrc/train_common.h
@@ -35,6 +35,10 @@
     float* PA;
     float2* WJ;
     int* TAP;
+    int tap_gather;
+    int* TAPB;
+    unsigned* INV;
+    unsigned* INVO;
     int* XC;
     float* S0; float* Y0;
     float* logits;
@@ -64,6 +68,8 @@
 struct TrainBwd {
     const float* dlogits; float* gflat;
     float* DXA[2]; float* DXB[2];
+    float* DPT;
+    int tap_gather;
     float* DZ;
     float* DS0; float* DY0;
     float* DGS;
@@ -110,12 +116,14 @@
     bool xcd_swizzle;
     bool ce_separate;
     bool event_fence;
+    bool tap_gather;
     bool aux_hoist;
     bool test_stack_gives_up;
 };
 void qpn_train_knobs_parse(TrainKnobs& k);
 
 #define TR_QHEAD_STRIDE 1056
+#define TR_QLATE 32
 #define TR_QHDR_WORDS 17920
 struct StackQ {
     unsigned* flags;
@@ -176,7 +184,8 @@
         const int pbase = base - p.B * p.qT[l + 1];
         first = pbase + bi * p.qT[l + 1] + t_lo; n = t_hi - t_lo + 1;
     }
-    a = make_int4(n0, l | (bi << 8) | (l == p.L - 1 ? 1 << 24 : 0) | (valid ? 1 << 25 : 0) | (ly.adaptive ? 1 << 26 : 0), first, n);
+    const int gth = (p.tap_gather && ly.adaptive && l > 0) ? 1 << 27 : 0, gup = (p.tap_gather && l < p.L - 1 && p.layers[l + 1].adaptive) ? 1 << 28 : 0;
+    a = make_int4(n0, l | (bi << 8) | (l == p.L - 1 ? 1 << 24 : 0) | (valid ? 1 << 25 : 0) | (ly.adaptive ? 1 << 26 : 0) | gth | gup, first, n);
     b = make_int4((l * p.B + bi) * p.N1, ly.tap_off + bi * p.N1, p.hoist ? tr_pa_off(p, l, bi, n0) : bi * p.N1, bi * p.BL * p.LC + l * p.C);
 }
 
diff --git a/qpnet_amd/csrc/train_fwd.hip b/qpnet_amd/csrc/train_fwd.hip
--- a/qpnet_amd/csrc/train_fwd.hip
+++ b/qpnet_amd/csrc/train_fwd.hip
@@ -54,6 +54,7 @@
             p.WJ[n] = make_float2(p.flat[p.up_w + j], __int_as_float(j));
         }
     if (p.qctl && blockIdx.x == 0 && b == 0 && threadIdx.x < 32) p.qctl[threadIdx.x < 16 ? threadIdx.x : 1024 + (threadIdx.x - 16) * TR_QHEAD_STRIDE] = 0u;
+    if (p.qctl && blockIdx.x == 0 && b == 0 && threadIdx.x >= 64 && threadIdx.x < 64 + TR_MAXL) p.qctl[TR_QLATE + threadIdx.x - 64] = 0u;
     if (p.qtab && b == 0)
         for (int pos = blockIdx.x * 256 + threadIdx.x; pos <= p.qtotal; pos += nprep * 256) {
             int4 ea, eb; tr_queue_entry_fwd(p, pos, ea, eb);
@@ -102,6 +103,11 @@
             } else tap = n - ly.dilation;
             tap = tap < 0 ? 0 : (tap >= N1 ? N1 - 1 : tap);
             p.TAP[ly.tap_off + (size_t)b * N1 + n] = tap;
+            if (p.tap_gather && ly.adaptive && l > 0) {
+                unsigned* inv = p.INV + ly.tap_off + (size_t)b * N1;
+                p.INVO[ly.tap_off + (size_t)b * N1 + n] = 0xFFFFFFFFu;
+                if (n >= ly.s_out) atomicMin(inv + tap, 0x80000000u | (unsigned)n);
+            }
         }
     }
 }
diff --git a/qpnet_amd/csrc/train_host.hip b/qpnet_amd/csrc/train_host.hip
--- a/qpnet_amd/csrc/train_host.hip
+++ b/qpnet_amd/csrc/train_host.hip
@@ -7,6 +7,7 @@
 void qpn_stack_fill(TrainParams& p);
 int qpn_launch_ce(const float* logits, const int64_t* tgt, int64_t tgt_stride, int B, int BL, int Q, float* dlogits, double* loss, int* status, bool loss_cleared, hipStream_t stream);
 int qpn_launch_bwd(const TrainParams& p, const TrainBwd& bw, const TrainKnobs& k, const AuxGeom& ag, const StackQ* sq, hipStream_t stream, bool post_done);
+bool qpn_tap_gather_applies(const TrainParams& p, const TrainKnobs& k);
 int qpn_launch_fwd_gemm(const TrainParams& p, const TrainGemm& w, hipStream_t stream);
 int qpn_launch_bwd_gemm(const TrainParams& p, const TrainBwd& bw, const TrainGemm& w, hipStream_t stream);
 int qpn_launch_adam(float* w, const float* g, float* m, float* v, int64_t n, int step, float lr, float b1, float b2, float eps, float wd, const float* den, int* status,
@@ -30,6 +31,7 @@
     AuxGeom ag;
     float* d_ws; size_t ws_cap;
     int* d_tap; size_t tap_cap;
+    int inv_cur; size_t inv_ntap; int inv_B, inv_N1;
     int* d_status; double* d_loss;
     hipStream_t last_stream;
     int* h_status_pinned; hipEvent_t ev_status[2]; bool status_pending[2]; int status_newest;
@@ -76,6 +78,7 @@
     k.xcd_swizzle = getenv("QPN_NO_XCD_SWIZZLE") == nullptr;
     k.ce_separate = getenv("QPN_CE_SEPARATE") != nullptr;
     k.event_fence = env_int("QPN_EVENT_FENCE", 0) == 1;
+    k.tap_gather = env_int("QPN_TAP_GATHER", 1) != 0;
     k.aux_hoist = env_int("QPN_AUX_HOIST", 1) != 0;
     k.test_stack_gives_up = false;
 #ifdef QPN_TESTING
@@ -187,7 +190,7 @@
     memset(&t->tp, 0, sizeof(t->tp)); memset(&t->bw, 0, sizeof(t->bw));
     t->d_wmap = nullptr; t->d_wp = nullptr; t->d_bstart = t->d_blist = nullptr; t->d_bp = nullptr;
     t->d_gdst = t->d_gdst_list = t->d_gzero = nullptr; t->n_gzero = 0;
-    t->d_ws = nullptr; t->ws_cap = 0; t->d_tap = nullptr; t->tap_cap = 0; t->d_status = nullptr; t->d_loss = nullptr; t->fwd_valid = false; t->loss_clear = false;
+    t->d_ws = nullptr; t->ws_cap = 0; t->d_tap = nullptr; t->tap_cap = 0; t->inv_cur = 0; t->inv_ntap = 0; t->inv_B = t->inv_N1 = 0; t->d_status = nullptr; t->d_loss = nullptr; t->fwd_valid = false; t->loss_clear = false;
     t->generation = 0; t->side = nullptr; t->ev_fork = t->ev_join = t->ev_mid = nullptr; t->ev_early = nullptr; t->early_recorded = 0; t->early_first = -1;
     t->d_sq = nullptr; t->sq_pos_cap = 0; t->sq_per_dir = 0; t->bwd_generation = -1; t->stack_disabled = false; memset(&t->sqf, 0, sizeof(t->sqf)); memset(&t->sqb, 0, sizeof(t->sqb));
     qpn_train_knobs_parse(t->knobs);
@@ -453,7 +456,7 @@
     const size_t nDX = (size_t)B * N1 * C, nDZ = (size_t)B * N1 * 2 * C, nDGS = (size_t)B * BL * L * C, nSlab = (size_t)bw.nch * bw.gstage;
     const size_t nXC = (size_t)B * (N1 + 1);
     const size_t nScr = (size_t)B * 1024 * 2 * 128;
-    size_t need = nScr + nX + 2 * nG + nH + 2 * (nS + 96 * (size_t)S + 64) + 2 * (size_t)(L + 1) * nDX + (size_t)L * nDZ + 2 * nS + nDGS + nH + nSlab + nXC + (t->use_gemm ? nG : 0) + 2 * nPA + nWJ + nGW + (size_t)L * TR_EB_SLOTS * 2 * C + 8192;
+    size_t need = nScr + nX + 2 * nG + nH + 2 * (nS + 96 * (size_t)S + 64) + 3 * (size_t)(L + 1) * nDX + (size_t)L * nDZ + 2 * nS + nDGS + nH + nSlab + nXC + (t->use_gemm ? nG : 0) + 2 * nPA + nWJ + nGW + (size_t)L * TR_EB_SLOTS * 2 * C + 8192;
     if (need > t->ws_cap) {
         if (t->d_ws) (void)hipFree(t->d_ws);
         t->d_ws = nullptr; t->ws_cap = 0;
@@ -465,13 +468,14 @@
     if (ntap > t->tap_cap) {
         if (t->d_tap) (void)hipFree(t->d_tap);
         t->d_tap = nullptr; t->tap_cap = 0;
-        QPN_HIP(hipMalloc(&t->d_tap, ntap * sizeof(int)));
-        t->tap_cap = ntap;
+        QPN_HIP(hipMalloc(&t->d_tap, 4 * ntap * sizeof(int)));
+        t->tap_cap = ntap; t->inv_ntap = 0;
     }
     float* w = t->d_ws;
     auto carve = [&](size_t n) { float* r = w; w += (n + 63) & ~(size_t)63; return r; };
     p.X = carve(nX); p.SG = carve(nG); p.TH = carve(nG); p.HUP = carve(nH); p.S0 = carve(nS + 96 * (size_t)S); p.Y0 = carve(nS + 96 * (size_t)S);
     bw.DXA[0] = carve((size_t)(L + 1) * nDX); bw.DXB[0] = carve((size_t)(L + 1) * nDX); bw.DXA[1] = bw.DXB[1] = nullptr;
+    bw.DPT = carve((size_t)(L + 1) * nDX);
     bw.DZ = carve((size_t)L * nDZ); bw.DS0 = carve(nS); bw.DY0 = carve(nS); bw.DGS = carve(nDGS); bw.DHUP = carve(nH); bw.slab = carve(nSlab);
     p.XC = (int*)carve(nXC);
     p.scratch_rows = carve(nScr);
@@ -504,6 +508,19 @@
         f.flags = t->d_sq + TR_QHDR_WORDS; f.head = t->d_sq + 1024; f.abort = t->d_sq + 1; f.stats = t->d_sq + 4; f.epoch = epoch; f.total = p.qtotal; f.tab = p.qtab;
         bq.flags = f.flags + t->sq_per_dir; bq.head = f.head + 8 * TR_QHEAD_STRIDE; bq.abort = f.abort; bq.stats = t->d_sq + 8; bq.epoch = epoch; bq.total = p.qtotal; bq.tab = p.qtab_b;
     }
+    {
+        p.TAPB = t->d_tap + t->tap_cap;
+        p.tap_gather = (!t->use_gemm && qpn_tap_gather_applies(p, t->knobs)) ? 1 : 0;
+        if (p.tap_gather) {
+            if (t->inv_ntap != ntap || t->inv_B != B || t->inv_N1 != N1) {
+                QPN_HIP(hipMemsetAsync(t->d_tap + 2 * t->tap_cap, 0xFF, 2 * t->tap_cap * sizeof(int), stream));
+                t->inv_ntap = ntap; t->inv_B = B; t->inv_N1 = N1;
+            }
+            t->inv_cur ^= 1;
+        }
+        p.INV = (unsigned*)(t->d_tap + (size_t)(2 + t->inv_cur) * t->tap_cap); p.INVO = (unsigned*)(t->d_tap + (size_t)(3 - t->inv_cur) * t->tap_cap);
+        bw.tap_gather = p.tap_gather;
+    }
     p.flat = d_flat; p.wp = (const float4*)t->d_wp; p.bp = t->d_bp; p.x = d_x; p.h = d_h; p.d = d_dfac; p.logits = d_logits;
     {
         const int* wmap = t->use_gemm ? t->d_gmap : t->d_wmap;
diff --git a/qpnet_amd/csrc/train_stack.hip b/qpnet_amd/csrc/train_stack.hip
--- a/qpnet_amd/csrc/train_stack.hip
+++ b/qpnet_amd/csrc/train_stack.hip
@@ -45,6 +45,8 @@
 __device__ __forceinline__ bool sq_valid(const SqTile& d) { return (d.meta >> 25) & 1; }
 __device__ __forceinline__ bool sq_last(const SqTile& d) { return (d.meta >> 24) & 1; }
 __device__ __forceinline__ int sq_layer(const SqTile& d) { return d.meta & 255; }
+__device__ __forceinline__ bool sq_gathers(const SqTile& d) { return (d.meta >> 27) & 1; }
+__device__ __forceinline__ bool sq_upgathers(const SqTile& d) { return (d.meta >> 28) & 1; }
 
 struct SqRaw { int4 a, b; int pos; };
 __device__ __forceinline__ SqRaw sq_fetch(const StackQ& q, int pos) {
@@ -369,7 +371,7 @@
             asm volatile("" :: "v"(w1[NJ - 1][0].w), "v"(w1[NJ - 1][1].w), "v"(w1[NJ - 1][2].w), "v"(w1[NJ - 1][3].w), "v"(w1[NJ - 1][4].w), "v"(w1[NJ - 1][5].w), "v"(w1[NJ - 1][6].w), "v"(w1[NJ - 1][7].w));
     };
     auto rsrc = [&](const float* base) { return __builtin_amdgcn_make_buffer_rsrc((void*)base, 0, xbytes, 0x00020000); };
-    float4 ra, rb2, rsg, rth, rdg;
+    float4 ra, rb2, rc3, rsg, rth, rdg;
     auto row_off = [&](const SqTile& d) { const int n = d.n0 + srow, nn_ = n < N1 ? n : N1 - 1; return __umul24((unsigned)nn_, (unsigned)C) + 4u * sc4; };
     auto load_own = [&](const SqTile& d) {
         const unsigned o = row_off(d);
@@ -378,13 +380,24 @@
         const int nw = nn_ >= win0 ? nn_ - win0 : 0;
         rdg = *(const float4*)(bw.DGS + (size_t)d.dgs + (__umul24((unsigned)nw, (unsigned)p.LC) + 4u * sc4));
     };
-    auto load_ab = [&](const SqTile& d, float4& a4, float4& b4_) {
+    auto load_inv = [&](const SqTile& d, unsigned& w) {
+        const int n = d.n0 + srow, nn_ = n < N1 ? n : N1 - 1;
+        w = p.INV[d.tapb + (sq_upgathers(d) ? p.B * N1 : 0) + nn_];
+    };
+    auto load_ab = [&](const SqTile& d, unsigned inv, float4& a4, float4& b4_, float4& c4_) {
         const unsigned ob = sq_last(d) ? SQ_OOB : row_off(d) * 4u;
+        const bool ug = sq_upgathers(d);
+        const unsigned src = inv & 0x7FFFFFFFu;
+        const unsigned obb = (ug && (inv >> 31)) ? SQ_OOB : ob;
+        const unsigned oc = (ug && src < (unsigned)N1) ? (__umul24(src, (unsigned)C) + 4u * sc4) * 4u : SQ_OOB;
         const u32x4 a = __builtin_amdgcn_raw_buffer_load_b128(rsrc(bw.DXA[0] + (size_t)d.xrow * C + nDX), (int)ob, 0, SQ_SC1);
-        const u32x4 b4 = __builtin_amdgcn_raw_buffer_load_b128(rsrc(bw.DXB[0] + (size_t)d.xrow * C + nDX), (int)ob, 0, SQ_SC1);
+        const u32x4 c4 = __builtin_amdgcn_raw_buffer_load_b128(rsrc(bw.DPT + (size_t)d.xrow * C + nDX), (int)oc, 0, SQ_SC1);
+        const u32x4 b4 = __builtin_amdgcn_raw_buffer_load_b128(rsrc(bw.DXB[0] + (size_t)d.xrow * C + nDX), (int)obb, 0, SQ_SC1);
         a4 = make_float4(__uint_as_float(a.x), __uint_as_float(a.y), __uint_as_float(a.z), __uint_as_float(a.w));
         b4_ = make_float4(__uint_as_float(b4.x), __uint_as_float(b4.y), __uint_as_float(b4.z), __uint_as_float(b4.w));
-    };
+        c4_ = make_float4(__uint_as_float(c4.x), __uint_as_float(c4.y), __uint_as_float(c4.z), __uint_as_float(c4.w));
+    };
+    auto add4 = [](float4& a, const float4& c) { a.x += c.x; a.y += c.y; a.z += c.z; a.w += c.w; };
     auto store_own = [&](const SqTile& d, float* B) {
         const int n = d.n0 + srow;
         const bool in = n < N1;
@@ -413,11 +426,12 @@
     };
     int tprow[4];
     auto load_taps = [&](const SqTile& d, int (&tp)[4]) {
-#pragma unroll
-        for (int i = 0; i < 4; ++i) { const int n = d.n0 + 4 * wave + i; tp[i] = (p.TAP + d.tapb)[n < N1 ? n : N1 - 1]; }
+        const int* tb = (sq_gathers(d) ? p.TAPB : p.TAP) + d.tapb;
+#pragma unroll
+        for (int i = 0; i < 4; ++i) { const int n = d.n0 + 4 * wave + i; tp[i] = tb[n < N1 ? n : N1 - 1]; }
     };
     auto outputs = [&](const SqTile& d, const float* Dx) {
-        const bool adaptive = (d.meta >> 26) & 1;
+        const bool adaptive = (d.meta >> 26) & 1, gathers = sq_gathers(d);
         const int dil = p.layers[sq_layer(d)].dilation;
 #if !(SQ_EXP & 16)
         {
@@ -427,12 +441,12 @@
             const u32x4 v = {__float_as_uint(o0.x + x0.x), __float_as_uint(o0.y + x0.y), __float_as_uint(o1.x + x1.x), __float_as_uint(o1.y + x1.y)};
             const unsigned off = n < N1 ? (__umul24((unsigned)n, (unsigned)C) + 4u * sc4) * 4u : SQ_OOB;
             __builtin_amdgcn_raw_buffer_store_b128(v, rsrc(bw.DXA[0] + (size_t)d.xrow * C), (int)off, 0, SQ_SC1);
-            if (!adaptive) {
+            if (!adaptive || gathers) {
                 const float2 p0 = *(const float2*)(Os + (size_t)srow * ldo + C + 4 * sc4), p1 = *(const float2*)(Os + (size_t)srow * ldo + C + 4 * sc4 + 2);
                 const u32x4 w = {__float_as_uint(p0.x), __float_as_uint(p0.y), __float_as_uint(p1.x), __float_as_uint(p1.y)};
-                const int tr = n - dil;
+                const int tr = gathers ? n : n - dil;
                 const unsigned offb = (n < N1 && tr >= 0) ? (__umul24((unsigned)tr, (unsigned)C) + 4u * sc4) * 4u : SQ_OOB;
-                __builtin_amdgcn_raw_buffer_store_b128(w, rsrc(bw.DXB[0] + (size_t)d.xrow * C), (int)offb, 0, SQ_SC1);
+                __builtin_amdgcn_raw_buffer_store_b128(w, rsrc((gathers ? bw.DPT : bw.DXB[0]) + (size_t)d.xrow * C), (int)offb, 0, SQ_SC1);
             }
         }
 #endif
@@ -443,8 +457,9 @@
             const int r = 4 * wave + i, n = d.n0 + r;
             const bool in = n < N1;
 #if !(SQ_EXP & 1)
-            if (adaptive) {
-                float* db = DBout + (__umul24((unsigned)tprow[i], (unsigned)C) + lane);
+            const int tpi = sq_rfl(tprow[i]);
+            if (adaptive && (!gathers || tpi < 0)) {
+                float* db = DBout + (__umul24((unsigned)(tpi & 0x7FFFFFFF), (unsigned)C) + lane);
                 atomicAdd(in ? db : dmy + 128 + lane, Os[(size_t)r * ldo + C + lane]);
             }
             if constexpr (!HOIST) if (lane < Ap) {
@@ -485,9 +500,11 @@
     int lw = sq_layer(cur);
     load_weights(lw, sq_last(cur));
     sq_wait(q, cur.dfirst, cur.dn, lane, p.status, 0u);
-    load_own(cur); load_ab(cur, ra, rb2);
+    unsigned invn; load_inv(cur, invn);
+    load_own(cur); load_ab(cur, invn, ra, rb2, rc3);
     if constexpr (HOIST) load_aux(cur, cwj, cpa);
     load_taps(cur, tprow);
+    add4(ra, rc3);
     store_own(cur, sm); store_dx(cur, sm, ra, rb2);
     bool cur_published = false;
     const __amdgpu_buffer_rsrc_t frs = __builtin_amdgcn_make_buffer_rsrc((void*)q.flags, 0, (int)((sq_fidx((unsigned)q.total) + 64u) * 4u), 0x00020000);
@@ -568,20 +585,22 @@
             __builtin_amdgcn_raw_buffer_store_b32(q.epoch_pub, frs, (int)foff, 0, SQ_SC1);
         }
         __builtin_amdgcn_sched_barrier(0);
+        load_inv(next, invn);
+        __builtin_amdgcn_sched_barrier(0);
         SQB_MFMA(4); SQB_MFMA(5); SQB_MFMA(6); SQB_MFMA(7);
 #undef SQB_MFMA
         SQ_PRIO(2);
         __builtin_amdgcn_sched_barrier(0);
         SQ_STAMPB(2);
         asm volatile("s_waitcnt vmcnt(0)" ::: "memory");
-        asm volatile("" : "+v"(fv0), "+v"(fv1), "+v"(rtk), "+v"(tpn[0]), "+v"(tpn[1]), "+v"(tpn[2]), "+v"(tpn[3]));
+        asm volatile("" : "+v"(fv0), "+v"(fv1), "+v"(rtk), "+v"(tpn[0]), "+v"(tpn[1]), "+v"(tpn[2]), "+v"(tpn[3]), "+v"(invn));
         if constexpr (HOIST) asm volatile("" : "+v"(nwj[0].x), "+v"(nwj[1].x), "+v"(nwj[2].x), "+v"(nwj[3].x), "+v"(npa[0]), "+v"(npa[1]), "+v"(npa[2]), "+v"(npa[3]));
         SQ_STAMPB(3);
         bool ready = fn == 0 || (fn <= 128 && __all(fv0 == q.epoch && fv1 == q.epoch));
 #if SQ_EXP & 32
         ready = true;
 #endif
-        load_ab(next, ra, rb2);
+        load_ab(next, invn, ra, rb2, rc3);
         store_own(next, Bn);
         const SqTile n2 = sq_take(raw2);
         if (tid == 0) ctl[16 + ((it + 1) & 1)] = (int)(rtk * NQ + sub);
@@ -623,7 +642,8 @@
             TR_LDS_BARRIER();
             any_slow = sq_rfl(ctl[12] | ctl[13] | ctl[14] | ctl[15]);
         }
-        asm volatile("" : "+v"(ra.w), "+v"(rb2.w));
+        asm volatile("" : "+v"(ra.w), "+v"(rb2.w), "+v"(rc3.w));
+        add4(ra, rc3);
         if (any_slow) {
             if (tid == 0) atomicAdd(q.stats, 1u);
             outputs(cur, Dx);
@@ -632,10 +652,12 @@
             if (tid == 0 && publishes(cur)) sq_st(q.flags + sq_fidx((unsigned)cur.pos), q.epoch_pub);
             cur_published = true;
             if (!ready) sq_wait(q, next.dfirst, next.dn, lane, p.status, 0u);
-            float4 la, lb; load_ab(next, la, lb);
+            float4 la, lb, lc; load_ab(next, invn, la, lb, lc);
+            add4(la, lc);
             store_dx(next, Bn, la, lb);
         } else if (any_late) {
-            float4 la, lb; load_ab(next, la, lb);
+            float4 la, lb, lc; load_ab(next, invn, la, lb, lc);
+            add4(la, lc);
             store_dx(next, Bn, la, lb);
             outputs(cur, Dx);
         } else {
```

Result: no change. 1468 steps/s (-0.4%).
